# ChanghyeonKim93/bundle_adjustment_solver

Measured on AMD Instinct MI355X. Metric: lm_iterations_per_sec, higher is better.
Workload: dtype f64; 1 GPU; C4 stereo 6-DoF: 1000 poses / 500k landmarks / 5M obs; n_opt_poses=995, n_opt_landmarks=500000, n_observations=5000000, parallelism=single GPU, exchange=none

## Files before the change

### bundle_adjustment_solver_amd/_lib.py

```python
import ctypes as C
import os

_HERE = os.path.dirname(os.path.abspath(__file__))
LIB_PATH = os.environ.get("BA_HIP_LIB") or os.path.join(_HERE, "libba_hip.so")


class BaOptions(C.Structure):
    _fields_ = [
        ("threshold_step_size", C.c_float),
        ("threshold_cost_change", C.c_float),
        ("threshold_huber_loss", C.c_float),
        ("threshold_outlier_rejection", C.c_float),
        ("max_num_iterations", C.c_int),
        ("initial_lambda", C.c_float),
        ("decrease_ratio_lambda", C.c_float),
        ("increase_ratio_lambda", C.c_float),
        ("gauss_newton", C.c_int),
    ]


def make_options(max_iter=50, thr_step=1e-5, thr_cost=1e-5, huber=1.0,
                 outlier=2.0, lambda0=100.0, dec=0.33, inc=3.0,
                 gauss_newton=False):
    o = BaOptions()
# ... 47 lines not shown

SIGNATURES = {
    "ba_create": (C.c_int, [C.POINTER(_P), C.c_int]),
    "ba_destroy": (None, [_P]),
    "ba_last_error": (C.c_char_p, []),
    "ba_set_stream": (C.c_int, [_P, _P]),
    "ba_set_cameras": (C.c_int, [_P, C.c_int, _D, _D]),
    "ba_set_poses": (C.c_int, [_P, C.c_int, _D, _U8]),
    "ba_set_points": (C.c_int, [_P, C.c_int, _D, _U8]),
    "ba_set_observations": (C.c_int, [_P, C.c_int64, _I32, _I32, _I32, _D]),
    "ba_set_shard": (C.c_int, [_P, C.c_int, C.c_int]),
    "ba_finalize": (C.c_int, [_P]),
    "ba_update_values": (C.c_int, [_P, _D, _D]),
    "ba_partition_points": (C.c_int, [C.c_int, _U8, C.c_int, _U8, C.c_int64,
                                      _I32, _I32, C.c_int, _I32]),
    "ba_set_allreduce": (C.c_int, [_P, ALLREDUCE_FN, _P]),
    "ba_reduce_buffer_size": (C.c_int64, [_P, C.c_int]),
    "ba_bind_reduce_buffer": (C.c_int, [_P, C.c_int, _P, C.c_int64]),
    "ba_gather_points": (C.c_int, [_P]),
    "ba_rccl_available": (C.c_int, []),
    "ba_rccl_get_unique_id": (C.c_int, [_U8]),
    "ba_rccl_comm_create": (C.c_int, [C.POINTER(_P), C.c_int, C.c_int, _U8, C.c_int]),
    "ba_rccl_comm_size": (C.c_int, [_P]),
    "ba_rccl_comm_calls": (C.c_int64, [_P]),
    "ba_rccl_comm_destroy": (None, [_P]),
    "ba_rccl_allreduce_hook": (C.c_int, [_P, C.c_int, _P, C.c_int64, _P]),
    "ba_stream_create": (C.c_int, [C.POINTER(_P), C.c_int, C.c_int, C.c_int64]),
    "ba_stream_destroy": (None, [_P]),
    "ba_stream_set_cameras": (C.c_int, [_P, C.c_int, _D, _D]),
    "ba_stream_set_poses": (C.c_int, [_P, C.c_int, _D, _U8]),
    "ba_stream_set_points": (C.c_int, [_P, C.c_int, _D, _U8]),
    "ba_stream_set_observations": (C.c_int, [_P, C.c_int64, _I32, _I32, _I32, _D]),
    "ba_stream_finalize": (C.c_int, [_P]),
    "ba_stream_solve": (C.c_int, [_P, C.POINTER(BaOptions), C.POINTER(BaIterInfo),
                                  C.c_int, C.POINTER(C.c_int), C.POINTER(C.c_int)]),
    "ba_stream_lm_begin": (C.c_int, [_P, C.POINTER(BaOptions)]),
    "ba_stream_lm_iterate": (C.c_int, [_P, C.c_int]),
    "ba_stream_lm_sync": (C.c_int, [_P, C.POINTER(BaIterInfo), C.c_int,
                                    C.POINTER(C.c_int), C.POINTER(C.c_int)]),
    "ba_stream_get_poses": (C.c_int, [_P, _D]),
    "ba_stream_get_points": (C.c_int, [_P, _D]),
    "ba_stream_info": (C.c_int, [_P, C.POINTER(C.c_int64)]),
    "ba_solve": (C.c_int, [_P, C.POINTER(BaOptions), C.POINTER(BaIterInfo),
                           C.c_int, C.POINTER(C.c_int), C.POINTER(C.c_int)]),
    "ba_lm_begin": (C.c_int, [_P, C.POINTER(BaOptions)]),
    "ba_lm_iterate": (C.c_int, [_P, C.c_int]),
    "ba_lm_sync": (C.c_int, [_P, C.POINTER(BaIterInfo), C.c_int,
                             C.POINTER(C.c_int), C.POINTER(C.c_int)]),
    "ba_gd_begin": (C.c_int, [_P, C.POINTER(BaOptions)]),
    "ba_gd_iterate": (C.c_int, [_P, C.c_int]),
    "ba_gd_sync": (C.c_int, [_P, C.POINTER(BaIterInfo), C.c_int,
                             C.POINTER(C.c_int), C.POINTER(C.c_int)]),
    "ba_solve_gd": (C.c_int, [_P, C.POINTER(BaOptions), C.POINTER(BaIterInfo),
                              C.c_int, C.POINTER(C.c_int), C.POINTER(C.c_int)]),
    "ba_gd_get_gradient": (C.c_int, [_P, _D, _D]),
    "ba_stage_cost": (C.c_int, [_P, _D]),
    "ba_stage_linearize": (C.c_int, [_P, C.c_double, C.c_double]),
    "ba_stage_schur": (C.c_int, [_P]),
    "ba_stage_solve_reduced": (C.c_int, [_P]),
    "ba_stage_backsub_update": (C.c_int, [_P]),
    "ba_stage_scalars": (C.c_int, [_P, _D, _D, _D, _D]),
    "ba_stage_commit": (C.c_int, [_P, C.c_int]),
    "ba_enable_stage_timing": (C.c_int, [_P, C.c_int]),
    "ba_get_stage_ms": (C.c_int, [_P, _D, C.c_int]),
    "ba_num_opt_poses": (C.c_int, [_P]),
    "ba_num_opt_points": (C.c_int, [_P]),
    "ba_num_pairs": (C.c_int64, [_P]),
    "ba_num_schur_blocks": (C.c_int64, [_P]),
    "ba_num_schur_triples": (C.c_int64, [_P]),
    "ba_get_poses": (C.c_int, [_P, _D]),
    "ba_get_points": (C.c_int, [_P, _D, _U8]),
    "ba_get_A": (C.c_int, [_P, _D, _D]),
    "ba_get_C": (C.c_int, [_P, _D, _D]),
    "ba_get_Cinv": (C.c_int, [_P, _D, _D]),
    "ba_get_pairs": (C.c_int, [_P, _I32, _I32, _D]),
    "ba_get_S": (C.c_int, [_P, _D, _D]),
    "ba_get_xy": (C.c_int, [_P, _D, _D]),
    "ba_kernel_count": (C.c_int, []),
    "ba_kernel_name": (C.c_char_p, [C.c_int]),
    "ba_get_kernel_ms": (C.c_int, [_P, _D, C.POINTER(C.c_int64), C.c_int]),
    "ba_get_dense_info": (C.c_int, [_P, _D]),
    "ba_get_schur_info": (C.c_int, [_P, C.POINTER(C.c_int64)]),
    "ba_get_lin_info": (C.c_int, [_P, C.POINTER(C.c_int64)]),
    "ba_get_mask_info": (C.c_int, [_P, C.POINTER(C.c_int64)]),
    "ba_get_dropped_pivots": (C.c_int, [_P, C.POINTER(C.c_int64), C.c_int]),
    "ba_dense_spd_solve": (C.c_int, [_P, C.c_int, _D, _D, _D, _D]),
    "ba_pose_only_mono6": (C.c_int, [_P, _F, _F, C.c_int, C.c_float, C.c_float,
                                     C.c_float, C.c_float, _F, _U8,
                                     C.POINTER(BaOptions), C.POINTER(BaPoIter),
                                     C.c_int, C.POINTER(C.c_int),
                                     C.POINTER(C.c_int), _F]),
    "ba_pose_only_stereo6": (C.c_int, [_P, _F, _F, _F, C.c_int, _F, _F, _F, _F,
                                       _U8, _U8, C.POINTER(BaOptions),
                                       C.POINTER(BaPoIter), C.c_int,
                                       C.POINTER(C.c_int), C.POINTER(C.c_int),
                                       _F]),
    "ba_pose_only_mono3": (C.c_int, [_P, _F, _F, C.c_int, C.c_float, C.c_float,
                                     C.c_float, C.c_float, _F, _F, _F, _U8,
                                     C.POINTER(BaOptions), C.POINTER(BaPoIter),
                                     C.c_int, C.POINTER(C.c_int),
                                     C.POINTER(C.c_int), _F]),
    "ba_pose_only_stereo3": (C.c_int, [_P, _F, _F, _F, C.c_int, _F, _F, _F, _F,
                                       _F, _F, _U8, _U8, C.POINTER(BaOptions),
                                       C.POINTER(BaPoIter), C.c_int,
                                       C.POINTER(C.c_int), C.POINTER(C.c_int),
                                       _F]),
    "ba_pose_only_mono6_batch": (C.c_int, [_P, C.c_int, _I32, _F, _F, _F, _F, _U8,
                                           C.POINTER(BaOptions), C.POINTER(BaPoIter),
                                           C.c_int, C.POINTER(BaPoResult), _F]),
    "ba_pose_only_stereo6_batch": (C.c_int, [_P, C.c_int, _I32, _F, _F, _F, _F, _F,
                                             _F, _F, _U8, _U8, C.POINTER(BaOptions),
                                             C.POINTER(BaPoIter), C.c_int,
                                             C.POINTER(BaPoResult), _F]),
    "ba_pose_only_mono6_batch_device": (C.c_int, [_P, C.c_int, _P, _P, _P, _P, _P, _P,
                                                  C.POINTER(BaOptions), _P, C.c_int,
                                                  _P, _P, _P]),
    "ba_pose_only_stereo6_batch_device": (C.c_int, [_P, C.c_int, _P, _P, _P, _P, _P, _P,
                                                    _P, _P, _P, C.POINTER(BaOptions),
                                                    _P, C.c_int, _P, _P, _P]),
    "ba_right_camera_record": (C.c_int, [_F, _F, _F]),
    "ba_pose_only_mono3_batch": (C.c_int, [_P, C.c_int, _I32, _F, _F, _F, _F, _F, _F, _U8,
                                           C.POINTER(BaOptions), C.POINTER(BaPoIter),
                                           C.c_int, C.POINTER(BaPoResult), _F]),
    "ba_pose_only_stereo3_batch": (C.c_int, [_P, C.c_int, _I32, _F, _F, _F, _F, _F, _F,
                                             _F, _F, _F, _U8, _U8, C.POINTER(BaOptions),
                                             C.POINTER(BaPoIter), C.c_int,
                                             C.POINTER(BaPoResult), _F]),
    "ba_pose_only_mono3_batch_device": (C.c_int, [_P, C.c_int, _P, _P, _P, _P, _P, _P, _P,
                                                  C.POINTER(BaOptions), _P, C.c_int,
                                                  _P, _P, _P]),
    "ba_pose_only_stereo3_batch_device": (C.c_int, [_P, C.c_int, _P, _P, _P, _P, _P, _P,
                                                    _P, _P, _P, C.POINTER(BaOptions),
                                                    _P, C.c_int, _P, _P, _P]),
    "ba_planar_record": (C.c_int, [_F, _F, _F, _F, _F, _F]),
}

_lib = None


def _preload_shared_hip_runtime():
    import importlib.util
    try:
        spec = importlib.util.find_spec("torch")
    except (ImportError, ValueError):
        spec = None
    if spec is None or not spec.submodule_search_locations:
        return
    libdir = os.path.join(list(spec.submodule_search_locations)[0], "lib")
    for name in ("libhsa-runtime64.so", "libamdhip64.so"):
        path = os.path.join(libdir, name)
        if os.path.exists(path):
            try:
                C.CDLL(path, mode=C.RTLD_GLOBAL)
            except OSError:
                return


def load():
    global _lib
    if _lib is not None:
        return _lib
    if not os.path.exists(LIB_PATH):
        raise RuntimeError(
            "libba_hip.so is not built (%s). Run `python -c 'import "
            "__graft_entry__ as g; g.build()'` or `make -C "
            "bundle_adjustment_solver_amd/csrc`. The HIP path has no CPU "
# ... 21 lines not shown
```

### bundle_adjustment_solver_amd/csrc/ba_api.hip

```cpp
#include <hip/hip_runtime.h>

#include <algorithm>
#include <chrono>
#include <cmath>
#include <cstdio>
#include <cstdlib>
#include <cstring>
#include <string>
#include <vector>

#include "ba_handle.h"

namespace {
thread_local std::string g_err;
}
void ba::set_last_error(const std::string &m) { g_err = m; }
int ba::fail(const std::string &m) {
  g_err = m;
  return -1;
}
using ba::fail;

namespace {

// ... 421 lines not shown
    for (int64_t bk = 0; bk < pl.B; ++bk) {
      int32_t *r = bd.data() + 16 * bk;
      const int64_t c0 = pl.blk_contrib_ptr[bk], c1 = pl.blk_contrib_ptr[bk + 1];
      r[0] = pl.sblk_j[bk];
      r[1] = pl.sblk_k[bk];
      r[2] = (int32_t)c0;
      r[3] = (int32_t)(c1 - c0);
      r[4] = pl.sblk_tchunk_ptr[bk];
      r[5] = pl.sblk_tchunk_ptr[bk + 1] - pl.sblk_tchunk_ptr[bk];
      for (int t = 0; t < 8; ++t) r[8 + t] = c0 + t < c1 ? pl.contrib_slot[c0 + t] : 0;
    }
    if (pl.contrib_slot.size() >= (size_t)INT32_MAX) return fail("too many slot contributions for int32 indices");
    if (h->upload(&d.blk_desc, bd)) return -1;
  }
  d.n_sup = (int)pl.sup_desc.size();
  d.n_bchunk = (int)pl.bchunk_lm.size() - 1;
  if (h->upload(&d.bchunk_lm, pl.bchunk_lm)) return -1;
  {
    std::vector<ba::DevProblem::LmChunk> lc((size_t)d.n_bchunk);
    for (int c = 0; c < d.n_bchunk; ++c) {
      const int l0 = pl.bchunk_lm[c], l1 = pl.bchunk_lm[c + 1];
      lc[c].pb = pl.lm_pair_ptr[l0];
      lc[c].ob = pl.lm_obs_ptr[l0];
      lc[c].l0 = l0;
      lc[c].nl = l1 - l0;
      lc[c].np = (int32_t)(pl.lm_pair_ptr[l1] - pl.lm_pair_ptr[l0]);
      lc[c].no = (int32_t)(pl.lm_obs_ptr[l1] - pl.lm_obs_ptr[l0]);
    }
    if (h->upload(&d.lm_chunk, lc)) return -1;
  }
  d.n_slot = (int)pl.slot_blk.size();
  {
    static_assert(sizeof(ba::Plan::SupDesc) == sizeof(ba::DevProblem::SupDesc), "desc layout");
    static_assert(sizeof(ba::Plan::ChunkDesc) == sizeof(ba::DevProblem::ChunkDesc), "desc layout");
    if (h->dalloc(&d.sup_desc, pl.sup_desc.size()) || h->dalloc(&d.chunk_desc, pl.chunk_desc.size()))
      return -1;
    if (!pl.sup_desc.empty())
      HIP_TRY(hipMemcpy(d.sup_desc, pl.sup_desc.data(), pl.sup_desc.size() * sizeof(ba::Plan::SupDesc),
                        hipMemcpyHostToDevice));
    if (!pl.chunk_desc.empty())
      HIP_TRY(hipMemcpy(d.chunk_desc, pl.chunk_desc.data(),
                        pl.chunk_desc.size() * sizeof(ba::Plan::ChunkDesc), hipMemcpyHostToDevice));
  }
  h->kind(2);
  if (h->dalloc(&d.spart2, (size_t)d.n_slot * ba::kSlotStride)) return -1;
  h->kind(1);
  {
    static_assert(sizeof(ba::Plan::GrpDesc) == sizeof(ba::DevProblem::GrpDesc) && sizeof(ba::Plan::GrpDesc) == 128,
                  "group descriptor layout");
    static_assert(sizeof(ba::Plan::LinDesc) == sizeof(ba::DevProblem::LinDesc) && sizeof(ba::Plan::LinDesc) == 48,
                  "group linearisation descriptor layout");
    d.n_grp32 = (int)pl.grp32.size();
    d.n_grp64 = (int)pl.grp64.size();
    d.n_grp128 = (int)pl.grp128.size();
    if (h->dalloc(&d.grp32, pl.grp32.size()) || h->dalloc(&d.grp64, pl.grp64.size()) ||
        h->dalloc(&d.grp128, pl.grp128.size()))
      return -1;
    if (d.n_grp128)
      HIP_TRY(hipMemcpy(d.grp128, pl.grp128.data(), pl.grp128.size() * sizeof(ba::Plan::GrpDesc), hipMemcpyHostToDevice));
    if (d.n_grp32)
      HIP_TRY(hipMemcpy(d.grp32, pl.grp32.data(), pl.grp32.size() * sizeof(ba::Plan::GrpDesc), hipMemcpyHostToDevice));
    if (d.n_grp64)
      HIP_TRY(hipMemcpy(d.grp64, pl.grp64.data(), pl.grp64.size() * sizeof(ba::Plan::GrpDesc), hipMemcpyHostToDevice));
    d.lin_chunk0 = pl.lin_groups ? pl.n_bchunk_grp : 0;
    d.n_lin_desc = (int)pl.lin_desc.size();
    d.n_lin_plain = pl.n_lin_plain;
    d.n_bs_grp = d.n_lin_desc;
    d.n_lm_part = d.n_bs_grp + (d.n_bchunk - d.lin_chunk0 + ba::kBsChunks - 1) / ba::kBsChunks;
    d.n_lin_cost = d.n_bchunk + d.n_lin_desc;
    if (h->dalloc(&d.lin_desc, pl.lin_desc.size())) return -1;
    if (d.n_lin_desc)
      HIP_TRY(hipMemcpy(d.lin_desc, pl.lin_desc.data(), pl.lin_desc.size() * sizeof(ba::Plan::LinDesc), hipMemcpyHostToDevice));
    if (h->dalloc(&d.grp_pat, pl.grp_pat.size() / 2) || h->upload(&d.pose_gpart_ptr, pl.pose_gpart_ptr) ||
        h->upload(&d.pose_gpart, pl.pose_gpart))
      return -1;
    h->kind(2);
    if (h->dalloc(&d.Apart2, (size_t)pl.n_apart2 * 27) || h->dalloc(&d.lin_dump, (size_t)ba::kLinDump)) return -1;
    if (!pl.grp_pat.empty())
      HIP_TRY(hipMemcpy(d.grp_pat, pl.grp_pat.data(), pl.grp_pat.size() * sizeof(int32_t), hipMemcpyHostToDevice));
    if (pl.n_apart2 > 0) HIP_TRY(hipMemset(d.Apart2, 0, (size_t)pl.n_apart2 * 27 * sizeof(double)));
  }

  lap("structure uploads");
  for (int k = 0; k < 2; ++k) {
    h->kind(2);
    if (h->dalloc(&d.Cu[k], (size_t)pl.M * 6) || h->dalloc(&d.b[k], (size_t)pl.M * 3) ||
        h->dalloc(&d.W[k], std::max<size_t>(2, (size_t)pl.P * ba::kWStride)))
      return -1;
    h->kind(0);
    if (h->dalloc(&d.A[k], (size_t)pl.N * 36) || h->dalloc(&d.a[k], (size_t)pl.N * 6)) return -1;
    HIP_TRY(hipMemset(d.W[k], 0, std::max<size_t>(1, (size_t)pl.P * ba::kWStride) * sizeof(double)));
    HIP_TRY(hipMemset(d.A[k], 0, std::max<size_t>(1, (size_t)pl.N * 36) * sizeof(double)));
    HIP_TRY(hipMemset(d.a[k], 0, std::max<size_t>(1, (size_t)pl.N * 6) * sizeof(double)));
  }
  d.n_obs_lm = pl.M > 0 ? pl.lm_obs_ptr[pl.M] : 0;
  h->kind(2);
  if (h->dalloc(&d.Cd, (size_t)pl.M * 6) || h->dalloc(&d.Cinv, (size_t)pl.M * 6) ||
      h->dalloc(&d.lin_cost_part, (size_t)std::max(1, d.n_lin_cost)) ||
      h->dalloc(&d.Apart, (size_t)d.n_achunk * 27) ||
      h->dalloc(&d.spart, (size_t)d.n_tchunk * ba::kSlotStride) ||
      h->dalloc(&d.y, (size_t)pl.M * 3) || h->dalloc(&d.lm_part, (size_t)std::max(1, d.n_lm_part) * 2))
    return -1;
  h->kind(0);
  if (h->dalloc(&d.x, (size_t)pl.N * 6 + 64) || h->dalloc(&d.cost_part, (size_t)ba::kCostGrid) ||
      h->dalloc(&d.pose_part, (size_t)2 + 2 * ba::kPoseGrid) ||
      h->dalloc(&d.scal, (size_t)4) || h->dalloc(&d.ctrl, (size_t)1))
    return -1;
  HIP_TRY(hipMemset(d.lin_cost_part, 0, (size_t)std::max(1, d.n_lin_cost) * sizeof(double)));
  HIP_TRY(hipMemset(d.x, 0, ((size_t)pl.N * 6 + 64) * sizeof(double)));
  HIP_TRY(hipMemset(d.y, 0, std::max<size_t>(1, (size_t)pl.M * 3) * sizeof(double)));
  HIP_TRY(hipMemset(d.cost_part, 0, ba::kCostGrid * sizeof(double)));
  HIP_TRY(hipMemset(d.lm_part, 0, (size_t)std::max(1, d.n_lm_part) * 2 * sizeof(double)));
  HIP_TRY(hipMemset(d.pose_part, 0, (2 + 2 * ba::kPoseGrid) * sizeof(double)));
  HIP_TRY(hipMemset(d.scal, 0, 4 * sizeof(double)));
  d.log_cap = 4096;
  if (h->dalloc(&d.log, (size_t)d.log_cap)) return -1;

  lap("block storage");
  if (h->dense_owner) {
    const ba_handle *o = h->dense_owner;
    if (!o->finalized || o->plan.N != pl.N || o->plan.B != pl.B)
      return fail("ba_finalize: the dense owner belongs to a different problem");
    h->sched = o->sched;
    h->ddev = o->ddev;
    h->pose_col_h = o->pose_col_h;
    d.nb = o->d.nb; d.npad = o->d.npad; d.ld = o->d.ld;
    d.L = o->d.L; d.Ldiag = o->d.Ldiag; d.pose_col = o->d.pose_col; d.col_x = o->d.col_x;
    d.zt_I = o->d.zt_I; d.zt_J = o->d.zt_J; d.n_zt = o->d.n_zt;
    d.x = o->d.x;
    h->xbuf_n[0] = pl.B * 36 + 6 * (int64_t)pl.N;
    h->xbuf_n[1] = 4;
    h->xbuf_n[2] = 3 * (int64_t)pl.n_pt_global;
    if (h->dalloc(&d.Spk, (size_t)h->xbuf_n[0])) return -1;
    HIP_TRY(hipMemset(d.Spk, 0, (size_t)h->xbuf_n[0] * sizeof(double)));
  } else {
    const char *nat = getenv("BA_DENSE_NATURAL");
    const char *full = getenv("BA_DENSE_FULL");
    const char *force = getenv("BA_DENSE_NB");
    ba::DenseSchedule cand[2];
    double cost[2];
    const int orders[2] = {32, 64};
    const double level_us[2] = {16.0, 30.0};
    for (int k = 0; k < 2; ++k) {
      int ncb_k = 0;
      std::vector<uint8_t> adj;
      ba::tile_pattern(pl, ba::dense_poses_per_tile(orders[k]), ncb_k, adj);
      if (full && atoi(full) != 0) std::fill(adj.begin(), adj.end(), 1);
      ba::build_dense_schedule(ncb_k, adj, nat && atoi(nat) != 0, orders[k], cand[k]);
      cost[k] = cand[k].nlev * level_us[k];
    }
    if (getenv("BA_PLAN_STATS"))
      fprintf(stderr, "dense schedules: nb32 %d tiles %d levels max_rows %d fill %.3f | nb64 %d tiles %d levels max_rows %d fill %.3f\n",
              cand[0].ncb, cand[0].nlev, cand[0].max_rows, cand[0].fill, cand[1].ncb, cand[1].nlev, cand[1].max_rows,
              cand[1].fill);
    const bool narrow = cand[0].max_rows <= 6;
    int pick = (narrow && cost[0] <= cost[1]) ? 0 : 1;
    if (force && atoi(force) == 32) pick = 0;
    if (force && atoi(force) == 64) pick = 1;
    h->sched = cand[pick];
    const int nb = h->sched.nb;
    const int ppt = ba::dense_poses_per_tile(nb);
    const int ncb = h->sched.ncb;
    d.nb = nb;
    d.npad = ncb * nb;
    d.ld = d.npad + nb;
    h->xbuf_n[0] = pl.B * 36 + 6 * (int64_t)pl.N;
    h->xbuf_n[1] = 4;
    h->xbuf_n[2] = 3 * (int64_t)pl.n_pt_global;
    if (h->dalloc(&d.Spk, (size_t)h->xbuf_n[0])) return -1;
    if (h->dalloc(&d.L, (size_t)d.npad * d.ld)) return -1;
    if (h->dalloc(&d.Ldiag, (size_t)ncb * ba::dense_ws_per_block(nb))) return -1;
    h->pose_col_h.assign(pl.N, 0);
    std::vector<int> col_x((size_t)d.npad, -1);
    for (int j = 0; j < pl.N; ++j) {
      const int c0 = h->sched.pos_of_tile[j / ppt] * nb + 6 * (j % ppt);
      h->pose_col_h[j] = c0;
      for (int r = 0; r < 6; ++r) col_x[c0 + r] = 6 * j + r;
    }
    const ba::DenseSchedule &sc = h->sched;
    ba::DenseDev &dd = h->ddev;
    if (h->upload(&d.pose_col, h->pose_col_h) || upload_dense_schedule(h, sc, col_x, dd)) return -1;
    d.col_x = dd.col_x;
    if (times && dd.dag_items) fprintf(stderr, "[finalize] k_chol_dag: %d items\n", dd.n_dag_items);
    std::vector<int> ztI, ztJ;
    for (int p = 0; p < ncb; ++p) {
      ztI.push_back(p);
      ztJ.push_back(p);
      for (int q = sc.row_ptr[p]; q < sc.row_ptr[p + 1]; ++q) {
        ztI.push_back(sc.rows[q]);
        ztJ.push_back(p);
      }
    }
    d.n_zt = (int)ztI.size();
    if (h->upload(&d.zt_I, ztI) || h->upload(&d.zt_J, ztJ)) return -1;
    HIP_TRY(hipMemset(d.L, 0, (size_t)d.npad * d.ld * sizeof(double)));
    HIP_TRY(hipMemset(d.Spk, 0, (size_t)h->xbuf_n[0] * sizeof(double)));
  }

  lap("dense schedule + image");
  std::memset(&h->hc, 0, sizeof(h->hc));
  h->hc.lambda = 100.0;
  h->hc.huber = 1.0;
  h->hc.max_iter = 1;
  HIP_TRY(hipMemcpy(d.ctrl, &h->hc, sizeof(ba::DevCtrl), hipMemcpyHostToDevice));
  HIP_TRY(hipDeviceSynchronize());
  h->finalized = true;
  return 0;
}

int ba_update_values(ba_handle *h, const double *T_jw12, const double *X3) {
  if (!h || !h->finalized) return fail("ba_update_values: not finalized");
  if (h->arena) return fail("ba_update_values: not available on a streamed chunk");
  if (use_device(h)) return -1;
  const ba::Plan &pl = h->plan;
  join_side(h);
  HIP_TRY(hipStreamSynchronize(h->stream));
  if (T_jw12) {
    h->pose_T.assign(T_jw12, T_jw12 + 12 * (size_t)pl.n_pose);
    std::vector<double> poses((size_t)pl.n_pose * 12);
    for (int p = 0; p < pl.n_pose; ++p)
      std::memcpy(&poses[(size_t)p * 12], T_jw12 + (size_t)pl.pose_user_of_int[p] * 12, 12 * sizeof(double));
    for (int k = 0; k < 2; ++k)
      HIP_TRY(hipMemcpy(h->d.poses[k], poses.data(), poses.size() * sizeof(double), hipMemcpyHostToDevice));
  }
  if (X3) {
    h->pt_X.assign(X3, X3 + 3 * (size_t)pl.n_pt_global);
    std::vector<double> pts((size_t)pl.n_pt * 3);
    for (int q = 0; q < pl.n_pt; ++q)
      std::memcpy(&pts[(size_t)q * 3], X3 + (size_t)pl.pt_user_of_int[q] * 3, 3 * sizeof(double));
    if (pl.n_pt > 0)
      for (int k = 0; k < 2; ++k)
        HIP_TRY(hipMemcpy(h->d.pts[k], pts.data(), pts.size() * sizeof(double), hipMemcpyHostToDevice));
  }
  h->gathered_valid = false;
  h->lm_begun = false;
  h->gd_begun = false;
  h->tiles_ready = false;
  return 0;
}

int ba_set_allreduce(ba_handle *h, ba_allreduce_fn fn, void *user) {
  if (!h) return fail("null handle");
  h->ar_fn = fn;
  h->ar_user = user;
  return 0;
}

int64_t ba_reduce_buffer_size(ba_handle *h, int which) {
  if (!h || !h->finalized || which < 0 || which > 2) return -1;
  return h->xbuf_n[which];
}

int ba_bind_reduce_buffer(ba_handle *h, int which, void *dev_ptr, int64_t n) {
  if (!h || !h->finalized) return fail("ba_bind_reduce_buffer: not finalized");
  h->drop_graph();
  if (which < 0 || which > 2 || !dev_ptr || n < h->xbuf_n[which])
    return fail("ba_bind_reduce_buffer: bad argument");
  if (which == 0)
    h->d.Spk = (double *)dev_ptr;
  else if (which == 1)
    h->d.scal = (double *)dev_ptr;
  else {
    h->gbuf = (double *)dev_ptr;
    h->gbuf_bound = true;
  }
  return 0;
}

}

int ba::lm_prepare_ctrl(ba_handle *h, const ba_options *opt, int *done_after) {
  if (opt->max_num_iterations > h->d.log_cap) {
    ba::DevIterRec *nl = nullptr;
    const int keep = h->alloc_kind;
    h->alloc_kind = 0;
    const int rc = h->dalloc(&nl, (size_t)opt->max_num_iterations);
    h->alloc_kind = keep;
    if (rc) return -1;
    h->drop_graph();
    h->d.log = nl;
    h->d.log_cap = opt->max_num_iterations;
  }
  h->tiles_ready = false;
  h->gathered_valid = false;
  if (pull_ctrl(h)) return -1;
  ba::DevCtrl &c = h->hc;
  c.lambda = (double)opt->initial_lambda;
  c.huber = (double)opt->threshold_huber_loss;
  c.thr_step = (double)opt->threshold_step_size;
  c.thr_cost = (double)opt->threshold_cost_change;
  c.dec_ratio = (double)opt->decrease_ratio_lambda;
  c.inc_ratio = (double)opt->increase_ratio_lambda;
  c.max_iter = opt->max_num_iterations;
  c.gn = opt->gauss_newton ? 1 : 0;
  c.iter = 0;
  c.converged = 0;
  c.prev_cost = 0.0;
  *done_after = (opt->max_num_iterations <= 0) ? 1 : 0;
  c.done = 0;
  if (push_ctrl(h)) return -1;
  HIP_TRY(hipMemsetAsync(h->ddev.bad_pivots, 0, sizeof(int), h->stream));
  return 0;
}
int ba::ctrl_pull(ba_handle *h) { return pull_ctrl(h); }
int ba::ctrl_push(ba_handle *h) { return push_ctrl(h); }

extern "C" {

int ba_lm_begin(ba_handle *h, const ba_options *opt) {
  if (!h || !opt) return fail("ba_lm_begin: bad argument");
  if (!h->finalized && ba_finalize(h)) return -1;
  if (use_device(h)) return -1;
  join_side(h);
  int done_after = 0;
  if (ba::lm_prepare_ctrl(h, opt, &done_after)) return -1;
  h->gd_begun = false;
  enqueue_linearize(h, 0);
  ba::launch_scalars_cost_only(h->d, 1, h->stream);
  if (xchg(h, 1)) return -1;
  ba::launch_init_ctrl_cost(h->d, h->stream);
  if (done_after) {
    if (pull_ctrl(h)) return -1;
    h->hc.done = 1;
    if (push_ctrl(h)) return -1;
  }
  HIP_TRY(hipGetLastError());
  h->lm_begun = true;
  return 0;
}

int ba_lm_iterate(ba_handle *h, int n) {
  if (h && !h->lm_begun && h->gd_begun)
    return fail("ba_lm_iterate: the handle is in a gradient-descent loop (ba_gd_begin); call ba_lm_begin first");
  if (!h || !h->lm_begun) return fail("ba_lm_iterate: call ba_lm_begin first");
  if (use_device(h)) return -1;
  h->gathered_valid = false;
  const bool graphable = h->use_graph && !h->timing && !h->ar_fn && h->stream != nullptr;
  if (graphable && !h->graph_exec && n > 0) {
    HIP_TRY(hipStreamBeginCapture(h->stream, hipStreamCaptureModeThreadLocal));
    const int rc = enqueue_iteration(h);
    hipGraph_t g = nullptr;
    const hipError_t ec = hipStreamEndCapture(h->stream, &g);
    if (rc != 0 || ec != hipSuccess || !g) {
      if (g) (void)hipGraphDestroy(g);
      (void)hipGetLastError();
      h->use_graph = false;
    } else {
      h->graph = g;
      if (hipGraphInstantiate(&h->graph_exec, g, nullptr, nullptr, 0) != hipSuccess) {
        (void)hipGetLastError();
        h->drop_graph();
        h->use_graph = false;
      }
    }
  }
  for (int k = 0; k < n; ++k) {
    if (graphable && h->graph_exec) {
      HIP_TRY(hipGraphLaunch(h->graph_exec, h->stream));
    } else if (enqueue_iteration(h)) {
      return -1;
    }
  }
  return 0;
}

int ba_lm_sync(ba_handle *h, ba_iter_info *out, int cap, int *n_iter,
               int *converged) {
  if (!h || !h->lm_begun) return fail("ba_lm_sync: call ba_lm_begin first");
  if (use_device(h)) return -1;
  if (h->side_pending) (void)hipStreamWaitEvent(h->stream, h->ev_join, 0);
  if (pull_ctrl(h)) return -1;
  {
    int bp = 0;
    HIP_TRY(hipMemcpy(&bp, h->ddev.bad_pivots, sizeof(int), hipMemcpyDeviceToHost));
    if (bp >= ba::kFlowTimeout)
      return fail("ba_lm_sync: a dataflow hand-off of the reduced solve timed out (" +
                  std::to_string(bp / ba::kFlowTimeout) + " polls gave up); the iterations since ba_lm_begin "
                  "are invalid. BA_DENSE_FLOW=0 selects the per-level launches");
  }
  const int n = h->hc.iter;
  if (n_iter) *n_iter = n;
  if (converged) *converged = h->hc.converged;
  if (out && cap > 0 && n > 0) {
    static_assert(sizeof(ba::DevIterRec) == sizeof(ba_iter_info), "iter layout");
    const int m = std::min(std::min(n, cap), h->d.log_cap);
    HIP_TRY(hipMemcpy(out, h->d.log, (size_t)m * sizeof(ba_iter_info), hipMemcpyDeviceToHost));
  }
  return h->hc.done ? 1 : 0;
}

int ba_solve(ba_handle *h, const ba_options *opt, ba_iter_info *out, int cap,
             int *n_iter, int *converged) {
  if (ba_lm_begin(h, opt)) return -1;
  int done = opt->max_num_iterations <= 0;
  int issued = 0;
  while (!done) {
    const int batch = std::min(4, opt->max_num_iterations - issued);
    if (batch <= 0) break;
    if (ba_lm_iterate(h, batch)) return -1;
    issued += batch;
    int rc = ba_lm_sync(h, nullptr, 0, nullptr, nullptr);
    if (rc < 0) return -1;
    done = rc;
  }
  int rc = ba_lm_sync(h, out, cap, n_iter, converged);
  return rc < 0 ? -1 : 0;
}


static int gd_prepare(ba_handle *h, const char *who) {
// ... 93 lines not shown
  h->gathered_valid = false;
  for (int k = 0; k < n; ++k) {
    ba::launch_gd_update(h->d, h->gd, h->stream);
    ba::launch_gd_pass(h->d, h->gd, h->stream);
    ba::launch_gd_control(h->d, h->gd, 1, h->stream);
  }
  HIP_TRY(hipGetLastError());
  return 0;
}

int ba_gd_sync(ba_handle *h, ba_iter_info *out, int cap, int *n_iter, int *converged) {
  if (!h) return fail("ba_gd_sync: null handle");
  if (!h->gd_begun) return fail("ba_gd_sync: call ba_gd_begin first");
  if (use_device(h)) return -1;
  if (pull_ctrl(h)) return -1;
  const int n = h->hc.iter;
  if (n_iter) *n_iter = n;
  if (converged) *converged = h->hc.converged;
  if (out && cap > 0 && n > 0) {
    const int m = std::min(std::min(n, cap), h->d.log_cap);
    HIP_TRY(hipMemcpy(out, h->d.log, (size_t)m * sizeof(ba_iter_info), hipMemcpyDeviceToHost));
  }
  return h->hc.done ? 1 : 0;
}

int ba_solve_gd(ba_handle *h, const ba_options *opt, ba_iter_info *out, int cap, int *n_iter, int *converged) {
  if (ba_gd_begin(h, opt)) return -1;
  int done = opt->max_num_iterations <= 0;
  int issued = 0;
  while (!done) {
    const int batch = std::min(8, opt->max_num_iterations - issued);
    if (batch <= 0) break;
    if (ba_gd_iterate(h, batch)) return -1;
    issued += batch;
    const int rc = ba_gd_sync(h, nullptr, 0, nullptr, nullptr);
    if (rc < 0) return -1;
    done = rc;
  }
  const int rc = ba_gd_sync(h, out, cap, n_iter, converged);
  return rc < 0 ? -1 : 0;
}

int ba_gd_get_gradient(ba_handle *h, double *a6, double *b3) {
  if (!h || !h->finalized) return fail("ba_gd_get_gradient: not finalized");
  if (!h->gd_ready) return fail("ba_gd_get_gradient: call ba_gd_begin first");
  if (use_device(h)) return -1;
  const ba::Plan &pl = h->plan;
  HIP_TRY(hipStreamSynchronize(h->stream));
  if (a6 && pl.N > 0) HIP_TRY(hipMemcpy(a6, h->gd.a, (size_t)pl.N * 6 * sizeof(double), hipMemcpyDeviceToHost));
  if (b3) {
    std::vector<double> b;
    if (download(b, h->gd.b, (size_t)pl.M * 3, h->stream)) return -1;
    for (int i = 0; i < pl.M; ++i)
      std::memcpy(b3 + (size_t)pl.iopt_of_user[pl.pt_user_of_int[i]] * 3, &b[(size_t)i * 3], 3 * sizeof(double));
  }
  return 0;
}

int ba_stage_cost(ba_handle *h, double *cost) {
  if (!h || !h->finalized || !cost) return fail("ba_stage_cost: bad argument");
  if (use_device(h)) return -1;
  if (pull_ctrl(h)) return -1;
  h->hc.done = 0;
  if (push_ctrl(h)) return -1;
  join_side(h);
  ba::launch_cost(h->d, 0, 0, h->stream);
  ba::launch_scalars_cost_only(h->d, 0, h->stream);
  if (xchg(h, 1)) return -1;
  HIP_TRY(hipMemcpyAsync(cost, h->d.scal, sizeof(double), hipMemcpyDeviceToHost, h->stream));
  HIP_TRY(hipStreamSynchronize(h->stream));
  return 0;
}

int ba_stage_linearize(ba_handle *h, double lambda, double huber) {
  if (!h || !h->finalized) return fail("ba_stage_linearize: not finalized");
  if (use_device(h)) return -1;
  if (pull_ctrl(h)) return -1;
  h->hc.done = 0;
  h->hc.lambda = lambda;
  h->hc.huber = huber;
  if (push_ctrl(h)) return -1;
  join_side(h);
  enqueue_linearize(h, 0);
  ba::launch_damp_invert(h->d, h->stream);
  HIP_TRY(hipStreamSynchronize(h->stream));
  HIP_TRY(hipGetLastError());
  return 0;
}

int ba_stage_schur(ba_handle *h) {
  if (!h || !h->finalized) return fail("ba_stage_schur: not finalized");
  if (use_device(h)) return -1;
  join_side(h);
  ba::launch_schur(h->d, false, true, h->stream);
  if (xchg(h, 0)) return -1;
  HIP_TRY(hipStreamSynchronize(h->stream));
  HIP_TRY(hipGetLastError());
  return 0;
}

int ba_stage_solve_reduced(ba_handle *h) {
  if (!h || !h->finalized) return fail("ba_stage_solve_reduced: not finalized");
  if (use_device(h)) return -1;
  ba::launch_scatter(h->d, h->stream);
  ba::launch_dense_solve(h->d, h->sched, h->ddev, h->stream);
  HIP_TRY(hipStreamSynchronize(h->stream));
  HIP_TRY(hipGetLastError());
  return 0;
}

int ba_stage_backsub_update(ba_handle *h) {
  if (!h || !h->finalized) return fail("ba_stage_backsub_update: not finalized");
  if (use_device(h)) return -1;
  ba::launch_backsub_update(h->d, h->stream);
  HIP_TRY(hipStreamSynchronize(h->stream));
  HIP_TRY(hipGetLastError());
  return 0;
}

int ba_stage_scalars(ba_handle *h, double *trial_cost, double *model_change,
                     double *pose_step_sum, double *point_step_sum) {
  if (!h || !h->finalized) return fail("ba_stage_scalars: not finalized");
  if (use_device(h)) return -1;
  ba::launch_cost(h->d, 1, 0, h->stream);
  ba::launch_scalars(h->d, 0, h->stream);
  if (xchg(h, 1)) return -1;
  double sc[4], pp[2];
  HIP_TRY(hipMemcpyAsync(sc, h->d.scal, sizeof(sc), hipMemcpyDeviceToHost, h->stream));
  HIP_TRY(hipMemcpyAsync(pp, h->d.pose_part, sizeof(pp), hipMemcpyDeviceToHost, h->stream));
  HIP_TRY(hipStreamSynchronize(h->stream));
  if (trial_cost) *trial_cost = sc[0];
  if (model_change) *model_change = -sc[1];
  if (point_step_sum) *point_step_sum = sc[2];
  if (pose_step_sum) *pose_step_sum = pp[1];
  return 0;
}

int ba_stage_commit(ba_handle *h, int accept) {
  if (!h || !h->finalized) return fail("ba_stage_commit: not finalized");
  if (use_device(h)) return -1;
  h->gathered_valid = false;
  if (pull_ctrl(h)) return -1;
  if (accept) h->hc.cur ^= 1;
  if (push_ctrl(h)) return -1;
  HIP_TRY(hipStreamSynchronize(h->stream));
  return 0;
}

int ba_enable_stage_timing(ba_handle *h, int on) {
  if (!h) return fail("null handle");
  if (use_device(h)) return -1;
  if (on && !h->ev_ok) {
    for (int k = 0; k <= ST_N; ++k) HIP_TRY(hipEventCreate(&h->ev[k]));
    h->ev_ok = true;
  }
  h->timing = on != 0;
  h->kt.on = h->timing;
  return 0;
}

int ba_get_stage_ms(ba_handle *h, double out8[8], int reset) {
  if (!h || !out8) return fail("ba_get_stage_ms: bad argument");
  for (int k = 0; k < 8; ++k) out8[k] = h->stage_ms[k];
  if (reset)
    for (int k = 0; k < 8; ++k) h->stage_ms[k] = 0.0;
  return 0;
}

int ba_num_opt_poses(ba_handle *h) { return (h && h->finalized) ? h->plan.N : -1; }
int ba_num_opt_points(ba_handle *h) { return (h && h->finalized) ? h->plan.M : -1; }
int64_t ba_num_pairs(ba_handle *h) { return (h && h->finalized) ? h->plan.P - h->plan.n_pair_pad : -1; }
int64_t ba_num_schur_blocks(ba_handle *h) { return (h && h->finalized) ? h->plan.B : -1; }
int64_t ba_num_schur_triples(ba_handle *h) { return (h && h->finalized) ? h->plan.T : -1; }

int ba_get_poses(ba_handle *h, double *T_jw12) {
  if (!h || !h->finalized || !T_jw12) return fail("ba_get_poses: bad argument");
  if (use_device(h) || pull_ctrl(h)) return -1;
  std::vector<double> buf;
  if (download(buf, h->d.poses[h->hc.cur], (size_t)h->plan.n_pose * 12, h->stream)) return -1;
  for (int p = 0; p < h->plan.n_pose; ++p)
    std::memcpy(T_jw12 + (size_t)h->plan.pose_user_of_int[p] * 12, &buf[(size_t)p * 12],
                12 * sizeof(double));
  return 0;
}

__global__ void k_points_to_user(const double *__restrict__ src, const int32_t *__restrict__ user_of_int, int n,
                                 double *__restrict__ dst) {
  const int q = blockIdx.x * blockDim.x + threadIdx.x;
  if (q >= n) return;
  const size_t u = (size_t)user_of_int[q] * 3;
  dst[u + 0] = src[(size_t)q * 3 + 0];
  dst[u + 1] = src[(size_t)q * 3 + 1];
  dst[u + 2] = src[(size_t)q * 3 + 2];
}

int ba_gather_points(ba_handle *h) {
  if (!h || !h->finalized) return fail("ba_gather_points: not finalized");
  if (use_device(h)) return -1;
  h->gathered_valid = false;
  if (!h->ar_fn || h->world <= 1) return 0;
  const ba::Plan &pl = h->plan;
  const size_t n3 = (size_t)pl.n_pt_global * 3;
  if (!h->gbuf && h->dalloc(&h->gbuf, n3)) return -1;
  if (!h->pt_user_dev && h->upload(&h->pt_user_dev, pl.pt_user_of_int)) return -1;
  if (pull_ctrl(h)) return -1;
  join_side(h);
  HIP_TRY(hipMemsetAsync(h->gbuf, 0, n3 * sizeof(double), h->stream));
  if (pl.n_pt > 0)
    hipLaunchKernelGGL(k_points_to_user, dim3((pl.n_pt + 255) / 256), dim3(256), 0, h->stream,
                       (const double *)h->d.pts[h->hc.cur], (const int32_t *)h->pt_user_dev, pl.n_pt, h->gbuf);
  if (h->ar_fn(h->ar_user, 2, (void *)h->gbuf, (int64_t)n3, (void *)h->stream) != 0)
    return fail("ba_gather_points: all-reduce hook returned an error");
  if (download(h->gathered, h->gbuf, n3, h->stream)) return -1;
  HIP_TRY(hipGetLastError());
  h->gathered_valid = true;
  return 0;
}

int ba_get_points(ba_handle *h, double *X3, uint8_t *owned_mask) {
  if (!h || !h->finalized || !X3) return fail("ba_get_points: bad argument");
  if (h->gathered_valid) {
    std::memcpy(X3, h->gathered.data(), h->gathered.size() * sizeof(double));
    if (owned_mask) std::memset(owned_mask, 1, (size_t)h->plan.n_pt_global);
    return 0;
  }
  if (use_device(h) || pull_ctrl(h)) return -1;
// ... 12 lines not shown
  if (!h || !h->finalized) return fail("ba_get_A: not finalized");
  if (use_device(h)) return -1;
  join_side(h);
  if (pull_ctrl(h)) return -1;
  const int lb = h->hc.lcur;
  if (A36) {
    HIP_TRY(hipMemcpy(A36, h->d.A[lb], (size_t)h->plan.N * 36 * sizeof(double), hipMemcpyDeviceToHost));
    const double lp1 = 1.0 + h->hc.lambda;
    for (int j = 0; j < h->plan.N; ++j)
      for (int r = 0; r < 6; ++r) A36[(size_t)j * 36 + r * 7] *= lp1;
  }
  if (a6) HIP_TRY(hipMemcpy(a6, h->d.a[lb], (size_t)h->plan.N * 6 * sizeof(double), hipMemcpyDeviceToHost));
  return 0;
}

static void expand_sym3(const double *s6, double *f9) {
  f9[0] = s6[0]; f9[1] = s6[1]; f9[2] = s6[2];
  f9[3] = s6[1]; f9[4] = s6[3]; f9[5] = s6[4];
  f9[6] = s6[2]; f9[7] = s6[4]; f9[8] = s6[5];
}

static int get_sym_vec(ba_handle *h, const double *dS6, const double *dV3,
                       double *out9, double *out3) {
  const ba::Plan &pl = h->plan;
  std::vector<double> s6, v3;
  if (download(s6, dS6, (size_t)pl.M * 6, h->stream)) return -1;
  if (download(v3, dV3, (size_t)pl.M * 3, h->stream)) return -1;
  for (int i = 0; i < pl.M; ++i) {
    const int g = pl.iopt_of_user[pl.pt_user_of_int[i]];
    if (out9) expand_sym3(&s6[(size_t)i * 6], out9 + (size_t)g * 9);
    if (out3) std::memcpy(out3 + (size_t)g * 3, &v3[(size_t)i * 3], 3 * sizeof(double));
  }
  return 0;
}

int ba_get_C(ba_handle *h, double *C9, double *b3) {
  if (!h || !h->finalized) return fail("ba_get_C: not finalized");
  if (use_device(h)) return -1;
  join_side(h);
  if (pull_ctrl(h)) return -1;
  ba::launch_damp_invert_export(h->d, h->stream);
  return get_sym_vec(h, h->d.Cd, h->d.b[h->hc.lcur], C9, b3);
}

int ba_get_Cinv(ba_handle *h, double *Cinv9, double *Cinvb3) {
  if (!h || !h->finalized) return fail("ba_get_Cinv: not finalized");
  if (use_device(h)) return -1;
  const ba::Plan &pl = h->plan;
  std::vector<double> s6, b3;
  join_side(h);
  if (pull_ctrl(h)) return -1;
  ba::launch_damp_invert_export(h->d, h->stream);
  if (download(s6, h->d.Cinv, (size_t)pl.M * 6, h->stream)) return -1;
  if (download(b3, h->d.b[h->hc.lcur], (size_t)pl.M * 3, h->stream)) return -1;
  for (int i = 0; i < pl.M; ++i) {
    const int g = pl.iopt_of_user[pl.pt_user_of_int[i]];
    const double *ci = &s6[(size_t)i * 6], *b = &b3[(size_t)i * 3];
    if (Cinv9) expand_sym3(ci, Cinv9 + (size_t)g * 9);
    if (Cinvb3) {
      double *o = Cinvb3 + (size_t)g * 3;
      o[0] = ci[0] * b[0] + ci[1] * b[1] + ci[2] * b[2];
      o[1] = ci[1] * b[0] + ci[3] * b[1] + ci[4] * b[2];
      o[2] = ci[2] * b[0] + ci[4] * b[1] + ci[5] * b[2];
    }
  }
  return 0;
}

int ba_get_pairs(ba_handle *h, int32_t *pair_i, int32_t *pair_j, double *W18) {
  if (!h || !h->finalized) return fail("ba_get_pairs: not finalized");
  if (use_device(h)) return -1;
  const ba::Plan &pl = h->plan;
  auto padded = [&](int64_t p) { return !pl.pair_pad.empty() && pl.pair_pad[p]; };
  {
    int64_t o = 0;
    for (int64_t p = 0; p < pl.P; ++p) {
      if (padded(p)) continue;
      if (pair_i) pair_i[o] = pl.iopt_of_user[pl.pt_user_of_int[pl.pair_lm[p]]];
      if (pair_j) pair_j[o] = pl.pair_pose[p];
      ++o;
    }
  }
  if (W18) {
    if (pull_ctrl(h)) return -1;
    std::vector<double> w12((size_t)pl.P * ba::kWStride);
    if (pl.P > 0)
      HIP_TRY(hipMemcpy(w12.data(), h->d.W[h->hc.lcur], w12.size() * sizeof(double), hipMemcpyDeviceToHost));
    int64_t o = 0;
    for (int64_t p = 0; p < pl.P; ++p) {
      if (padded(p)) continue;
      const double *k = &w12[(size_t)p * ba::kWStride];
      double *W = W18 + (size_t)o * 18;
      for (int e = 0; e < 9; ++e) W[e] = k[e];
      for (int c = 0; c < 3; ++c) {
        W[9 + c] = k[10] * k[6 + c] - k[11] * k[3 + c];
        W[12 + c] = k[11] * k[c] - k[9] * k[6 + c];
        W[15 + c] = k[9] * k[3 + c] - k[10] * k[c];
      }
      ++o;
    }
  }
  return 0;
}

int ba_get_S(ba_handle *h, double *S, double *rhs) {
  if (!h || !h->finalized) return fail("ba_get_S: not finalized");
  if (use_device(h)) return -1;
  const ba::DevProblem &d = h->d;
  const int n6 = 6 * h->plan.N;
  std::vector<double> L;
  ba::launch_scatter(d, h->stream);
  if (download(L, d.L, (size_t)d.npad * d.ld, h->stream)) return -1;
  auto colof = [&](int e) { return h->pose_col_h[e / 6] + e % 6; };
  for (int c = 0; c < n6; ++c) {
    for (int r = c; r < n6; ++r) {
      int rr = colof(r), cc = colof(c);
      if (rr < cc) std::swap(rr, cc);
      const double v = L[(size_t)cc * d.ld + rr];
      if (S) {
        S[(size_t)r * n6 + c] = v;
        S[(size_t)c * n6 + r] = v;
      }
    }
    if (rhs) rhs[c] = L[(size_t)colof(c) * d.ld + d.npad];
  }
  return 0;
}

int ba_get_xy(ba_handle *h, double *x6, double *y3) {
  if (!h || !h->finalized) return fail("ba_get_xy: not finalized");
  if (use_device(h)) return -1;
  const ba::Plan &pl = h->plan;
  HIP_TRY(hipStreamSynchronize(h->stream));
  if (x6 && pl.N > 0)
    HIP_TRY(hipMemcpy(x6, h->d.x, (size_t)pl.N * 6 * sizeof(double), hipMemcpyDeviceToHost));
  if (y3) {
    std::vector<double> y;
    if (download(y, h->d.y, (size_t)pl.M * 3, h->stream)) return -1;
    for (int i = 0; i < pl.M; ++i) {
      const int g = pl.iopt_of_user[pl.pt_user_of_int[i]];
      std::memcpy(y3 + (size_t)g * 3, &y[(size_t)i * 3], 3 * sizeof(double));
    }
  }
  return 0;
}

int ba_kernel_count(void) { return ba::K_COUNT; }

const char *ba_kernel_name(int id) {
  static const char *names[ba::K_COUNT] = {
      "k_cost", "k_lin_landmarks", "k_lin_poses", "k_pose_finalize", "k_dense_init",
      "k_schur_lds", "k_schur_partial", "k_schur_final", "k_scatter",
      "k_chol_diag", "k_chol_trsm", "k_chol_update", "k_chol_back", "k_chol_diag_trsm", "k_chol_tail", "k_backsub_update",
      "k_pose_update", "k_scalars", "k_control", "k_damp_invert", "k_schur_grp", "k_lin_grp"};
  return (id >= 0 && id < ba::K_COUNT) ? names[id] : "";
}

int ba_get_kernel_ms(ba_handle *h, double *ms_out, int64_t *calls_out, int reset) {
  if (!h || !ms_out || !calls_out) return fail("ba_get_kernel_ms: bad argument");
  for (int k = 0; k < ba::K_COUNT; ++k) {
    ms_out[k] = h->kt.ms[k];
    calls_out[k] = h->kt.calls[k];
  }
  if (reset) h->kt.reset();
  return 0;
}

int ba_get_dense_info(ba_handle *h, double out4[4]) {
  if (!h || !h->finalized || !out4) return fail("ba_get_dense_info: bad argument");
  out4[0] = h->sched.fill;
  out4[1] = h->sched.flops;
  out4[2] = (double)h->sched.nlev;
  out4[3] = (double)h->d.npad;
  return 0;
}

int ba_get_schur_info(ba_handle *h, int64_t out8[8]) {
  if (!h || !h->finalized || !out8) return fail("ba_get_schur_info: bad argument");
  const ba::Plan &pl = h->plan;
  int64_t pairs = 0, triples = 0, mfma = 0;
  for (const auto *list : {&pl.grp32, &pl.grp64, &pl.grp128})
    for (const auto &g : *list) {
      pairs += (int64_t)g.nl * g.d;
      triples += (int64_t)g.nl * g.d * (g.d + 1) / 2;
      const int nt = list == &pl.grp32 ? 2 : (list == &pl.grp64 ? 4 : 8), krw = nt == 2 ? 36 : (nt == 4 ? 20 : 8);
      const int nlw = std::min(64 / g.d, krw / 3);
      for (int c0 = 0; c0 < g.nl; c0 += nlw)
        mfma += (int64_t)((3 * std::min(nlw, g.nl - c0) + 3) / 4) * (nt * (nt + 1) / 2);
    }
  out8[0] = (int64_t)pl.grp32.size();
  out8[1] = (int64_t)(pl.grp64.size() + pl.grp128.size());
  out8[2] = pl.M_grp;
  out8[3] = (int64_t)pl.sup_desc.size();
  out8[4] = pairs;
  out8[5] = triples;
  out8[6] = mfma;
  out8[7] = (int64_t)pl.tri_p.size();
  return 0;
}

int ba_get_lin_info(ba_handle *h, int64_t out4[4]) {
  if (!h || !h->finalized || !out4) return fail("ba_get_lin_info: bad argument");
  const ba::Plan &pl = h->plan;
  int64_t obs = 0;
  for (const auto &g : pl.lin_desc) obs += (int64_t)g.nl * g.no;
  out4[0] = (int64_t)pl.lin_desc.size();
  out4[1] = obs;
  out4[2] = (int64_t)pl.bchunk_lm.size() - 1 - (pl.lin_groups ? pl.n_bchunk_grp : 0);
  out4[3] = pl.n_pobs;
  return 0;
}

int ba_get_mask_info(ba_handle *h, int64_t out4[4]) {
  if (!h || !h->finalized || !out4) return fail("ba_get_mask_info: bad argument");
  const ba::Plan &pl = h->plan;
  int64_t lm = 0;
  for (const auto &g : pl.grp_range) lm += g.masked ? g.nl : 0;
  out4[0] = (int64_t)pl.lin_desc.size() - pl.n_lin_plain;
  out4[1] = lm;
  out4[2] = pl.n_obs - (pl.n_obs_global > 0 && h->world == 1 ? pl.n_obs_global : pl.n_obs);
  {
    int64_t pad = 0;
    for (int64_t s2 = 0; s2 < pl.n_obs; ++s2) pad += !(pl.obs_uv[2 * s2] == pl.obs_uv[2 * s2]);
    out4[2] = pad;
  }
  out4[3] = pl.n_pair_pad;
  return 0;
}

int ba_get_dropped_pivots(ba_handle *h, int64_t *count, int reset) {
  if (!h || !h->finalized || !count) return fail("ba_get_dropped_pivots: bad argument");
  if (use_device(h)) return -1;
  int v = 0;
  HIP_TRY(hipMemcpyAsync(&v, h->ddev.bad_pivots, sizeof(int), hipMemcpyDeviceToHost, h->stream));
  if (reset) HIP_TRY(hipMemsetAsync(h->ddev.bad_pivots, 0, sizeof(int), h->stream));
  HIP_TRY(hipStreamSynchronize(h->stream));
  *count = v % ba::kFlowTimeout;
  return 0;
}

int ba_dense_spd_solve(ba_handle *h, int n, const double *A, const double *b,
                       double *x, double *ms) {
  if (!h || n <= 0 || !A || !b || !x) return fail("ba_dense_spd_solve: bad argument");
  if (use_device(h)) return -1;
  const int nb = 64;
  const int ncb = (n + nb - 1) / nb;
  const int npad = ncb * nb;
  const int ld = npad + nb;
  std::vector<uint8_t> adj((size_t)ncb * ncb, 0);
  for (int I = 0; I < ncb; ++I)
    for (int J = 0; J < I; ++J) {
      bool any = false;
      for (int r = I * nb; r < std::min(n, (I + 1) * nb) && !any; ++r)
        for (int c = J * nb; c < (J + 1) * nb && !any; ++c) any = A[(size_t)r * n + c] != 0.0;
      adj[(size_t)I * ncb + J] = adj[(size_t)J * ncb + I] = any;
    }
  ba::DenseSchedule sc;
  const char *nat = getenv("BA_DENSE_NATURAL");
  ba::build_dense_schedule(ncb, adj, nat && atoi(nat) != 0, nb, sc);
  std::vector<int> colmap(npad), col_x(npad, -1);
  for (int c = 0; c < npad; ++c) colmap[c] = sc.pos_of_tile[c / nb] * nb + c % nb;
  std::vector<double> L((size_t)npad * ld, 0.0);
  for (int c = 0; c < npad; ++c) {
    if (c < n) {
      col_x[colmap[c]] = c;
      for (int r = c; r < n; ++r) {
        int rr = colmap[r], cc = colmap[c];
        if (rr < cc) std::swap(rr, cc);
        L[(size_t)cc * ld + rr] = A[(size_t)r * n + c];
      }
      L[(size_t)colmap[c] * ld + npad] = b[c];
    } else {
      L[(size_t)colmap[c] * ld + colmap[c]] = 1.0;
    }
  }
  struct Scratch {
    ba_handle *h;
    size_t mark;
    int kind;
    ~Scratch() {
// ... 522 lines not shown
```

### bundle_adjustment_solver_amd/csrc/ba_device.h

```cpp
#ifndef BA_DEVICE_H_
#define BA_DEVICE_H_

#include <hip/hip_runtime.h>
#include <stdint.h>
#include <stdlib.h>

#include <vector>

namespace ba {

struct DevCtrl {
  double lambda;
  double prev_cost;
  double huber;
  double thr_step;
  double thr_cost;
  double dec_ratio;
  double inc_ratio;
  unsigned long long t_last;
  int cur;
  int done;
  int iter;
  int converged;
  int max_iter;
  int gn;
  int lcur;
  int tcur, tlcur;
  int pad_;
};

struct DevIterRec {
  double cost, cost_change, average_reprojection_error, abs_gradient, abs_step,
      damping_term, iter_time_ms;
  int iteration_status, pad_;
  double rho, model_change, trial_cost;
};

constexpr int kWStride = 12;

struct DevProblem {
  int n_cam, n_pose, N, n_pt, M, M_global;
  int64_t n_obs, n_obs_opt, n_obs_global, P, n_pobs, T, B;
  int n_achunk, n_tchunk;
  double *cams;
  double *poses[2];
  double *pts[2];
  int4 *obs_idx;
  double2 *obs_uv;
  int64_t *lm_obs_ptr;
  int64_t *lm_pair_ptr;
  int32_t *pair_pose;
  int32_t *pair_lm;
  int2 *pobs_idx;
  int2 *obs_cp;
  double2 *pobs_uv;
  int32_t *achunk_pose;
  int64_t *achunk_begin, *achunk_end;
  int32_t *pose_achunk_ptr;
  int32_t *sblk_j, *sblk_k;
  int32_t *diag_blk;
  int64_t *tri_p, *tri_q;
  int32_t *tchunk_blk;
  int64_t *tchunk_begin, *tchunk_end;
  int32_t *sblk_tchunk_ptr;
  int n_sup, n_slot;
  struct SupDesc {
    int32_t s0, ns, chunk_begin, chunk_end;
  };
  struct ChunkDesc {
    int64_t p0, tb, sp;
    int32_t l0, nl, np, nt;
  };
  struct GrpDesc {
    int64_t p0;
    int32_t l0, nl, d, s0;
    int32_t pose[20];
    int32_t pad_[6];
  };
  struct LinDesc {
    int64_t p0, o0;
    int32_t l0, nl, d, no;
    int32_t pat0;
    int32_t apart0, cost_idx;
    int32_t pad_;
  };
  LinDesc *lin_desc;
  int n_lin_desc;
  int n_lin_plain;
  GrpDesc *grp32, *grp64, *grp128;
  int n_grp32, n_grp64, n_grp128;
  int2 *grp_pat;
  double *Apart2;
  double *lin_dump;
  int32_t *pose_gpart_ptr, *pose_gpart;
  int lin_chunk0;
  int n_lin_cost;
  int n_bs_grp;
  int n_lm_part;
  SupDesc *sup_desc;
  uint32_t *sup_lane;
  ChunkDesc *chunk_desc;
  uint16_t *chunk_sp;
  uint32_t *ltri;
  int64_t *blk_contrib_ptr;
  int32_t *contrib_slot;
  int32_t *blk_desc;
  double *spart2;
  double *Cu[2];
  double *b[2];
  double *W[2];
  double *A[2];
  double *a[2];
  double *Cinv;
  double *Cd;
  double *Apart;
  double *spart;
  double *x;
  double *y;
  double *cost_part;
  double *lin_cost_part;
  int64_t n_obs_lm;
  double *lm_part;
  double *pose_part;
  double *scal;
  DevCtrl *ctrl;
  DevIterRec *log;
  int log_cap;
  double *Spk;
  double *L;
  int npad, ld;
  double *Ldiag;
  int nb;
  int *pose_col;
  int *col_x;
  int32_t *bchunk_lm;
  struct LmChunk {
    int64_t pb, ob;
    int32_t l0, nl, np, no;
  };
  LmChunk *lm_chunk;
  int n_bchunk;
  int *zt_I, *zt_J;
  int n_zt;
};

constexpr int kLinDump = 64 * 4 * 4;
constexpr int kFlowTimeout = 1 << 20;
constexpr int kBsChunks = 4;
constexpr int kCostGrid = 1792;
constexpr int kLmGrid = 1024;
constexpr int kPoseGrid = 16;
constexpr int kGdFixGrid = 1024;
constexpr int kGdChunk = 512;
constexpr int kSlotStride = 42;

enum KernelId {
  K_COST = 0, K_LIN_LANDMARKS, K_LIN_POSES, K_POSE_FINALIZE, K_DENSE_INIT,
  K_SCHUR_LDS, K_SCHUR_PARTIAL, K_SCHUR_FINAL, K_SCATTER,
  K_CHOL_DIAG, K_CHOL_TRSM, K_CHOL_UPDATE, K_CHOL_BACK, K_CHOL_DIAG_TRSM, K_CHOL_TAIL, K_BACKSUB_UPDATE,
  K_POSE_UPDATE, K_SCALARS, K_CONTROL, K_DAMP_INVERT, K_SCHUR_GRP, K_LIN_GRP, K_COUNT
};
struct KernelTimer {
  bool on = false;
  std::vector<hipEvent_t> pool;
  std::vector<int> ids;
  double ms[K_COUNT] = {0};
  long calls[K_COUNT] = {0};
  void begin(int id, hipStream_t s);
  void end(hipStream_t s);
  void collect();
  void reset();
};
extern thread_local KernelTimer *g_ktimer;
#define BA_LAUNCH(id, kernel, grid, block, stream, ...)                     \
  do {                                                                      \
    if (::ba::g_ktimer && ::ba::g_ktimer->on) ::ba::g_ktimer->begin(id, stream); \
    hipLaunchKernelGGL(kernel, grid, block, 0, stream, __VA_ARGS__);        \
    if (::ba::g_ktimer && ::ba::g_ktimer->on) ::ba::g_ktimer->end(stream);  \
  } while (0)

#define BA_KEEP_S(x) asm volatile("" ::"s"(x))

void launch_cost(const DevProblem &d, int sel, int64_t begin, hipStream_t s);
void launch_lin_poses(const DevProblem &d, int sel, hipStream_t s);
void launch_lin_landmarks(const DevProblem &d, int sel, hipStream_t s);
void launch_damp_invert(const DevProblem &d, hipStream_t s);
void launch_schur(const DevProblem &d, bool direct, bool with_init, hipStream_t s);
void launch_schur_accumulate(const DevProblem &d, hipStream_t s);
void launch_schur_final(const DevProblem &d, bool direct, hipStream_t s);
void launch_backsub_update(const DevProblem &d, hipStream_t s, bool zero_tiles = false);
void launch_scatter(const DevProblem &d, hipStream_t s);
void launch_scalars_cost_only(const DevProblem &d, int cost_src, hipStream_t s);
void launch_scalars(const DevProblem &d, int cost_src, hipStream_t s);
// ... 129 lines not shown
```

### bundle_adjustment_solver_amd/csrc/ba_handle.h

```cpp
#ifndef BA_HANDLE_H_
#define BA_HANDLE_H_

#include <hip/hip_runtime.h>

#include <cstdint>
#include <chrono>
#include <string>
#include <vector>

#include "../../include/ba_hip.h"
#include "ba_dense_sched.h"
#include "ba_device.h"
#include "ba_plan.h"

namespace ba {
void launch_damp_invert_export(const DevProblem &d, hipStream_t s);
void set_last_error(const std::string &m);
int fail(const std::string &m);

struct DeviceArena {
  char *base = nullptr;
  size_t cap = 0;
};
}

#define HIP_TRY(expr)                                                        \
  do {                                                                       \
    hipError_t e_ = (expr);                                                  \
    if (e_ != hipSuccess)                                                    \
      return ::ba::fail(std::string(#expr) + ": " + hipGetErrorString(e_));  \
  } while (0)

enum Stage { ST_BUILD = 0, ST_SCHUR, ST_SOLVE, ST_BACKSUB, ST_COST, ST_CTRL, ST_XCHG, ST_N = 8 };

struct ba_handle {
  int device = 0;
  hipStream_t own_stream = nullptr;
  hipStream_t stream = nullptr;
  hipStream_t side_stream = nullptr;
  hipEvent_t ev_fork = nullptr, ev_join = nullptr;
  bool overlap = true;
  bool side_pending = false;
  bool tiles_ready = false;
  bool use_graph = false;
  hipGraph_t graph = nullptr;
  hipGraphExec_t graph_exec = nullptr;
  void drop_graph() {
    if (graph_exec) (void)hipGraphExecDestroy(graph_exec);
    if (graph) (void)hipGraphDestroy(graph);
    graph_exec = nullptr;
    graph = nullptr;
  }
  int n_cam = 0, n_pose = 0, n_pt = 0;
  int64_t n_obs = 0;
  std::vector<double> cam_intr, cam_T, pose_T, pt_X, obs_uv;
  std::vector<uint8_t> pose_fixed, pt_fixed;
  std::vector<int32_t> obs_cam, obs_pose, obs_pt;
  int rank = 0, world = 1;
  bool finalized = false;
  ba::Plan plan;
  ba::DevProblem d;
  std::vector<void *> allocs;
  ba_allreduce_fn ar_fn = nullptr;
  void *ar_user = nullptr;
  int64_t xbuf_n[3] = {0, 0, 0};
  double *gbuf = nullptr;
  bool gbuf_bound = false;
  int32_t *pt_user_dev = nullptr;
  std::vector<double> gathered;
  bool gathered_valid = false;
  ba::DevCtrl hc;
  bool timing = false;
  hipEvent_t ev[ST_N + 1];
  bool ev_ok = false;
  double stage_ms[ST_N] = {0, 0, 0, 0, 0, 0, 0, 0};
  bool lm_begun = false;
  ba::KernelTimer kt;
  ba::DenseSchedule sched;
  ba::DenseDev ddev;
  std::vector<int> pose_col_h;
  bool gd_ready = false;
  bool gd_begun = false;
  ba::GdDev gd{};
  uint8_t *po_dev = nullptr, *po_host = nullptr;
  size_t po_cap = 0;
  float *po_part = nullptr;

  ba::DeviceArena *arena = nullptr;
  size_t arena_imm = 0, arena_mut = 0;
  int alloc_kind = 0;
  ba_handle *dense_owner = nullptr;
  void kind(int k) { alloc_kind = arena ? k : 0; }

  template <class T>
  int dalloc(T **p, size_t n) {
    *p = nullptr;
    if (n == 0) n = 1;
    if (arena && alloc_kind != 0) {
      const size_t sz = (n * sizeof(T) + 255) & ~(size_t)255;
      if (arena_imm + arena_mut + sz > arena->cap)
        return ::ba::fail("the landmark chunk does not fit the device arena (" + std::to_string(arena->cap >> 20) +
                          " MiB): use more chunks or a larger arena");
      if (alloc_kind == 1) {
        *p = (T *)(arena->base + arena_imm);
        arena_imm += sz;
      } else {
        arena_mut += sz;
        *p = (T *)(arena->base + arena->cap - arena_mut);
      }
      return 0;
    }
    hipError_t e = hipMalloc((void **)p, n * sizeof(T));
    if (e != hipSuccess)
      return ::ba::fail(std::string("hipMalloc: ") + hipGetErrorString(e));
    allocs.push_back((void *)*p);
    return 0;
  }
  bool up_times = false;
  double up_alloc_s = 0, up_copy_s = 0;
  size_t up_bytes = 0, up_calls = 0;
  template <class T, class A>
  int upload(T **p, const std::vector<T, A> &v) {
    const auto t0 = up_times ? std::chrono::steady_clock::now() : std::chrono::steady_clock::time_point();
    if (dalloc(p, v.size())) return -1;
    const auto t1 = up_times ? std::chrono::steady_clock::now() : std::chrono::steady_clock::time_point();
    if (!v.empty()) {
      hipError_t e = hipMemcpy(*p, v.data(), v.size() * sizeof(T),
                               hipMemcpyHostToDevice);
      if (e != hipSuccess)
        return ::ba::fail(std::string("hipMemcpy H2D: ") + hipGetErrorString(e));
    }
    if (up_times) {
      const auto t2 = std::chrono::steady_clock::now();
      up_alloc_s += std::chrono::duration<double>(t1 - t0).count();
      up_copy_s += std::chrono::duration<double>(t2 - t1).count();
      up_bytes += v.size() * sizeof(T);
      ++up_calls;
    }
    return 0;
  }
  void free_device() {
    for (void *p : allocs) (void)hipFree(p);
    allocs.clear();
    if (po_dev) (void)hipFree(po_dev);
    if (po_host) (void)hipHostFree(po_host);
    po_dev = po_host = nullptr;
    po_cap = 0;
    po_part = nullptr;
    gbuf = nullptr;
    gbuf_bound = false;
    pt_user_dev = nullptr;
    gathered_valid = false;
    gd_ready = false;
    gd_begun = false;
    gd = ba::GdDev{};
    finalized = false;
  }
};

// ... 8 lines not shown
```

### bundle_adjustment_solver_amd/csrc/ba_kernels.hip

```cpp
#include "ba_device.h"
#include "ba_plan.h"

namespace ba {

thread_local KernelTimer *g_ktimer = nullptr;

void KernelTimer::begin(int id, hipStream_t s) {
  const size_t k = ids.size();
  while (pool.size() < 2 * (k + 1)) {
    hipEvent_t e;
    if (hipEventCreate(&e) != hipSuccess) return;
    pool.push_back(e);
  }
  ids.push_back(id);
  (void)hipEventRecord(pool[2 * k], s);
}
void KernelTimer::end(hipStream_t s) {
  if (ids.empty()) return;
  (void)hipEventRecord(pool[2 * (ids.size() - 1) + 1], s);
}
void KernelTimer::collect() {
  for (size_t k = 0; k < ids.size(); ++k) {
    float t = 0.f;
    if (hipEventElapsedTime(&t, pool[2 * k], pool[2 * k + 1]) == hipSuccess) {
// ... 18 lines not shown

template <int CTRL>
__device__ __forceinline__ double dpp_f64(double v) {
  union { double d; int i[2]; } u, r;
  u.d = v;
  r.i[0] = __builtin_amdgcn_update_dpp(0, u.i[0], CTRL, 0xf, 0xf, false);
  r.i[1] = __builtin_amdgcn_update_dpp(0, u.i[1], CTRL, 0xf, 0xf, false);
  return r.d;
}
__device__ __forceinline__ double lane_f64(double v, int src) {
  union { double d; int i[2]; } u;
  u.d = v;
  u.i[0] = __builtin_amdgcn_readlane(u.i[0], src);
  u.i[1] = __builtin_amdgcn_readlane(u.i[1], src);
  return u.d;
}
__device__ __forceinline__ double wave_sum(double v) {
  v += dpp_f64<0xB1>(v);
  v += dpp_f64<0x4E>(v);
  v += dpp_f64<0x141>(v);
  v += dpp_f64<0x140>(v);
  return ((lane_f64(v, 0) + lane_f64(v, 16)) + lane_f64(v, 32)) + lane_f64(v, 48);
}

__device__ __forceinline__ double block_sum(double v, double *sm) {
  v = wave_sum(v);
  const int lane = threadIdx.x & 63, wv = threadIdx.x >> 6;
  __syncthreads();
  if (lane == 0) sm[wv] = v;
  __syncthreads();
  double r = 0.0;
  if (threadIdx.x == 0) {
    const int nw = (blockDim.x + 63) >> 6;
    for (int w = 0; w < nw; ++w) r += sm[w];
  }
  return r;
}

__device__ __forceinline__ void block_sum2(double &a, double &b, double *sm) {
  a = wave_sum(a);
  b = wave_sum(b);
  const int lane = threadIdx.x & 63, wv = threadIdx.x >> 6;
  __syncthreads();
  if (lane == 0) {
    sm[wv] = a;
    sm[4 + wv] = b;
  }
  __syncthreads();
  if (threadIdx.x == 0) {
    a = ((sm[0] + sm[1]) + sm[2]) + sm[3];
    b = ((sm[4] + sm[5]) + sm[6]) + sm[7];
  }
}

constexpr int kCamLds = 8;
__device__ __forceinline__ void stage_cams(const DevProblem &d, double *cams_s) {
  const int n = (d.n_cam < kCamLds ? d.n_cam : kCamLds) * 16;
  for (int k = threadIdx.x; k < n; k += blockDim.x) cams_s[k] = d.cams[k];
}
template <bool LDSCAM>
__device__ __forceinline__ void load_cam(const DevProblem &d, const double *cams_s,
                                         int idx, double cam[16]) {
  if (LDSCAM) {
#pragma unroll
    for (int k = 0; k < 16; ++k) cam[k] = cams_s[idx * 16 + k];
  } else {
#pragma unroll
    for (int k = 0; k < 16; ++k) cam[k] = d.cams[(size_t)idx * 16 + k];
  }
}

struct ObsGeom {
  double Xij[3];
  double Xc[3];
  double r0, r1;
};

__device__ __forceinline__ void project(const double *__restrict__ cam,
                                        const double *__restrict__ T,
                                        const double X0, const double X1,
                                        const double X2, const double u,
                                        const double v, ObsGeom &g) {
#pragma clang fp contract(fast)
#pragma unroll
  for (int r = 0; r < 3; ++r)
    g.Xij[r] = (T[r * 3 + 0] * X0 + T[r * 3 + 1] * X1 + T[r * 3 + 2] * X2) +
               T[9 + r];
  const double *Rc = cam + 4;
  const double *tc = cam + 13;
#pragma unroll
  for (int r = 0; r < 3; ++r)
    g.Xc[r] = (Rc[r * 3 + 0] * g.Xij[0] + Rc[r * 3 + 1] * g.Xij[1] +
               Rc[r * 3 + 2] * g.Xij[2]) +
              tc[r];
  const double invz = 1.0 / g.Xc[2];
  g.r0 = cam[0] * (g.Xc[0] * invz) + cam[2] - u;
  g.r1 = cam[1] * (g.Xc[1] * invz) + cam[3] - v;
}

__device__ __forceinline__ void weight_and_G(const double *__restrict__ cam,
                                             const ObsGeom &g, double huber,
                                             double &w, double G[6]) {
#pragma clang fp contract(fast)
  const double invz = 1.0 / g.Xc[2];
  const double fxinvz = cam[0] * invz, fyinvz = cam[1] * invz;
  const double xinvz = g.Xc[0] * invz, yinvz = g.Xc[1] * invz;
  const double fx_xinvz2 = fxinvz * xinvz, fy_yinvz2 = fyinvz * yinvz;
  const double absr = fabs(g.r0) + fabs(g.r1);
  w = (absr > huber) ? (huber / absr) : 1.0;
  const double *Rc = cam + 4;
  G[0] = fxinvz * Rc[0] + (-fx_xinvz2) * Rc[6];
  G[1] = fxinvz * Rc[1] + (-fx_xinvz2) * Rc[7];
  G[2] = fxinvz * Rc[2] + (-fx_xinvz2) * Rc[8];
  G[3] = fyinvz * Rc[3] + (-fy_yinvz2) * Rc[6];
  G[4] = fyinvz * Rc[4] + (-fy_yinvz2) * Rc[7];
  G[5] = fyinvz * Rc[5] + (-fy_yinvz2) * Rc[8];
}

__device__ __forceinline__ void make_Q(const double G[6], const double Xij[3],
                                       double Q[12]) {
#pragma clang fp contract(fast)
#pragma unroll
  for (int r = 0; r < 2; ++r) {
    const double g0 = G[r * 3 + 0], g1 = G[r * 3 + 1], g2 = G[r * 3 + 2];
    Q[r * 6 + 0] = g0;
    Q[r * 6 + 1] = g1;
    Q[r * 6 + 2] = g2;
    Q[r * 6 + 3] = g2 * Xij[1] - g1 * Xij[2];
    Q[r * 6 + 4] = g0 * Xij[2] - g2 * Xij[0];
    Q[r * 6 + 5] = g1 * Xij[0] - g0 * Xij[1];
  }
}

__device__ __forceinline__ void make_R(const double G[6],
                                       const double *__restrict__ T,
                                       double Rm[6]) {
#pragma clang fp contract(fast)
#pragma unroll
  for (int r = 0; r < 2; ++r)
#pragma unroll
    for (int c = 0; c < 3; ++c)
      Rm[r * 3 + c] = G[r * 3 + 0] * T[0 * 3 + c] + G[r * 3 + 1] * T[1 * 3 + c] +
                      G[r * 3 + 2] * T[2 * 3 + c];
}

__device__ __forceinline__ void expand_W(const double *__restrict__ k12, double W[18]) {
#pragma unroll
  for (int e = 0; e < 9; ++e) W[e] = k12[e];
  const double X0 = k12[9], X1 = k12[10], X2 = k12[11];
#pragma unroll
  for (int c = 0; c < 3; ++c) {
    W[9 + c] = X1 * k12[6 + c] - X2 * k12[3 + c];
    W[12 + c] = X2 * k12[c] - X0 * k12[6 + c];
    W[15 + c] = X0 * k12[3 + c] - X1 * k12[c];
  }
}

__device__ __forceinline__ void ldlt3_inverse(const double c[6], double o[6]) {
  double a00 = c[0], a01 = c[1], a02 = c[2], a11 = c[3], a12 = c[4], a22 = c[5];
  int s0 = 0;
  {
    double m = fabs(a00);
    if (fabs(a11) > m) {
      m = fabs(a11);
      s0 = 1;
    }
    if (fabs(a22) > m) s0 = 2;
  }
  double t;
  if (s0 == 1) {
// ... 151 lines not shown
    id0.load(d, s);
    cuv = d.obs_uv[s];
  }
  if (d.ctrl->done) return;
  const int buf = sel == 2 ? d.ctrl->tcur : (d.ctrl->cur ^ sel);
  const double *__restrict__ poses = d.poses[buf];
  const double *__restrict__ pts = d.pts[buf];
  const int64_t s1 = s + stride < d.n_obs ? s + stride : d.n_obs - 1;
  ObsRec<SLIM> idn;
  idn.load(d, s1);
  double2 uvn = d.obs_uv[s1];
  double TA[12], XA[3], TB[12], XB[3];
  {
    const double *Tp = poses + (size_t)id0.pose() * 12;
    const double *Xp = pts + (size_t)id0.pt() * 3;
#pragma unroll
    for (int k = 0; k < 12; ++k) TA[k] = Tp[k];
#pragma unroll
    for (int k = 0; k < 3; ++k) XA[k] = Xp[k];
  }
  int ccam = id0.cam();
  double acc = 0.0;
  __syncthreads();
  while (s < d.n_obs) {
    COST_STEP(TA, XA, TB, XB)
    s += stride;
    if (s >= d.n_obs) break;
    COST_STEP(TB, XB, TA, XA)
    s += stride;
  }
  const double tot = block_sum(acc, sm);
  if (threadIdx.x == 0) d.cost_part[blockIdx.x] = tot;
}

#ifdef BA_LL_DBG
__device__ long long g_ll_dbg[32];
#define LL_STAMP() { if (ll_on && ll_n < 32) ll_s[ll_n++] = clock64(); }
#else
#define LL_STAMP()
#endif
template <bool LDSCAM>
__global__ __launch_bounds__(kBlock, 5) void k_lin_landmarks(DevProblem d, int sel) {
#ifdef BA_LL_DBG
  __shared__ long long ll_s[32];
  const bool ll_on = blockIdx.x == 9000 && threadIdx.x == 0;
  int ll_n = 0;
#endif
  LL_STAMP()
  __shared__ __attribute__((aligned(16))) double Wst[kSchurPairs * kWStride];
  __shared__ double Cb[kBlock * 9];
  __shared__ double cams_s[kCamLds * 16];
  __shared__ int lq[kSchurLandmarks + 1];
  __shared__ double smc[4];
  const int chunk = blockIdx.x + d.lin_chunk0;
  const DevProblem::LmChunk lc = d.lm_chunk[chunk];
  const int done = d.ctrl->done;
  const int buf = sel ? d.ctrl->tcur : d.ctrl->cur;
  const int lb = sel ? d.ctrl->tlcur : d.ctrl->lcur;
  const double huber = d.ctrl->huber;
  BA_KEEP_S((int)lc.pb);
  BA_KEEP_S((int)lc.ob);
  BA_KEEP_S(lc.l0);
  BA_KEEP_S(lc.no);
  BA_KEEP_S(done);
  if (LDSCAM) stage_cams(d, cams_s);
  const int tid = threadIdx.x;
  const int64_t pb = lc.pb;
  const int npair = lc.np;
  const int64_t ob = lc.ob, oe = lc.ob + lc.no;
  int4 id = make_int4(0, 0, 0, -1);
  double2 uv = make_double2(0.0, 0.0);
  if (tid < lc.no) {
    id = d.obs_idx[ob + tid];
    uv = d.obs_uv[ob + tid];
  }
  const int i = lc.l0 + tid;
  const bool own = tid < lc.nl;
  int64_t q0 = 0;
  if (own) q0 = d.lm_obs_ptr[i];
  if (done) return;
  LL_STAMP()
  const double *__restrict__ poses = d.poses[buf];
  const double *__restrict__ pts = d.pts[buf];
  double *__restrict__ Wg = d.W[lb];
  double cost_acc = 0.0;
  if (tid <= lc.nl) lq[tid] = (tid < lc.nl) ? (int)(q0 - ob) : lc.no;
  constexpr int kSumIt = (kSchurLandmarks * 9 + kBlock - 1) / kBlock;
  double csum[kSumIt];
#pragma unroll
  for (int k = 0; k < kSumIt; ++k) csum[k] = 0.0;
  __syncthreads();
  for (int64_t t0 = ob; t0 < oe; t0 += kBlock) {
    const int64_t s = t0 + tid;
    if (t0 > ob && s < oe) {
      id = d.obs_idx[s];
      uv = d.obs_uv[s];
    }
    if (s < oe) {
#pragma clang fp contract(fast)
      double cam[16];
      load_cam<LDSCAM>(d, cams_s, id.x, cam);
      const double *T = poses + (size_t)id.y * 12;
      const double *X = pts + (size_t)id.z * 3;
      ObsGeom g;
      project(cam, T, X[0], X[1], X[2], uv.x, uv.y, g);
      cost_acc += sqrt(g.r0 * g.r0 + g.r1 * g.r1);
      double w, G[6], Rm[6];
      weight_and_G(cam, g, huber, w, G);
      make_R(G, T, Rm);
      double *cb = Cb + tid * 9;
      cb[0] = w * (Rm[0] * Rm[0] + Rm[3] * Rm[3]);
      cb[1] = w * (Rm[0] * Rm[1] + Rm[3] * Rm[4]);
      cb[2] = w * (Rm[0] * Rm[2] + Rm[3] * Rm[5]);
      cb[3] = w * (Rm[1] * Rm[1] + Rm[4] * Rm[4]);
      cb[4] = w * (Rm[1] * Rm[2] + Rm[4] * Rm[5]);
      cb[5] = w * (Rm[2] * Rm[2] + Rm[5] * Rm[5]);
      const double wr0 = w * g.r0, wr1 = w * g.r1;
      cb[6] = Rm[0] * wr0 + Rm[3] * wr1;
      cb[7] = Rm[1] * wr0 + Rm[4] * wr1;
      cb[8] = Rm[2] * wr0 + Rm[5] * wr1;
      if (id.w >= 0) {
        const int lp = (int)(id.w - pb);
        double *Wp = (lp < kSchurPairs) ? (Wst + lp * kWStride)
                                        : (Wg + (size_t)id.w * kWStride);
#pragma unroll
        for (int r = 0; r < 3; ++r)
#pragma unroll
          for (int c = 0; c < 3; ++c)
            Wp[r * 3 + c] = w * (G[r] * Rm[c] + G[3 + r] * Rm[3 + c]);
#pragma unroll
        for (int r = 0; r < 3; ++r) Wp[9 + r] = g.Xij[r];
      }
    }
    LL_STAMP()
    __syncthreads();
    LL_STAMP()
    {
      const int o0 = (int)(t0 - ob);
#pragma unroll
      for (int k = 0; k < kSumIt; ++k) {
        const int t = tid + k * kBlock;
        if (t < lc.nl * 9) {
          const int li = t / 9, v = t - li * 9;
          const int a = max(lq[li], o0), b = min(lq[li + 1], o0 + kBlock);
          double sacc = 0.0;
          const double *cp = Cb + (a - o0) * 9 + v;
          int n = b - a;
          for (; n >= 4; n -= 4, cp += 36) {
            const double v0 = cp[0], v1 = cp[9], v2 = cp[18], v3 = cp[27];
            sacc = (((sacc + v0) + v1) + v2) + v3;
          }
          for (; n > 0; --n, cp += 9) sacc += cp[0];
          csum[k] += sacc;
        }
      }
    }
    LL_STAMP()
    __syncthreads();
    LL_STAMP()
  }
#pragma unroll
  for (int k = 0; k < kSumIt; ++k) {
    const int t = tid + k * kBlock;
    if (t < lc.nl * 9) Cb[t] = csum[k];
  }
  __syncthreads();
  double c00 = 0, c01 = 0, c02 = 0, c11 = 0, c12 = 0, c22 = 0;
// ... 48 lines not shown
template <bool LDSCAM, bool MASKED>
__device__ __forceinline__ void lin_grp_body(const DevProblem &d, const int sel, const int bid, double *red,
                                             double *cams_s, double *smc, int *slot_b, int *slot_e) {
#ifdef BA_LG_DBG
  __shared__ long long lg_s[64];
  const bool lg_on = blockIdx.x == 300 && threadIdx.x == 0;
  int lg_n = 0;
#endif
  LG_STAMP()
  const DevProblem::LinDesc *gp = d.lin_desc + bid;
  const int64_t p0 = gp->p0, o0 = gp->o0;
  const int l0 = gp->l0, nl = gp->nl, dd = gp->d, no = gp->no, pat0 = gp->pat0;
  const int apart0 = gp->apart0, cost_idx = gp->cost_idx;
  const int done = d.ctrl->done;
  const int buf = sel ? d.ctrl->tcur : d.ctrl->cur;
  const int lb = sel ? d.ctrl->tlcur : d.ctrl->lcur;
  const double huber = d.ctrl->huber;
  if (LDSCAM) stage_cams(d, cams_s);
  const int tid = threadIdx.x, lane = tid & 63;
  const int wv = __builtin_amdgcn_readfirstlane(tid >> 6);
  const int nlw = 64 / no < 7 ? 64 / no : 7;
  const int ilw = lane / no, oo = lane - ilw * no;
  const bool lane_on = ilw < nlw;
  const int2 pat = d.grp_pat[pat0 + oo];
  if (done) return;
  const int cam_id = pat.y & 0xffff, jj = (pat.y >> 16) & 0xff;
  const bool opt = (pat.y >> 29) & 1, lastw = (pat.y >> 30) & 1;
  {
    const int pose_prev = __shfl_up(pat.x, 1), pose_next = __shfl_down(pat.x, 1);
    if (tid < no && opt) {
      if (oo == 0 || pose_prev != pat.x) slot_b[jj] = oo;
      if (oo == no - 1 || pose_next != pat.x) slot_e[jj] = oo + 1;
    }
  }
  const double *__restrict__ pts = d.pts[buf];
#define LING_LDX(p_) (*(p_))
  double T[12], cam[16];
  {
    const double *Tp = d.poses[buf] + (size_t)pat.x * 12;
#pragma unroll
    for (int k = 0; k < 12; ++k)
      T[k] = Tp[k];
  }
  __syncthreads();
  load_cam<LDSCAM>(d, cams_s, cam_id, cam);
  unsigned later_bits = 0u, pose_bits = 0u;
  if (MASKED && opt) {
    const int sb_l = slot_b[jj], se_l = slot_e[jj];
    const unsigned upto_e = se_l >= 32 ? 0xffffffffu : ((1u << se_l) - 1u);
    pose_bits = upto_e & ~((1u << sb_l) - 1u);
    later_bits = oo + 1 >= 32 ? 0u : (upto_e & ~((1u << (oo + 1)) - 1u));
  }
  double *__restrict__ Wg = d.W[lb];
  double *__restrict__ Cg = d.Cu[lb];
  double *__restrict__ bg = d.b[lb];
  double *cbw = red + wv * kLgArea;
  double acc[27];
#pragma unroll
  for (int k = 0; k < 27; ++k) acc[k] = 0.0;
  double cost_acc = 0.0;
  const int per_step = 4 * nlw;
  const int nstep = (nl + per_step - 1) / per_step;
  auto il_of = [&](int st) { return (st * 4 + wv) * nlw + ilw; };
  auto clampi = [&](int il) { return min(il, nl - 1); };
  double2 uvq[3];
  double Xq[3][3];
#pragma unroll
  for (int u = 0; u < 2; ++u) {
    const int ilc = clampi(il_of(u));
    uvq[u] = d.obs_uv[o0 + (int64_t)ilc * no + oo];
    const double *Xp = pts + (size_t)(l0 + ilc) * 3;
    Xq[u][0] = LING_LDX(&Xp[0]);
    Xq[u][1] = LING_LDX(&Xp[1]);
    Xq[u][2] = LING_LDX(&Xp[2]);
  }
  const int sum_li = lane / 9, sum_v = lane - sum_li * 9;
  const bool sum_on = lane < nlw * 9, sum_neg = sum_v >= 6;
  const double *sum_p = cbw + (sum_on ? sum_li * no * 9 + sum_v : 0);
  double *sum_g = sum_v < 6 ? Cg + (size_t)l0 * 6 + sum_v : bg + (size_t)l0 * 3 + (sum_v - 6);
  const int sum_stride = sum_v < 6 ? 6 : 3;
  double2 *dumpW = (double2 *)(d.lin_dump + (size_t)((bid & 63) * 4 + wv) * 4);
  double *dumpC = (double *)dumpW + 2;
  double2 *stgW = (double2 *)(cbw + 64 * 9);
  double2 *stgW_mine = stgW + (ilw * dd + jj) * 6;
  constexpr int kLgPass = (7 * 10 * 6 + 63) / 64;
  int il0p = nl;
  double vv[8];
  double2 wvv[kLgPass];
  int lastp = 0;
  double2 *dstWp = dumpW;
#define LING_FLUSH_ISSUE()                                                          \
  {                                                                                 \
    _Pragma("unroll") for (int u_ = 0; u_ < 8; ++u_) vv[u_] = sum_p[(u_ < no ? u_ : 0) * 9]; \
    const int nls_ = nl - il0p < nlw ? nl - il0p : nlw;                             \
    const int n2_ = nls_ * dd * 6;                                                  \
    dstWp = n2_ > 0 ? (double2 *)(Wg + (size_t)(p0 + (int64_t)il0p * dd) * kWStride) : dumpW; \
    lastp = n2_ > 0 ? n2_ - 1 : 0;                                                  \
    _Pragma("unroll") for (int k_ = 0; k_ < kLgPass; ++k_) wvv[k_] = stgW[min(lane + 64 * k_, lastp)]; \
  }
#define LING_FLUSH_FINISH()                                                         \
  {                                                                                 \
    double sacc_ = 0.0;                                                             \
    _Pragma("unroll") for (int u_ = 0; u_ < 8; ++u_) sacc_ += (u_ < no) ? vv[u_] : 0.0; \
    for (int q_ = 8; q_ < no; ++q_) sacc_ += sum_p[q_ * 9];                         \
    const int ils_ = il0p + sum_li;                                                 \
    double *dst_ = (sum_on && ils_ < nl) ? sum_g + (size_t)ils_ * sum_stride : dumpC; \
    *dst_ = sum_neg ? -sacc_ : sacc_;                                               \
    _Pragma("unroll") for (int k_ = 0; k_ < kLgPass; ++k_) dstWp[min(lane + 64 * k_, lastp)] = wvv[k_]; \
  }
#define LING_STEP(CUR, NXT2)                                                        \
  {                                                                                 \
    _Pragma("clang fp contract(fast)")                                              \
    LG_STAMP()                                                                      \
    LING_FLUSH_ISSUE()                                                              \
    {                                                                               \
      const int ilc_ = clampi(il_of(st + 2));                                       \
      uvq[NXT2] = d.obs_uv[o0 + (int64_t)ilc_ * no + oo];                           \
      const double *Xp_ = pts + (size_t)(l0 + ilc_) * 3;                            \
      Xq[NXT2][0] = LING_LDX(&Xp_[0]);                                              \
      Xq[NXT2][1] = LING_LDX(&Xp_[1]);                                              \
      Xq[NXT2][2] = LING_LDX(&Xp_[2]);                                              \
    }                                                                               \
    const int il0_ = (st * 4 + wv) * nlw;                                           \
    const int il_ = il0_ + ilw;                                                     \
    const bool valid_ = lane_on && il_ < nl && (!MASKED || uvq[CUR].x == uvq[CUR].x); \
    bool wr_ = lastw;                                                               \
    if (MASKED) {                                                                   \
      const unsigned long long vb_ = __ballot(valid_);                              \
      const unsigned mine_ = (unsigned)(vb_ >> (lane - oo));                        \
      wr_ = opt && (valid_ ? (mine_ & later_bits) == 0u : (lastw && (mine_ & pose_bits) == 0u)); \
    }                                                                               \
    ObsGeom g;                                                                      \
    project(cam, T, Xq[CUR][0], Xq[CUR][1], Xq[CUR][2], uvq[CUR].x, uvq[CUR].y, g); \
    if (MASKED) {                                                                   \
      g.r0 = valid_ ? g.r0 : 0.0;                                                   \
      g.r1 = valid_ ? g.r1 : 0.0;                                                   \
    }                                                                               \
    cost_acc += valid_ ? sqrt(g.r0 * g.r0 + g.r1 * g.r1) : 0.0;                     \
    double w, G[6], Rm[6], Q[12], cbv[9], kk[12];                                   \
    weight_and_G(cam, g, huber, w, G);                                              \
    w = valid_ ? w : 0.0;                                                           \
    make_R(G, T, Rm);                                                               \
    {                                                                               \
                      \
      double wR[6];                                                                 \
      _Pragma("unroll") for (int e_ = 0; e_ < 6; ++e_) wR[e_] = w * Rm[e_];         \
      cbv[0] = Rm[0] * wR[0] + Rm[3] * wR[3];                                       \
      cbv[1] = Rm[0] * wR[1] + Rm[3] * wR[4];                                       \
      cbv[2] = Rm[0] * wR[2] + Rm[3] * wR[5];                                       \
      cbv[3] = Rm[1] * wR[1] + Rm[4] * wR[4];                                       \
      cbv[4] = Rm[1] * wR[2] + Rm[4] * wR[5];                                       \
      cbv[5] = Rm[2] * wR[2] + Rm[5] * wR[5];                                       \
      cbv[6] = wR[0] * g.r0 + wR[3] * g.r1;                                         \
      cbv[7] = wR[1] * g.r0 + wR[4] * g.r1;                                         \
      cbv[8] = wR[2] * g.r0 + wR[5] * g.r1;                                         \
       \
       \
      _Pragma("unroll") for (int r = 0; r < 3; ++r)                                 \
      _Pragma("unroll") for (int c = 0; c < 3; ++c)                                 \
        kk[r * 3 + c] = G[r] * wR[c] + G[3 + r] * wR[3 + c];                        \
      _Pragma("unroll") for (int r = 0; r < 3; ++r) kk[9 + r] = g.Xij[r];           \
    }                                                                               \
    {                                                                               \
             \
      const double wq = opt ? w : 0.0;                                              \
      make_Q(G, g.Xij, Q);                                                          \
      int k = 0;                                                                    \
      _Pragma("unroll") for (int r = 0; r < 6; ++r) {                               \
        const double q0 = wq * Q[r], q1 = wq * Q[6 + r];                            \
        _Pragma("unroll") for (int c = r; c < 6; ++c)                               \
          { acc[k] = fma(q0, Q[c], fma(q1, Q[6 + c], acc[k])); ++k; }               \
      }                                                                             \
      const double ar0 = wq * g.r0, ar1 = wq * g.r1;                                \
      _Pragma("unroll") for (int c = 0; c < 6; ++c)                                 \
        acc[21 + c] = fma(Q[c], ar0, fma(Q[6 + c], ar1, acc[21 + c]));              \
    }                                                                               \
    LG_STAMP()                                                                      \
    LING_FLUSH_FINISH()                                                             \
    LG_STAMP()                                                                      \
                           \
    __builtin_amdgcn_fence(__ATOMIC_RELEASE, "wavefront");                          \
    __builtin_amdgcn_wave_barrier();                                                \
    __builtin_amdgcn_fence(__ATOMIC_ACQUIRE, "wavefront");                          \
    {                                                                               \
      double *cb = cbw + lane * 9;                                                  \
      _Pragma("unroll") for (int e_ = 0; e_ < 9; ++e_) cb[e_] = cbv[e_];            \
      if (wr_ && lane_on) {                                                         \
        _Pragma("unroll") for (int r = 0; r < 6; ++r)                               \
          stgW_mine[r] = make_double2(kk[2 * r], kk[2 * r + 1]);                    \
      }                                                                             \
    }                                                                               \
    il0p = il0_;                                                                    \
    __builtin_amdgcn_fence(__ATOMIC_RELEASE, "wavefront");                          \
    __builtin_amdgcn_wave_barrier();                                                \
    __builtin_amdgcn_fence(__ATOMIC_ACQUIRE, "wavefront");                          \
  }
  int st = 0;
  while (st < nstep) {
    LING_STEP(0, 2)
    if (++st >= nstep) break;
    LING_STEP(1, 0)
    if (++st >= nstep) break;
    LING_STEP(2, 1)
    ++st;
  }
  LING_FLUSH_ISSUE()
  LING_FLUSH_FINISH()
#undef LING_STEP
#undef LING_LDX
#undef LING_FLUSH_ISSUE
#undef LING_FLUSH_FINISH
  LG_STAMP()
  {
    const double tot = block_sum(cost_acc, smc);
    if (tid == 0) d.lin_cost_part[cost_idx] = tot;
  }
#pragma unroll
  for (int half = 0; half < 2; ++half) {
    __syncthreads();
#pragma unroll
    for (int k = 0; k < 14; ++k)
      if (half * 14 + k < 27) cbw[k * 64 + lane] = acc[half * 14 + k];
    __syncthreads();
    for (int t = tid; t < dd * 14; t += kBlock) {
      const int pj = t / 14, k = t - pj * 14, e = half * 14 + k;
      if (e >= 27) continue;
      const int sb = slot_b[pj], se = slot_e[pj];
      double sacc = 0.0;
      for (int w4 = 0; w4 < 4; ++w4)
        for (int li = 0; li < nlw; ++li)
          for (int q = sb; q < se; ++q) sacc += red[w4 * kLgArea + k * 64 + li * no + q];
      d.Apart2[(size_t)(apart0 + pj) * 27 + e] = sacc;
    }
  }
  LG_STAMP()
#ifdef BA_LG_DBG
  if (lg_on) { for (int q = 0; q < 64; ++q) g_lg_dbg[q] = q < lg_n ? lg_s[q] : 0; }
#endif
}

template <bool LDSCAM, bool MASKED>
__global__ __launch_bounds__(kBlock, 2) void k_lin_grp(DevProblem d, int sel, int piece0) {
  __shared__ __attribute__((aligned(16))) double red[4 * kLgArea];
  __shared__ double cams_s[kCamLds * 16];
  __shared__ double smc[4];
  __shared__ int slot_b[kGrpMaxPoses], slot_e[kGrpMaxPoses];
  lin_grp_body<LDSCAM, MASKED>(d, sel, piece0 + blockIdx.x, red, cams_s, smc, slot_b, slot_e);
}

__global__ __launch_bounds__(kBlock) void k_damp_invert(DevProblem d, int store_cd) {
  const int i = blockIdx.x * kBlock + threadIdx.x;
  const int ic = i < d.M ? i : 0;
  const double lp1 = 1.0 + d.ctrl->lambda;
  const int lb = d.ctrl->lcur;
  const int done = d.ctrl->done;
  const double *c = d.Cu[lb] + (size_t)ic * 6;
  double cd[6];
#pragma unroll
  for (int k = 0; k < 6; ++k) cd[k] = c[k];
  if (done || i >= d.M) return;
  cd[0] *= lp1;
  cd[3] *= lp1;
  cd[5] *= lp1;
  double ci[6];
  spd3_inverse(cd, ci);
  double *Io = d.Cinv + (size_t)i * 6;
#pragma unroll
  for (int k = 0; k < 6; ++k) Io[k] = ci[k];
  if (store_cd) {
    double *Do = d.Cd + (size_t)i * 6;
#pragma unroll
    for (int k = 0; k < 6; ++k) Do[k] = cd[k];
// ... 121 lines not shown
    while (k >= 6 - r) {
      k -= 6 - r;
      ++r;
    }
    const int c = r + k;
    d.A[lb][(size_t)j * 36 + r * 6 + c] = s;
    d.A[lb][(size_t)j * 36 + c * 6 + r] = s;
  } else {
    const int r = e - 21;
    d.a[lb][(size_t)j * 6 + r] = -s;
  }
}
__global__ __launch_bounds__(kBlock) void k_pose_finalize(DevProblem d, int sel) {
  if (d.ctrl->done) return;
  pose_finalize_body(d, sel, blockIdx.x * kBlock + threadIdx.x);
}

constexpr int kWLds = 14;
constexpr int kSchurRW = (kSchurPairs * (kWStride / 2) + kBlock - 1) / kBlock;
constexpr int kSchurRC = (kSchurLandmarks * 3 + kBlock - 1) / kBlock;
static_assert(kSchurTri <= 4 * kBlock, "one uint4 of triple words per lane");
constexpr int kSchurRB = (kSchurLandmarks * 3 + kBlock - 1) / kBlock;

#define SCHUR_PREFETCH(cd_)                                                   \
  {                                                                           \
    const double2 *src_ = (const double2 *)(Wg + (size_t)(cd_).p0 * kWStride);  \
    _Pragma("unroll") for (int k_ = 0; k_ < kSchurRW; ++k_) {                 \
      const int t_ = tid + k_ * kBlock;                                       \
      rw[k_] = (t_ < (cd_).np * 6) ? src_[t_] : make_double2(0.0, 0.0);       \
    }                                                                         \
    const double2 *cs_ = (const double2 *)(d.Cinv + (size_t)(cd_).l0 * 6);    \
    _Pragma("unroll") for (int k_ = 0; k_ < kSchurRC; ++k_) {                 \
      const int t_ = tid + k_ * kBlock;                                       \
      rc[k_] = (t_ < (cd_).nl * 3) ? cs_[t_] : make_double2(0.0, 0.0);        \
    }                                                                         \
     \
    rt = (tid * 4 < (cd_).nt) ? ((const uint4 *)(d.ltri + (cd_).tb))[tid]     \
                              : make_uint4(0u, 0u, 0u, 0u);                   \
    _Pragma("unroll") for (int k_ = 0; k_ < kSchurRB; ++k_) {                 \
      const int t_ = tid + k_ * kBlock;                                       \
      rb[k_] = (t_ < (cd_).nl * 3) ? bg[(size_t)(cd_).l0 * 3 + t_] : 0.0;     \
    }                                                                         \
          \
    rpl = (tid < (cd_).np) ? d.pair_lm[(cd_).p0 + tid] : 0;                   \
    rsp = (tid <= ns) ? (int)d.chunk_sp[(cd_).sp + tid] : 0;                  \
  }

__device__ __forceinline__ int64_t uni64(int64_t v) {
  const uint32_t lo = __builtin_amdgcn_readfirstlane((uint32_t)v);
  const uint32_t hi = __builtin_amdgcn_readfirstlane((uint32_t)((uint64_t)v >> 32));
  return (int64_t)(((uint64_t)hi << 32) | lo);
}
#ifdef BA_SCHUR_DBG
__device__ long long g_schur_dbg[4][160];
#define DBG_STAMP() { if (dbg_on && dbg_n < 160) dbg_s[dbg_n++] = clock64(); }
#else
#define DBG_STAMP()
#endif
__global__ __launch_bounds__(kBlock, 3) void k_schur_lds(DevProblem d) {
#ifdef BA_SCHUR_DBG
  __shared__ long long dbg_s[160];
  const int dbg_slot = blockIdx.x == 10 ? 0 : blockIdx.x == 700 ? 1 : blockIdx.x == 1200 ? 2 : blockIdx.x == 1900 ? 3 : -1;
  const bool dbg_on = dbg_slot >= 0 && threadIdx.x == 0;
  int dbg_n = 0;
  DBG_STAMP()
#endif
  __shared__ __attribute__((aligned(16))) double Ws[kSchurPairs * kWLds];
  __shared__ __attribute__((aligned(16))) double Vs[kSchurPairs * 18];
  __shared__ __attribute__((aligned(16))) double Cs[kSchurLandmarks * 6];
  __shared__ double Bs[kSchurLandmarks * 3];
  __shared__ __attribute__((aligned(16))) uint32_t Ts[kSchurTri];
  __shared__ uint16_t Sp[kSchurSlots + 1];
  __shared__ uint16_t Pl[kSchurPairs];
  __shared__ DevProblem::ChunkDesc Cdsc[kSchurSuperChunks];
  const int tid = threadIdx.x;
  const DevProblem::SupDesc sd = d.sup_desc[blockIdx.x];
  const uint32_t lane_word = d.sup_lane[(size_t)blockIdx.x * kBlock + tid];
  const int ns = sd.ns;
  const int done = d.ctrl->done;
  const int lbs = d.ctrl->lcur;
  BA_KEEP_S(sd.chunk_begin);
  BA_KEEP_S(done);
  if (done) return;
  const double *__restrict__ Wg = d.W[lbs];
  const double *__restrict__ bg = d.b[lbs];
  const int slot = (int)(lane_word & 0xffu);
  const int h = (int)((lane_word >> 8) & 1u), sub2 = (int)((lane_word >> 9) & 0x1fu);
  const int tps2 = (int)((lane_word >> 14) & 0x3fu);
  const bool owner = slot < ns;
  double acc[18], racc[3];
#pragma unroll
  for (int k = 0; k < 18; ++k) acc[k] = 0.0;
#pragma unroll
  for (int k = 0; k < 3; ++k) racc[k] = 0.0;
  DevProblem::ChunkDesc cd = d.chunk_desc[sd.chunk_begin];
  if (tid < sd.chunk_end - sd.chunk_begin) Cdsc[tid] = d.chunk_desc[sd.chunk_begin + tid];
  double2 rw[kSchurRW], rc[kSchurRC];
  uint4 rt;
  double rb[kSchurRB];
  int rpl, rsp;
  SCHUR_PREFETCH(cd)
  __syncthreads();
  for (int ch = sd.chunk_begin; ch < sd.chunk_end; ++ch) {
    {
      double2 *dst = (double2 *)Ws;
#pragma unroll
      for (int k = 0; k < kSchurRW; ++k) {
        const int t = tid + k * kBlock;
        const int pr = t / 6;
        if (t < cd.np * 6) dst[pr * (kWLds / 2) + (t - pr * 6)] = rw[k];
      }
      double2 *cdst = (double2 *)Cs;
#pragma unroll
      for (int k = 0; k < kSchurRC; ++k) {
        const int t = tid + k * kBlock;
        if (t < cd.nl * 3) cdst[t] = rc[k];
      }
      if (tid * 4 < cd.nt) ((uint4 *)Ts)[tid] = rt;
#pragma unroll
      for (int k = 0; k < kSchurRB; ++k) {
        const int t = tid + k * kBlock;
        if (t < cd.nl * 3) Bs[t] = rb[k];
      }
      if (tid < cd.np) Pl[tid] = (uint16_t)(rpl - cd.l0);
      if (tid <= ns) Sp[tid] = (uint16_t)rsp;
    }
    const int np = cd.np;
    DBG_STAMP()
    if (ch + 1 < sd.chunk_end) {
      const DevProblem::ChunkDesc *q = &Cdsc[ch + 1 - sd.chunk_begin];
      cd.p0 = uni64(q->p0);
      cd.tb = uni64(q->tb);
      cd.sp = uni64(q->sp);
      cd.l0 = __builtin_amdgcn_readfirstlane(q->l0);
      cd.nl = __builtin_amdgcn_readfirstlane(q->nl);
      cd.np = __builtin_amdgcn_readfirstlane(q->np);
      cd.nt = __builtin_amdgcn_readfirstlane(q->nt);
      SCHUR_PREFETCH(cd)
    }
    DBG_STAMP()
    __syncthreads();
    DBG_STAMP()
    {
      static_assert(kBlock == 2 * kSchurPairs && (kSchurPairs & (kSchurPairs - 1)) == 0, "V phase mapping");
      const int pr = tid & (kSchurPairs - 1);
      const bool hi = tid >= kSchurPairs;
      if (pr < np) {
        const double *kk = Ws + pr * kWLds;
        const double *ci = Cs + (int)Pl[pr] * 6;
        double k9[9], c6[6], x3[3], wr[9];
#pragma unroll
        for (int e = 0; e < 9; ++e) k9[e] = kk[e];
#pragma unroll
        for (int e = 0; e < 6; ++e) c6[e] = ci[e];
        if (hi) {
#pragma unroll
          for (int e = 0; e < 3; ++e) x3[e] = kk[9 + e];
#pragma unroll
          for (int c = 0; c < 3; ++c) {
            wr[c] = x3[1] * k9[6 + c] - x3[2] * k9[3 + c];
            wr[3 + c] = x3[2] * k9[c] - x3[0] * k9[6 + c];
            wr[6 + c] = x3[0] * k9[3 + c] - x3[1] * k9[c];
          }
        } else {
#pragma unroll
          for (int e = 0; e < 9; ++e) wr[e] = k9[e];
        }
// ... 9 lines not shown
    }
    DBG_STAMP()
    __syncthreads();
    DBG_STAMP()
    if (owner) {
      const int t1 = (int)Sp[slot + 1];
      int t = (int)Sp[slot] + sub2;
      uint32_t pq = Ts[t < kSchurTri ? t : kSchurTri - 1];
      while (t < t1) {
        const int tn = t + tps2;
        const uint32_t pqn = Ts[tn < kSchurTri ? tn : kSchurTri - 1];
        __builtin_amdgcn_sched_barrier(0);
        const uint32_t pp = pq >> 16, qq = pq & 0xffu;
        const double *vp = Vs + pp * 18 + h * 9;
        const double2 *wp = (const double2 *)(Ws + qq * kWLds);
        const double *bp = Bs + ((pq >> 8) & 0xffu) * 3;
        const double bm = (pp == qq) ? 1.0 : 0.0;
        const double b0 = bp[0] * bm, b1 = bp[1] * bm, b2 = bp[2] * bm;
        double w[12];
#pragma unroll
        for (int k = 0; k < 6; ++k) {
          const double2 b2 = wp[k];
          w[2 * k] = b2.x;
          w[2 * k + 1] = b2.y;
        }
        const double X0 = w[9], X1 = w[10], X2 = w[11];
#pragma unroll
        for (int r = 0; r < 3; ++r) {
          const double v0 = vp[r * 3 + 0], v1 = vp[r * 3 + 1], v2 = vp[r * 3 + 2];
          const double t0 = fma(v2, w[2], fma(v1, w[1], v0 * w[0]));
          const double t1 = fma(v2, w[5], fma(v1, w[4], v0 * w[3]));
          const double t2 = fma(v2, w[8], fma(v1, w[7], v0 * w[6]));
          acc[r * 6 + 0] += t0;
          acc[r * 6 + 1] += t1;
          acc[r * 6 + 2] += t2;
          acc[r * 6 + 3] = fma(-X2, t1, fma(X1, t2, acc[r * 6 + 3]));
          acc[r * 6 + 4] = fma(-X0, t2, fma(X2, t0, acc[r * 6 + 4]));
          acc[r * 6 + 5] = fma(-X1, t0, fma(X0, t1, acc[r * 6 + 5]));
          racc[r] = fma(v2, b2, fma(v1, b1, fma(v0, b0, racc[r])));
        }
        pq = pqn;
        t = tn;
      }
    }
    DBG_STAMP()
    __syncthreads();
    DBG_STAMP()
  }
  DBG_STAMP()
#pragma unroll
  for (int k = 0; k < 21; ++k) {
    double a2 = k < 18 ? acc[k] : racc[k - 18];
    int w = tps2;
#pragma unroll
    for (int off = 8; off >= 1; off >>= 1) {
      const double o2 = __shfl_down(a2, 2 * off, 64);
      if (sub2 + off < w) a2 += o2;
      w = w < off ? w : off;
    }
    if (k < 18) acc[k] = a2; else racc[k - 18] = a2;
  }
#ifdef BA_SCHUR_DBG
  if (dbg_on)
    for (int k = 0; k < 160; ++k) g_schur_dbg[dbg_slot][k] = k < dbg_n ? dbg_s[k] : 0;
#endif
  if (owner && sub2 == 0) {
    double *o = d.spart2 + (size_t)(sd.s0 + slot) * kSlotStride;
#pragma unroll
    for (int k = 0; k < 18; ++k) o[h * 18 + k] = acc[k];
#pragma unroll
    for (int k = 0; k < 3; ++k) o[36 + h * 3 + k] = racc[k];
  }
}

#ifndef BA_GRP_KRW
#define BA_GRP_KRW 36
#endif
#ifdef BA_GRP_DBG
__device__ long long g_grp_dbg[256];
#define GRP_STAMP() { if (gdbg_on && gdbg_n < 256) gdbg_s[gdbg_n++] = clock64(); }
#else
#define GRP_STAMP()
#endif
template <int NT>
__global__ __launch_bounds__(kBlock, (NT == 2 && BA_GRP_KRW <= 24) ? 3 : 2) void k_schur_grp(DevProblem d, const DevProblem::GrpDesc *grps) {
  constexpr int TW = 16 * NT;
#ifndef BA_GRP_KRW
#define BA_GRP_KRW 36
#endif
  constexpr int KRW = NT == 2 ? BA_GRP_KRW : 20;
  constexpr int NTILE = NT * (NT + 1) / 2;
  constexpr int RS = 2 * TW + (NT == 2 ? 6 : 0);
  constexpr int IMG = (KRW / 2) * RS;
  __shared__ __attribute__((aligned(16))) double VA[4][IMG];
  __shared__ __attribute__((aligned(16))) double WB[4][IMG];
  static_assert(IMG >= 256, "the final reduction uses VA as 4 x 256 doubles");
#ifdef BA_GRP_DBG
  __shared__ long long gdbg_s[256];
  const bool gdbg_on = blockIdx.x == 600 && threadIdx.x == 0;
  int gdbg_n = 0;
#endif
  const int tid = threadIdx.x, lane = tid & 63, wv = tid >> 6;
  const int lr = lane & 15, lk = lane >> 4;
  const DevProblem::GrpDesc gd = grps[blockIdx.x];
  const int done = d.ctrl->done;
  const int lb = d.ctrl->lcur;
  BA_KEEP_S(gd.l0);
  BA_KEEP_S(done);
  if (done) return;
  const double *__restrict__ Wg = d.W[lb];
  const double *__restrict__ bg = d.b[lb];
  const double *__restrict__ Cug = d.Cu[lb];
  const double lp1 = 1.0 + d.ctrl->lambda;
  const int dd = gd.d;
  const int nlw = min(64 / dd, KRW / 3);
  const int il = lane / dd, jj = lane - il * dd;
  const int nch = (gd.nl + nlw - 1) / nlw;
  double *va = VA[wv], *wb = WB[wv];
  for (int e = lane; e < IMG; e += 64) {
    va[e] = 0.0;
    wb[e] = 0.0;
  }
  double2 rw[2][6], rc[2][3];
  double rb[2][3];
#define GRP_PREFETCH(B, ch_)                                                        \
  {                                                                                 \
    const int c0_ = (ch_) * nlw;                                                    \
    const bool on_ = il < min(nlw, gd.nl - c0_);                                    \
    const double2 *wp_ = (const double2 *)(Wg + (size_t)(gd.p0 + (int64_t)c0_ * dd + (on_ ? lane : 0)) * kWStride); \
    const int lm_ = gd.l0 + c0_ + (on_ ? il : 0);                                   \
    const double2 *cp_ = (const double2 *)(Cug + (size_t)lm_ * 6);                  \
    _Pragma("unroll") for (int k_ = 0; k_ < 6; ++k_) rw[B][k_] = wp_[k_];           \
    _Pragma("unroll") for (int k_ = 0; k_ < 3; ++k_) rc[B][k_] = cp_[k_];           \
    _Pragma("unroll") for (int k_ = 0; k_ < 3; ++k_) rb[B][k_] = bg[(size_t)lm_ * 3 + k_]; \
  }
  v4f64 acc[NTILE];
#pragma unroll
  for (int t = 0; t < NTILE; ++t) acc[t] = (v4f64){0.0, 0.0, 0.0, 0.0};
  if (wv < nch) GRP_PREFETCH(0, wv)
  if (wv + 4 < nch) GRP_PREFETCH(1, wv + 4)
#define GRP_IDX(k_, col_) (((k_) >> 1) * RS + (col_) * 2 + ((k_) & 1))
#define GRP_STAGE(B)                                                                \
  if (ch < nch) {                                                                   \
    GRP_STAMP()                                                                     \
    const int nlc = min(nlw, gd.nl - ch * nlw);                                     \
    if (il < nlc) {                                                                 \
       \
      _Pragma("clang fp contract(fast)")                                            \
      const double k9[9] = {rw[B][0].x, rw[B][0].y, rw[B][1].x, rw[B][1].y, rw[B][2].x, \
                            rw[B][2].y, rw[B][3].x, rw[B][3].y, rw[B][4].x};        \
      const double x0 = rw[B][4].y, x1 = rw[B][5].x, x2 = rw[B][5].y;               \
          \
      const double cd_[6] = {rc[B][0].x * lp1, rc[B][0].y, rc[B][1].x, rc[B][1].y * lp1, rc[B][2].x, rc[B][2].y * lp1}; \
      double c6[6];                                                                 \
      spd3_inverse(cd_, c6);                                                        \
      double w[18];                                                                 \
      _Pragma("unroll") for (int e = 0; e < 9; ++e) w[e] = k9[e];                   \
      _Pragma("unroll") for (int c = 0; c < 3; ++c) {                               \
        w[9 + c] = x1 * k9[6 + c] - x2 * k9[3 + c];                                 \
        w[12 + c] = x2 * k9[c] - x0 * k9[6 + c];                                    \
        w[15 + c] = x0 * k9[3 + c] - x1 * k9[c];                                    \
      }                                                                             \
      const int kb = 3 * il, cb = 6 * jj;                                           \
      const int i0 = GRP_IDX(kb, cb), i1 = GRP_IDX(kb + 1, cb), i2 = GRP_IDX(kb + 2, cb); \
      _Pragma("unroll") for (int r = 0; r < 6; ++r) {                               \
        const double w0 = w[r * 3], w1 = w[r * 3 + 1], w2 = w[r * 3 + 2];           \
        va[i0 + 2 * r] = w0 * c6[0] + w1 * c6[1] + w2 * c6[2];                      \
        va[i1 + 2 * r] = w0 * c6[1] + w1 * c6[3] + w2 * c6[4];                      \
        va[i2 + 2 * r] = w0 * c6[2] + w1 * c6[4] + w2 * c6[5];                      \
        wb[i0 + 2 * r] = w0;                                                        \
        wb[i1 + 2 * r] = w1;                                                        \
        wb[i2 + 2 * r] = w2;                                                        \
      }                                                                             \
      if (jj == 0) {                           \
        wb[GRP_IDX(kb, 6 * dd)] = rb[B][0];                                         \
        wb[GRP_IDX(kb + 1, 6 * dd)] = rb[B][1];                                     \
        wb[GRP_IDX(kb + 2, 6 * dd)] = rb[B][2];                                     \
      }                                                                             \
    }                                                                               \
    const int nks = (3 * nlc + 3) >> 2;                                             \
    if (nlc < nlw) {  \
      for (int e = lane; e < (4 * nks - 3 * nlc) * TW; e += 64) {                   \
        const int k_ = 3 * nlc + e / TW, c_ = e - (e / TW) * TW;                    \
        va[GRP_IDX(k_, c_)] = 0.0;                                                  \
        wb[GRP_IDX(k_, c_)] = 0.0;                                                  \
      }                                                                             \
    }                                                                               \
    GRP_STAMP()                                                                     \
    if (ch + 8 < nch) GRP_PREFETCH(B, ch + 8)                                       \
    GRP_STAMP()                                                                     \
    __builtin_amdgcn_fence(__ATOMIC_RELEASE, "wavefront");                          \
    __builtin_amdgcn_wave_barrier();                                                \
    __builtin_amdgcn_fence(__ATOMIC_ACQUIRE, "wavefront");                          \
    {                                                                               \
       \
      const double *ap = va + (lk >> 1) * RS + lr * 2 + (lk & 1);                   \
      const double *bp = wb + (lk >> 1) * RS + lr * 2 + (lk & 1);                   \
      double a[NT], b[NT], an[NT], bn[NT];                                          \
      _Pragma("unroll") for (int t = 0; t < NT; ++t) {                              \
        a[t] = ap[32 * t];                                                          \
        b[t] = bp[32 * t];                                                          \
      }                                                                             \
      for (int ks = 0; ks < nks; ++ks) {                                            \
        const int kn = ks + 1 < nks ? ks + 1 : ks;  \
        _Pragma("unroll") for (int t = 0; t < NT; ++t) {                            \
          an[t] = ap[kn * 2 * RS + 32 * t];                                         \
          bn[t] = bp[kn * 2 * RS + 32 * t];                                         \
        }                                                                           \
        int tile = 0;                                                               \
        _Pragma("unroll") for (int ti = 0; ti < NT; ++ti)                           \
        _Pragma("unroll") for (int tj = ti; tj < NT; ++tj) {                        \
          acc[tile] = __builtin_amdgcn_mfma_f64_16x16x4f64(a[ti], b[tj], acc[tile], 0, 0, 0); \
          ++tile;                                                                   \
        }                                                                           \
        _Pragma("unroll") for (int t = 0; t < NT; ++t) {                            \
          a[t] = an[t];                                                             \
          b[t] = bn[t];                                                             \
        }                                                                           \
      }                                                                             \
    }                                                                               \
    __builtin_amdgcn_fence(__ATOMIC_RELEASE, "wavefront");                          \
    __builtin_amdgcn_wave_barrier();                                                \
    __builtin_amdgcn_fence(__ATOMIC_ACQUIRE, "wavefront");                          \
    GRP_STAMP()                                                                     \
    ch += 4;                                                                        \
  }
  for (int ch = wv; ch < nch;) {
    GRP_STAGE(0)
    GRP_STAGE(1)
  }
#undef GRP_STAGE
#undef GRP_IDX
#undef GRP_PREFETCH
  GRP_STAMP()
#ifdef BA_GRP_DBG
  if (gdbg_on) for (int q = 0; q < 256; ++q) g_grp_dbg[q] = q < gdbg_n ? gdbg_s[q] : 0;
#endif
  __syncthreads();
  double *R = &VA[0][0];
  int tile = 0;
#pragma unroll
  for (int ti = 0; ti < NT; ++ti)
#pragma unroll
    for (int tj = ti; tj < NT; ++tj) {
#pragma unroll
      for (int g = 0; g < 4; ++g) R[wv * 256 + g * 64 + lane] = acc[tile][g];
      __syncthreads();
      {
        const double v = ((R[tid] + R[256 + tid]) + R[512 + tid]) + R[768 + tid];
        const int g = tid >> 6, ln = tid & 63;
        const int row = 16 * ti + (ln >> 4) + 4 * g;
        const int col = 16 * tj + (ln & 15);
        const int pj = row / 6, r = row - 6 * pj;
        if (pj < dd) {
          const int sj = gd.s0 + pj * dd - (pj * (pj - 1)) / 2;
          if (col == 6 * dd) {
            d.spart2[(size_t)sj * kSlotStride + 36 + r] = v;
          } else if (col < 6 * dd) {
            const int pk = col / 6, c = col - 6 * pk;
            if (pk >= pj) d.spart2[(size_t)(sj + (pk - pj)) * kSlotStride + r * 6 + c] = v;
          }
        }
      }
      __syncthreads();
      ++tile;
    }
}

#define GW_LDS_BARRIER() asm volatile("s_waitcnt lgkmcnt(0)\n\ts_barrier" ::: "memory")
__global__ __launch_bounds__(kBlock, 2) void k_schur_grp_wide(DevProblem d, const DevProblem::GrpDesc *grps) {
  constexpr int TW = 128;
  constexpr int LPW = 2;
  constexpr int KRW = 4 * LPW * 3;
  constexpr int RS = 2 * TW + 6;
  constexpr int IMG = (KRW / 2) * RS;
  __shared__ __attribute__((aligned(16))) double VA[IMG];
  __shared__ __attribute__((aligned(16))) double WB[IMG];
#ifdef BA_GRP_DBG
  __shared__ long long gdbg_s[256];
  #ifndef BA_GRP_DBG_TID
#define BA_GRP_DBG_TID 0
#endif
  const bool gdbg_on = blockIdx.x == 100 && threadIdx.x == BA_GRP_DBG_TID;
  int gdbg_n = 0;
#endif
  GRP_STAMP()
  const int tid = threadIdx.x, lane = tid & 63, wv = tid >> 6;
  const int lr = lane & 15, lk = lane >> 4;
  const DevProblem::GrpDesc *gp = grps + blockIdx.x;
  const int64_t gp0 = gp->p0;
  const int gl0 = gp->l0, gnl = gp->nl, dd = gp->d, gs0 = gp->s0;
  const int done = d.ctrl->done;
  const int lb = d.ctrl->lcur;
  if (done) return;
  const double *__restrict__ Wg = d.W[lb];
  const double *__restrict__ bg = d.b[lb];
  const double *__restrict__ Cug = d.Cu[lb];
  const double lp1 = 1.0 + d.ctrl->lambda;
  const int nlw = min(64 / dd, LPW);
  const int il = lane / dd, jj = lane - il * dd;
  const int li = wv * nlw + il;
  const int per_stage = 4 * nlw;
  const int nst = (gnl + per_stage - 1) / per_stage;
  for (int e = tid; e < IMG; e += kBlock) {
    VA[e] = 0.0;
    WB[e] = 0.0;
  }
  double2 rw[1][6], rc[1][3];
  double rb[1][3];
#define GW_PREFETCH(B, st_)                                                         \
  {                                                                                 \
    const int c0_ = (st_) * per_stage;                                              \
    const bool on_ = il < nlw && c0_ + li < gnl;                                     \
    const double2 *wp_ = (const double2 *)(Wg + (size_t)(gp0 + (int64_t)(c0_ + wv * nlw) * dd + (on_ ? lane : 0)) * kWStride); \
    const int lm_ = gl0 + (on_ ? c0_ + li : 0);                                     \
    const double2 *cp_ = (const double2 *)(Cug + (size_t)lm_ * 6);                  \
    if (!on_) wp_ = (const double2 *)(Wg + (size_t)gp0 * kWStride);                 \
    _Pragma("unroll") for (int k_ = 0; k_ < 6; ++k_) rw[B][k_] = wp_[k_];           \
    _Pragma("unroll") for (int k_ = 0; k_ < 3; ++k_) rc[B][k_] = cp_[k_];           \
    _Pragma("unroll") for (int k_ = 0; k_ < 3; ++k_) rb[B][k_] = bg[(size_t)lm_ * 3 + k_]; \
  }
  v4f64 acc[9];
#pragma unroll
  for (int t = 0; t < 9; ++t) acc[t] = (v4f64){0.0, 0.0, 0.0, 0.0};
  const int n_first = 8 - wv;
  GW_PREFETCH(0, 0)
#define GW_IDX(k_, col_) (((k_) >> 1) * RS + (col_) * 2 + ((k_) & 1))
#define GW_STAGE(B)                                                                 \
  {                                                                                 \
    const int c0 = st * per_stage;                                                  \
    const int nlc = min(per_stage, gnl - c0);                                       \
               \
    _Pragma("unroll") for (int k_ = 0; k_ < 6; ++k_) asm volatile("" : "+v"(rw[B][k_].x), "+v"(rw[B][k_].y)); \
    _Pragma("unroll") for (int k_ = 0; k_ < 3; ++k_) asm volatile("" : "+v"(rc[B][k_].x), "+v"(rc[B][k_].y), "+v"(rb[B][k_])); \
    if (il < nlw && li < nlc) {                                                     \
      _Pragma("clang fp contract(fast)")                                            \
      const double k9[9] = {rw[B][0].x, rw[B][0].y, rw[B][1].x, rw[B][1].y, rw[B][2].x, \
                            rw[B][2].y, rw[B][3].x, rw[B][3].y, rw[B][4].x};        \
      const double x0 = rw[B][4].y, x1 = rw[B][5].x, x2 = rw[B][5].y;               \
      const double cd_[6] = {rc[B][0].x * lp1, rc[B][0].y, rc[B][1].x, rc[B][1].y * lp1, rc[B][2].x, rc[B][2].y * lp1}; \
      double c6[6];                                                                 \
      spd3_inverse(cd_, c6);                                                        \
      double w[18];                                                                 \
      _Pragma("unroll") for (int e = 0; e < 9; ++e) w[e] = k9[e];                   \
      _Pragma("unroll") for (int c = 0; c < 3; ++c) {                               \
        w[9 + c] = x1 * k9[6 + c] - x2 * k9[3 + c];                                 \
        w[12 + c] = x2 * k9[c] - x0 * k9[6 + c];                                    \
        w[15 + c] = x0 * k9[3 + c] - x1 * k9[c];                                    \
      }                                                                             \
      const int kb = 3 * li, cb = 6 * jj;                                           \
      const int i0 = GW_IDX(kb, cb), i1 = GW_IDX(kb + 1, cb), i2 = GW_IDX(kb + 2, cb); \
      _Pragma("unroll") for (int r = 0; r < 6; ++r) {                               \
        const double w0 = w[r * 3], w1 = w[r * 3 + 1], w2 = w[r * 3 + 2];           \
        VA[i0 + 2 * r] = w0 * c6[0] + w1 * c6[1] + w2 * c6[2];                      \
        VA[i1 + 2 * r] = w0 * c6[1] + w1 * c6[3] + w2 * c6[4];                      \
        VA[i2 + 2 * r] = w0 * c6[2] + w1 * c6[4] + w2 * c6[5];                      \
        WB[i0 + 2 * r] = w0;                                                        \
        WB[i1 + 2 * r] = w1;                                                        \
        WB[i2 + 2 * r] = w2;                                                        \
      }                                                                             \
      if (jj == 0) {                                                                \
        WB[GW_IDX(kb, 6 * dd)] = rb[B][0];                                          \
        WB[GW_IDX(kb + 1, 6 * dd)] = rb[B][1];                                      \
        WB[GW_IDX(kb + 2, 6 * dd)] = rb[B][2];                                      \
      }                                                                             \
    }                                                                               \
    GRP_STAMP()                                                                     \
    const int nks = (3 * nlc + 3) >> 2;                                             \
    if (nlc < per_stage) {  \
      for (int e = tid; e < (4 * nks - 3 * nlc) * TW; e += kBlock) {                \
        const int k_ = 3 * nlc + e / TW, c_ = e - (e / TW) * TW;                    \
        VA[GW_IDX(k_, c_)] = 0.0;                                                   \
        WB[GW_IDX(k_, c_)] = 0.0;                                                   \
      }                                                                             \
    }                                                                               \
        \
    GW_PREFETCH(B, min(st + 1, nst - 1))                                            \
    GRP_STAMP()                                                                     \
    asm volatile("s_waitcnt lgkmcnt(0)" ::: "memory");                              \
    GRP_STAMP()                                                                     \
    GW_LDS_BARRIER();                                                                \
    GRP_STAMP()                                                                     \
    {                                                                               \
      const double *ap = VA + (lk >> 1) * RS + lr * 2 + (lk & 1);                   \
      const double *bp = WB + (lk >> 1) * RS + lr * 2 + (lk & 1);                   \
      for (int ks = 0; ks < nks; ++ks) {                                            \
        const double a0 = ap[ks * 2 * RS + 32 * wv], a1 = ap[ks * 2 * RS + 32 * (7 - wv)]; \
        _Pragma("unroll") for (int t = 0; t < 9; ++t) {                             \
          const bool first = t < n_first;                                           \
          const int tj = first ? wv + t : 7 - wv + (t - n_first);                   \
          const double bv = bp[ks * 2 * RS + 32 * tj];                              \
          acc[t] = __builtin_amdgcn_mfma_f64_16x16x4f64(first ? a0 : a1, bv, acc[t], 0, 0, 0); \
        }                                                                           \
      }                                                                             \
    }                                                                               \
    GRP_STAMP()                                                                     \
    GW_LDS_BARRIER();                                                                \
    GRP_STAMP()                                                                     \
    ++st;                                                                           \
  }
  GW_LDS_BARRIER();
  for (int st = 0; st < nst;) {
    GW_STAGE(0)
  }
#undef GW_STAGE
#undef GW_IDX
#undef GW_PREFETCH
  GRP_STAMP()
#pragma unroll
  for (int t = 0; t < 9; ++t) {
    const bool first = t < n_first;
    const int ti = first ? wv : 7 - wv;
    const int tj = first ? wv + t : 7 - wv + (t - n_first);
#pragma unroll
    for (int g = 0; g < 4; ++g) {
      const double v = acc[t][g];
      const int row = 16 * ti + lk + 4 * g;
      const int col = 16 * tj + lr;
      const int pj = row / 6, r = row - 6 * pj;
      if (pj < dd) {
        const int sj = gs0 + pj * dd - (pj * (pj - 1)) / 2;
        if (col == 6 * dd) {
          d.spart2[(size_t)sj * kSlotStride + 36 + r] = v;
        } else if (col < 6 * dd) {
          const int pk = col / 6, c = col - 6 * pk;
          if (pk >= pj) d.spart2[(size_t)(sj + (pk - pj)) * kSlotStride + r * 6 + c] = v;
        }
      }
    }
  }
  GRP_STAMP()
#ifdef BA_GRP_DBG
  if (gdbg_on) for (int q = 0; q < 256; ++q) g_grp_dbg[q] = q < gdbg_n ? gdbg_s[q] : 0;
#endif
}

__global__ __launch_bounds__(64) void k_schur_partial(DevProblem d) {
  if (d.ctrl->done) return;
  const double *__restrict__ Wg = d.W[d.ctrl->lcur];
  const double *__restrict__ bg = d.b[d.ctrl->lcur];
  const int ch = blockIdx.x;
  double acc[36], racc[6];
#pragma unroll
  for (int k = 0; k < 36; ++k) acc[k] = 0.0;
#pragma unroll
  for (int k = 0; k < 6; ++k) racc[k] = 0.0;
  const int64_t e = d.tchunk_end[ch];
  for (int64_t t = d.tchunk_begin[ch] + threadIdx.x; t < e; t += 64) {
    const int64_t p = d.tri_p[t];
    const bool dg = p == d.tri_q[t];
    double Wp[18];
    expand_W(Wg + (size_t)p * kWStride, Wp);
    const double *ci = d.Cinv + (size_t)d.pair_lm[p] * 6;
    const double *bi = bg + (size_t)d.pair_lm[p] * 3;
    const double b0 = dg ? bi[0] : 0.0, b1 = dg ? bi[1] : 0.0, b2 = dg ? bi[2] : 0.0;
    double v[18], w[18];
#pragma unroll
    for (int r = 0; r < 6; ++r) {
      const double w0 = Wp[r * 3 + 0], w1 = Wp[r * 3 + 1], w2 = Wp[r * 3 + 2];
      v[r * 3 + 0] = w0 * ci[0] + w1 * ci[1] + w2 * ci[2];
      v[r * 3 + 1] = w0 * ci[1] + w1 * ci[3] + w2 * ci[4];
      v[r * 3 + 2] = w0 * ci[2] + w1 * ci[4] + w2 * ci[5];
      racc[r] += v[r * 3 + 0] * b0 + v[r * 3 + 1] * b1 + v[r * 3 + 2] * b2;
    }
    expand_W(Wg + (size_t)d.tri_q[t] * kWStride, w);
#pragma unroll
    for (int r = 0; r < 6; ++r)
#pragma unroll
      for (int c = 0; c < 6; ++c)
        acc[r * 6 + c] += v[r * 3 + 0] * w[c * 3 + 0] +
                          v[r * 3 + 1] * w[c * 3 + 1] +
                          v[r * 3 + 2] * w[c * 3 + 2];
  }
#pragma unroll
  for (int k = 0; k < 36; ++k) {
    const double tot = wave_sum(acc[k]);
    if (threadIdx.x == 0) d.spart[(size_t)ch * kSlotStride + k] = tot;
  }
#pragma unroll
  for (int k = 0; k < 6; ++k) {
    const double tot = wave_sum(racc[k]);
    if (threadIdx.x == 0) d.spart[(size_t)ch * kSlotStride + 36 + k] = tot;
  }
}

template <bool DIRECT>
__device__ __forceinline__ void schur_final_body(const DevProblem &d, int64_t blk,
                                                 double (*part)[42]) {
  const int q = threadIdx.x / 42, e = threadIdx.x - q * 42;
  const int4 *bq = (const int4 *)(d.blk_desc + 16 * (size_t)blk);
  const int4 b0 = bq[0], b1 = bq[1], b2 = bq[2], b3 = bq[3];
  const int done = d.ctrl->done;
  if (done) return;
  const int j = b0.x, k = b0.y;
  double pre = 0.0;
  int pcj = 0, pck = 0;
  if (threadIdx.x < 42 && (e < 36 || j == k)) {
    const int lb = d.ctrl->lcur;
    if (e >= 36) pre = d.a[lb][(size_t)j * 6 + (e - 36)];
    else if (j == k) {
      pre = d.A[lb][(size_t)j * 36 + e];
      if (e % 7 == 0) pre *= (1.0 + d.ctrl->lambda);
    }
    pcj = d.pose_col[j];
    pck = d.pose_col[k];
  }
  if (q < 6 && (e < 36 || j == k)) {
    double s = 0.0;
    const int nc = b0.w;
    if (q < nc) {
      const int sl = q == 0 ? b2.x : q == 1 ? b2.y : q == 2 ? b2.z : q == 3 ? b2.w : q == 4 ? b3.x : b3.y;
      s += d.spart2[(size_t)sl * kSlotStride + e];
    }
    if (q + 6 < nc) {
      const int sl = q == 0 ? b3.z : q == 1 ? b3.w : d.contrib_slot[(size_t)b0.z + q + 6];
      s += d.spart2[(size_t)sl * kSlotStride + e];
    }
    for (int ci = q + 12; ci < nc; ci += 6)
      s += d.spart2[(size_t)d.contrib_slot[(size_t)b0.z + ci] * kSlotStride + e];
    const int ch1 = b1.x + b1.y;
    for (int ch = b1.x + q; ch < ch1; ch += 6)
      s += d.spart[(size_t)ch * kSlotStride + e];
// ... 103 lines not shown
__device__ __forceinline__ void pose_update_body(const DevProblem &d, const int bid, double *sm) {
  const int cur = d.ctrl->cur;
  const int lbp = d.ctrl->lcur;
  const double lp1p = 1.0 + d.ctrl->lambda;
  if (bid == 0 && threadIdx.x == 0) {
    d.ctrl->tcur = cur ^ 1;
    d.ctrl->tlcur = lbp ^ 1;
  }
  const double *__restrict__ Tc = d.poses[cur];
  double *__restrict__ Tt = d.poses[cur ^ 1];
  double est = 0.0, nrm = 0.0;
  for (int j = bid * kBlock + threadIdx.x; j < d.N; j += kPoseGrid * kBlock) {
    const double *xj = d.x + (size_t)j * 6;
    const double v0 = xj[0], v1 = xj[1], v2 = xj[2];
    const double w0 = xj[3], w1 = xj[4], w2 = xj[5];
    double dR[9], dt[3];
    se3_exp(v0, v1, v2, w0, w1, w2, dR, dt);
    const double *T = Tc + (size_t)j * 12;
    double *To = Tt + (size_t)j * 12;
#pragma unroll
    for (int r = 0; r < 3; ++r) {
#pragma unroll
      for (int c = 0; c < 3; ++c)
        To[r * 3 + c] = dR[r * 3 + 0] * T[0 * 3 + c] + dR[r * 3 + 1] * T[1 * 3 + c] + dR[r * 3 + 2] * T[2 * 3 + c];
      To[9 + r] = dR[r * 3 + 0] * T[9] + dR[r * 3 + 1] * T[10] + dR[r * 3 + 2] * T[11] + dt[r];
    }
    const double *aj = d.a[lbp] + (size_t)j * 6;
    const double *Aj = d.A[lbp] + (size_t)j * 36;
    double e = 0.0;
#pragma unroll
    for (int r = 0; r < 6; ++r) e += aj[r] * xj[r];
    double q = 0.0;
#pragma unroll
    for (int c = 0; c < 6; ++c) {
      double rowc = 0.0;
#pragma unroll
      for (int r = 0; r < 6; ++r)
        rowc += xj[r] * (r == c ? Aj[r * 6 + c] * lp1p : Aj[r * 6 + c]);
      q += rowc * xj[c];
    }
    est += e + q;
    nrm += sqrt(v0 * v0 + v1 * v1 + v2 * v2 + w0 * w0 + w1 * w1 + w2 * w2);
  }
  const double t0 = block_sum(est, sm);
  const double t1 = block_sum(nrm, sm);
  if (threadIdx.x == 0) {
    d.pose_part[2 + 2 * bid + 0] = t0;
    d.pose_part[2 + 2 * bid + 1] = t1;
  }
}

#define BACKSUB_ISSUE(t0_, np_)                                                 \
  {                                                                             \
    const double2 *src_ = (const double2 *)(Wg + (size_t)(t0_) * kWStride);     \
    _Pragma("unroll") for (int k_ = 0; k_ < kBsRW; ++k_) {                      \
      const int t_ = tid + k_ * kBlock;                                         \
      rw[k_] = (t_ < (np_) * 6) ? src_[t_] : make_double2(0.0, 0.0);            \
    }                                                                           \
    _Pragma("unroll") for (int k_ = 0; k_ < kBsRX; ++k_) {                      \
      const int t_ = tid + k_ * kBlock;                                         \
      rpj[k_] = (t_ < (np_) * 3) ? d.pair_pose[(t0_) + t_ / 3] : 0;             \
    }                                                                           \
  }
#define BACKSUB_GATHER(np_)                                                     \
  {                                                                             \
    _Pragma("unroll") for (int q_ = 0; q_ < kBsRX; ++q_) {                      \
      const int t_ = tid + q_ * kBlock;                                         \
      const int c_ = t_ - (t_ / 3) * 3;                                         \
      rx[q_] = (t_ < (np_) * 3)                                                 \
                   ? *(const double2 *)(d.x + (size_t)rpj[q_] * 6 + 2 * c_)     \
                   : make_double2(0.0, 0.0);                                    \
    }                                                                           \
  }
constexpr int kBsRW = (kSchurPairs * (kWStride / 2) + kBlock - 1) / kBlock;
constexpr int kBsRX = (kSchurPairs * 3 + kBlock - 1) / kBlock;

#ifdef BA_BS_DBG
__device__ long long g_bs_dbg[96];
#define BS_STAMP() { if (bs_on && bs_n < 96) bs_s[bs_n++] = clock64(); }
#else
#define BS_STAMP()
#endif
constexpr int kBgLm = 16;
constexpr int kBgArea = 64 * kWStride + 64 * 3 + 64 * 12 + 64 * 3;
constexpr int kBsLds = (kSchurPairs * (kWStride + 6 + 3) > 4 * kBgArea) ? kSchurPairs * (kWStride + 6 + 3) : 4 * kBgArea;

__device__ __forceinline__ void backsub_chunk_body(const DevProblem &d, const int bx, const int part, double *lds,
                                                   double *sm, int *recs) {
  double *Ws = lds;
  double *Xs = Ws + kSchurPairs * kWStride;
  double *Us = Xs + kSchurPairs * 6;
  const int tid = threadIdx.x;
#ifdef BA_BS_DBG
  __shared__ long long bs_s[96];
  const bool bs_on = bx == 2000 && threadIdx.x == 0;
  int bs_n = 0;
#endif
  BS_STAMP()
  const int c0 = d.lin_chunk0 + bx * kBsChunks;
  const int nk = min(kBsChunks, d.n_bchunk - c0);
  const DevProblem::LmChunk lc0 = d.lm_chunk[c0];
  if (tid < nk * 8) recs[tid] = ((const int *)d.lm_chunk)[(size_t)c0 * 8 + tid];
  const int done = d.ctrl->done;
  const int cur = d.ctrl->cur;
  const int lbs = d.ctrl->lcur;
  const double lp1 = 1.0 + d.ctrl->lambda;
  BA_KEEP_S((int)lc0.pb);
  BA_KEEP_S(lc0.np);
  BA_KEEP_S(done);
  if (done) return;
  const double *__restrict__ Xc = d.pts[cur];
  double *__restrict__ Xt = d.pts[cur ^ 1];
  const double *__restrict__ Wg = d.W[lbs];
  const double *__restrict__ bg = d.b[lbs];
  const double *__restrict__ Cg = d.Cu[lbs];
  double2 rw[kBsRW];
  int rpj[kBsRX];
  int64_t r_pb = lc0.pb;
  int r_l0 = lc0.l0, r_nl = lc0.nl, r_np = lc0.np;
  double2 rx[kBsRX];
  {
    const int np0 = r_np < kSchurPairs ? r_np : kSchurPairs;
    BACKSUB_ISSUE(r_pb, np0)
    BACKSUB_GATHER(np0)
  }
  __syncthreads();
  BS_STAMP()
  double est_acc = 0.0, nrm_acc = 0.0;
  for (int k = 0; k < nk; ++k) {
    const int64_t pb = r_pb, pe = r_pb + r_np;
    const int l0 = r_l0, nl = r_nl;
    const int i = l0 + tid;
    const bool own = tid < nl;
    int64_t q0 = 0, q1 = 0;
    double ci[6], Xi[3], bi[3], C[6];
#pragma unroll
    for (int e = 0; e < 6; ++e) ci[e] = C[e] = 0.0;
#pragma unroll
    for (int e = 0; e < 3; ++e) Xi[e] = bi[e] = 0.0;
    if (own) {
      q0 = d.lm_pair_ptr[i];
      q1 = d.lm_pair_ptr[i + 1];
#pragma unroll
      for (int e = 0; e < 3; ++e) Xi[e] = Xc[(size_t)i * 3 + e];
#pragma unroll
      for (int e = 0; e < 3; ++e) bi[e] = bg[(size_t)i * 3 + e];
#pragma unroll
      for (int e = 0; e < 6; ++e) C[e] = Cg[(size_t)i * 6 + e];
    }
    BS_STAMP()
    double bx0 = 0, bx1 = 0, bx2 = 0;
    int64_t t0 = pb;
    int np = (int)min((int64_t)kSchurPairs, pe - t0);
    for (;;) {
      {
        double2 *dst = (double2 *)Ws;
#pragma unroll
        for (int q = 0; q < kBsRW; ++q) {
          const int t = tid + q * kBlock;
          if (t < np * 6) dst[t] = rw[q];
        }
        double2 *xd = (double2 *)Xs;
#pragma unroll
        for (int q = 0; q < kBsRX; ++q) {
          const int t = tid + q * kBlock;
          if (t < np * 3) xd[t] = rx[q];
        }
      }
      BS_STAMP()
      const bool last_tile = t0 + kSchurPairs >= pe;
      if (last_tile && k + 1 < nk) {
        const int *rr = recs + (k + 1) * 8;
        r_pb = uni64(*(const int64_t *)rr);
        r_l0 = __builtin_amdgcn_readfirstlane(rr[4]);
        r_nl = __builtin_amdgcn_readfirstlane(rr[5]);
        r_np = __builtin_amdgcn_readfirstlane(rr[6]);
        const int npn = r_np < kSchurPairs ? r_np : kSchurPairs;
        BACKSUB_ISSUE(r_pb, npn)
      }
      BS_STAMP()
      __syncthreads();
      BS_STAMP()
      for (int t = tid; t < np * 3; t += kBlock) {
        const int lp = t / 3, c = t - lp * 3;
        const double *xj = Xs + lp * 6;
        const double *w = Ws + lp * kWStride;
        const double X0 = w[9], X1 = w[10], X2 = w[11];
        const double e0 = xj[0] + (xj[4] * X2 - xj[5] * X1);
        const double e1 = xj[1] + (xj[5] * X0 - xj[3] * X2);
        const double e2 = xj[2] + (xj[3] * X1 - xj[4] * X0);
        Us[t] = fma(w[6 + c], e2, fma(w[3 + c], e1, w[c] * e0));
      }
      BS_STAMP()
      __syncthreads();
      BS_STAMP()
      if (own) {
// ... 2 lines not shown
          const double *u = Us + (p - t0) * 3;
          bx0 += u[0];
          bx1 += u[1];
          bx2 += u[2];
        }
      }
      BS_STAMP()
      if (last_tile) break;
      t0 += kSchurPairs;
      np = (int)min((int64_t)kSchurPairs, pe - t0);
      __syncthreads();
      BACKSUB_ISSUE(t0, np)
      BACKSUB_GATHER(np)
    }
    if (k + 1 < nk) {
      const int npn = r_np < kSchurPairs ? r_np : kSchurPairs;
      BACKSUB_GATHER(npn)
    }
    double est = 0.0, nrm = 0.0;
    if (own) {
      {
        const double cdm[6] = {C[0] * lp1, C[1], C[2], C[3] * lp1, C[4], C[5] * lp1};
        ldlt3_inverse(cdm, ci);
      }
      const double cb0 = ci[0] * bi[0] + ci[1] * bi[1] + ci[2] * bi[2];
      const double cb1 = ci[1] * bi[0] + ci[3] * bi[1] + ci[4] * bi[2];
      const double cb2 = ci[2] * bi[0] + ci[4] * bi[1] + ci[5] * bi[2];
      const double y0 = cb0 - (ci[0] * bx0 + ci[1] * bx1 + ci[2] * bx2);
      const double y1 = cb1 - (ci[1] * bx0 + ci[3] * bx1 + ci[4] * bx2);
      const double y2 = cb2 - (ci[2] * bx0 + ci[4] * bx1 + ci[5] * bx2);
      double *yo = d.y + (size_t)i * 3;
      yo[0] = y0; yo[1] = y1; yo[2] = y2;
      double *Xo = Xt + (size_t)i * 3;
      Xo[0] = Xi[0] + y0;
      Xo[1] = Xi[1] + y1;
      Xo[2] = Xi[2] + y2;
      const double C0 = C[0] * lp1, C3 = C[3] * lp1, C5 = C[5] * lp1;
      double e = bi[0] * y0 + bi[1] * y1 + bi[2] * y2;
      const double r0 = y0 * C0 + y1 * C[1] + y2 * C[2];
      const double r1 = y0 * C[1] + y1 * C3 + y2 * C[4];
      const double r2 = y0 * C[2] + y1 * C[4] + y2 * C5;
      e += r0 * y0 + r1 * y1 + r2 * y2;
      e += 2.0 * (y0 * bx0 + y1 * bx1 + y2 * bx2);
      est = e;
      nrm = sqrt(y0 * y0 + y1 * y1 + y2 * y2);
    }
    BS_STAMP()
    est_acc += est;
    nrm_acc += nrm;
  }
  block_sum2(est_acc, nrm_acc, sm);
  if (tid == 0) {
    d.lm_part[2 * part + 0] = est_acc;
    d.lm_part[2 * part + 1] = nrm_acc;
  }
  BS_STAMP()
#ifdef BA_BS_DBG
  if (bs_on) for (int q = 0; q < 96; ++q) g_bs_dbg[q] = q < bs_n ? bs_s[q] : 0;
#endif
}

__device__ __forceinline__ void backsub_grp_body(const DevProblem &d, const int piece, const int part, double *lds,
                                                 double *sm) {
  const DevProblem::LinDesc *gp = d.lin_desc + piece;
  const int64_t p0 = gp->p0;
  const int l0 = gp->l0, nl = gp->nl, dd = gp->d;
  const int done = d.ctrl->done;
  const int cur = d.ctrl->cur;
  const int lbs = d.ctrl->lcur;
  const double lp1 = 1.0 + d.ctrl->lambda;
  const int tid = threadIdx.x, lane = tid & 63, wv = tid >> 6;
  const int ddv = dd > 0 ? dd : 1;
  const int nlwb = 64 / ddv < kBgLm ? 64 / ddv : kBgLm;
  const int ilw = lane / ddv, jj = lane - ilw * ddv;
  const bool lane_on = dd > 0 && ilw < nlwb;
  const int pose = dd > 0 ? d.pair_pose[p0 + jj] : 0;
  if (done) return;
  double xj[6];
  {
    const double2 *xp = (const double2 *)(d.x + (size_t)pose * 6);
    const double2 a0 = xp[0], a1 = xp[1], a2 = xp[2];
    xj[0] = a0.x; xj[1] = a0.y; xj[2] = a1.x; xj[3] = a1.y; xj[4] = a2.x; xj[5] = a2.y;
  }
  double *__restrict__ Xt = d.pts[cur ^ 1];
  const double2 *__restrict__ Wg2 = (const double2 *)d.W[lbs];
  double *Wim = lds + wv * kBgArea;
  double *Us = Wim + 64 * kWStride;
  double *Lm = Us + 64 * 3;
  double *Bx = Lm + 64 * 12;
  const int S = 64 / nlwb;
  const int per_step = 4 * nlwb;
  const int nstep = (nl + per_step - 1) / per_step;
  auto il0_of = [&](int st) { return (st * 4 + wv) * nlwb; };
  const double *lm_p[3];
  int lm_l[3], lm_e[3], lm_m[3], lm_q[3];
#pragma unroll
  for (int k = 0; k < 3; ++k) {
    const int q = min(lane + 64 * k, nlwb * 12 - 1);
    const int nc = nlwb * 6, nb = nlwb * 9;
    const int a = q < nc ? 0 : (q < nb ? 1 : 2);
    const int r = q - (a == 0 ? 0 : (a == 1 ? nc : nb));
    lm_m[k] = a == 0 ? 6 : 3;
    lm_l[k] = r / lm_m[k];
    lm_e[k] = r - lm_l[k] * lm_m[k];
    lm_p[k] = (a == 0 ? d.Cu[lbs] : (a == 1 ? d.b[lbs] : d.pts[cur])) + (size_t)l0 * lm_m[k] + lm_e[k];
    lm_q[k] = q;
  }
  double2 rwA0, rwA1, rwA2, rwA3, rwA4, rwA5, rwB0, rwB1, rwB2, rwB3, rwB4, rwB5;
  double lmA0, lmA1, lmA2, lmB0, lmB1, lmB2;
#define BSG_ISSUE(R, L, ST)                                                         \
  {                                                                                 \
    const int il0_ = il0_of(ST);                                                    \
    const int nls_ = max(0, min(nlwb, nl - il0_));                                  \
    const int last_ = max(0, nls_ * dd * 6 - 1);                                    \
    const int ilb_ = nls_ > 0 ? il0_ : 0;                                           \
    const int lml_ = max(0, nls_ - 1);                                              \
    const double2 *src_ = Wg2 + (dd > 0 ? (size_t)(p0 + (int64_t)ilb_ * dd) * 6 : (size_t)0); \
    R##0 = src_[min(lane, last_)];                                                  \
    R##1 = src_[min(lane + 64, last_)];                                             \
    R##2 = src_[min(lane + 128, last_)];                                            \
    R##3 = src_[min(lane + 192, last_)];                                            \
    R##4 = src_[min(lane + 256, last_)];                                            \
    R##5 = src_[min(lane + 320, last_)];                                            \
    L##0 = lm_p[0][(size_t)(ilb_ + min(lm_l[0], lml_)) * lm_m[0]];                  \
    L##1 = lm_p[1][(size_t)(ilb_ + min(lm_l[1], lml_)) * lm_m[1]];                  \
    L##2 = lm_p[2][(size_t)(ilb_ + min(lm_l[2], lml_)) * lm_m[2]];                  \
  }
#define BSG_WAVE_SYNC()                                                             \
  {                                                                                 \
    __builtin_amdgcn_fence(__ATOMIC_RELEASE, "wavefront");                          \
    __builtin_amdgcn_wave_barrier();                                                \
    __builtin_amdgcn_fence(__ATOMIC_ACQUIRE, "wavefront");                          \
  }
  double est_acc = 0.0, nrm_acc = 0.0;
  double *dump = d.lin_dump + (size_t)((blockIdx.x & 63) * 4 + wv) * 4;
  int sb = 0, st_b0 = 0;
  const int ls_ = lane / nlwb, lli = lane - ls_ * nlwb;
  const int sli = lane / 3, slc = lane - sli * 3;
#define BSG_STEP(R, L, TAG)                                                         \
  {                                                                                 \
                                  \
    asm volatile("; k_backsub_update group step " TAG);                             \
                                   \
    ((double2 *)Wim)[lane] = R##0;                                                  \
    ((double2 *)Wim)[lane + 64] = R##1;                                             \
    ((double2 *)Wim)[lane + 128] = R##2;                                            \
    ((double2 *)Wim)[lane + 192] = R##3;                                            \
    ((double2 *)Wim)[lane + 256] = R##4;                                            \
    ((double2 *)Wim)[lane + 320] = R##5;                                            \
    Lm[sb * nlwb * 12 + lm_q[0]] = L##0;                                            \
    Lm[sb * nlwb * 12 + lm_q[1]] = L##1;                                            \
    Lm[sb * nlwb * 12 + lm_q[2]] = L##2;                                            \
    BSG_ISSUE(R, L, st + 2)                                                         \
    BSG_WAVE_SYNC()                                                                 \
    if (lane_on) {                                                                  \
                   \
      const double2 *w2 = (const double2 *)(Wim + lane * kWStride);                 \
      const double2 k01 = w2[0], k23 = w2[1], k45 = w2[2], k67 = w2[3], k8x = w2[4], xx = w2[5]; \
      const double X0 = k8x.y, X1 = xx.x, X2 = xx.y;                                \
      const double e0 = xj[0] + (xj[4] * X2 - xj[5] * X1);                          \
      const double e1 = xj[1] + (xj[5] * X0 - xj[3] * X2);                          \
      const double e2 = xj[2] + (xj[3] * X1 - xj[4] * X0);                          \
      double *u = Us + lane * 3;                                                    \
      u[0] = fma(k67.x, e2, fma(k23.y, e1, k01.x * e0));                            \
      u[1] = fma(k67.y, e2, fma(k45.x, e1, k01.y * e0));                            \
      u[2] = fma(k8x.x, e2, fma(k45.y, e1, k23.x * e0));                            \
    }                                                                               \
    BSG_WAVE_SYNC()                                                                 \
         \
    if (lane < nlwb * 3) {                                                          \
      const double *u = Us + sli * dd * 3 + slc;                                    \
      double bx_ = 0.0;                                                             \
      for (int q_ = 0; q_ < dd; ++q_) bx_ += u[q_ * 3];                             \
      Bx[(sb * nlwb + sli) * 3 + slc] = bx_;                                        \
    }                                                                               \
    BSG_WAVE_SYNC()                                                                 \
     \
     \
     \
     \
    const bool do_lm_ = (sb + 1 == S) || (st + 1 >= nstep);                         \
    double y0 = 0.0, y1 = 0.0, y2 = 0.0, xn0 = 0.0, xn1 = 0.0, xn2 = 0.0;           \
    bool lm_on_ = false;                                                            \
    size_t i_ = 0;                                                                  \
    if (do_lm_) {                                                                   \
      const int il_ = il0_of(st_b0 + ls_) + lli;                                    \
      lm_on_ = ls_ <= sb && il_ < nl;                                               \
      i_ = (size_t)l0 + il_;                                                        \
      const double *lmp = Lm + ls_ * nlwb * 12;                                     \
      double C[6], bi[3], Xi[3];                                                    \
      _Pragma("unroll") for (int e_ = 0; e_ < 6; ++e_) C[e_] = lmp[lli * 6 + e_];   \
      _Pragma("unroll") for (int e_ = 0; e_ < 3; ++e_) bi[e_] = lmp[nlwb * 6 + lli * 3 + e_]; \
      _Pragma("unroll") for (int e_ = 0; e_ < 3; ++e_) Xi[e_] = lmp[nlwb * 9 + lli * 3 + e_]; \
      const double bx0 = Bx[lane * 3], bx1 = Bx[lane * 3 + 1], bx2 = Bx[lane * 3 + 2]; \
      double ci[6];                                                                 \
      {                                                                             \
        const double cdm[6] = {C[0] * lp1, C[1], C[2], C[3] * lp1, C[4], C[5] * lp1}; \
        spd3_inverse(cdm, ci);                                                      \
      }                                                                             \
      const double cb0 = ci[0] * bi[0] + ci[1] * bi[1] + ci[2] * bi[2];             \
      const double cb1 = ci[1] * bi[0] + ci[3] * bi[1] + ci[4] * bi[2];             \
      const double cb2 = ci[2] * bi[0] + ci[4] * bi[1] + ci[5] * bi[2];             \
      y0 = cb0 - (ci[0] * bx0 + ci[1] * bx1 + ci[2] * bx2);                         \
      y1 = cb1 - (ci[1] * bx0 + ci[3] * bx1 + ci[4] * bx2);                         \
      y2 = cb2 - (ci[2] * bx0 + ci[4] * bx1 + ci[5] * bx2);                         \
      xn0 = Xi[0] + y0;                                                             \
      xn1 = Xi[1] + y1;                                                             \
      xn2 = Xi[2] + y2;                                                             \
            \
      const double C0 = C[0] * lp1, C3 = C[3] * lp1, C5 = C[5] * lp1;               \
      double e = bi[0] * y0 + bi[1] * y1 + bi[2] * y2;                              \
      const double r0 = y0 * C0 + y1 * C[1] + y2 * C[2];                            \
      const double r1 = y0 * C[1] + y1 * C3 + y2 * C[4];                            \
      const double r2 = y0 * C[2] + y1 * C[4] + y2 * C5;                            \
      e += r0 * y0 + r1 * y1 + r2 * y2;                                             \
      e += 2.0 * (y0 * bx0 + y1 * bx1 + y2 * bx2);                                  \
      est_acc += lm_on_ ? e : 0.0;                                                  \
      nrm_acc += lm_on_ ? sqrt(y0 * y0 + y1 * y1 + y2 * y2) : 0.0;                  \
    }                                                                               \
    {                                                                               \
      double *yo = lm_on_ ? d.y + i_ * 3 : dump;                                    \
      yo[0] = y0; yo[1] = y1; yo[2] = y2;                                           \
      double *Xo = lm_on_ ? Xt + i_ * 3 : dump;                                     \
      Xo[0] = xn0; Xo[1] = xn1; Xo[2] = xn2;                                        \
    }                                                                               \
    if (do_lm_) {                                                                   \
      sb = 0;                                                                       \
      st_b0 = st + 1;                                                               \
    } else {                                                                        \
      ++sb;                                                                         \
    }                                                                               \
    BSG_WAVE_SYNC()                                                                 \
  }
  BSG_ISSUE(rwA, lmA, 0)
  BSG_ISSUE(rwB, lmB, 1)
  int st = 0;
  while (st < nstep) {
    BSG_STEP(rwA, lmA, "A")
    if (++st >= nstep) break;
    BSG_STEP(rwB, lmB, "B")
    ++st;
  }
// ... 474 lines not shown
  ctl->iter += 1;
  ctl->converged = conv ? 1 : 0;
  if (conv || ctl->iter >= ctl->max_iter) ctl->done = 1;
}

inline int cdiv(int64_t a, int64_t b) { return (int)((a + b - 1) / b); }

}

void launch_cost(const DevProblem &d, int sel, int64_t begin, hipStream_t s) {
  if (begin >= d.n_obs) return;
  const bool lds = d.n_cam <= kCamLds, slim = d.obs_cp != nullptr;
  if (lds && slim) {
    BA_LAUNCH(K_COST, (k_cost<true, true>), dim3(kCostGrid), dim3(kBlock), s, d, sel, begin);
  } else if (lds) {
    BA_LAUNCH(K_COST, (k_cost<true, false>), dim3(kCostGrid), dim3(kBlock), s, d, sel, begin);
  } else if (slim) {
    BA_LAUNCH(K_COST, (k_cost<false, true>), dim3(kCostGrid), dim3(kBlock), s, d, sel, begin);
  } else {
    BA_LAUNCH(K_COST, (k_cost<false, false>), dim3(kCostGrid), dim3(kBlock), s, d, sel, begin);
  }
}

void launch_lin_landmarks(const DevProblem &d, int sel, hipStream_t s) {
  if (d.lin_chunk0 > 0) {
    const int n_plain = d.n_lin_plain, n_mask = d.n_lin_desc - d.n_lin_plain;
    if (d.n_cam <= kCamLds) {
      if (n_plain > 0) BA_LAUNCH(K_LIN_GRP, (k_lin_grp<true, false>), dim3(n_plain), dim3(kBlock), s, d, sel, 0);
      if (n_mask > 0) BA_LAUNCH(K_LIN_GRP, (k_lin_grp<true, true>), dim3(n_mask), dim3(kBlock), s, d, sel, n_plain);
    } else {
      if (n_plain > 0) BA_LAUNCH(K_LIN_GRP, (k_lin_grp<false, false>), dim3(n_plain), dim3(kBlock), s, d, sel, 0);
      if (n_mask > 0) BA_LAUNCH(K_LIN_GRP, (k_lin_grp<false, true>), dim3(n_mask), dim3(kBlock), s, d, sel, n_plain);
    }
  }
  const int nch = d.n_bchunk - d.lin_chunk0;
  if (nch <= 0) return;
  if (d.n_cam <= kCamLds)
    BA_LAUNCH(K_LIN_LANDMARKS, k_lin_landmarks<true>, dim3(nch), dim3(kBlock), s, d, sel);
  else
    BA_LAUNCH(K_LIN_LANDMARKS, k_lin_landmarks<false>, dim3(nch), dim3(kBlock), s, d, sel);
}

void launch_lin_poses(const DevProblem &d, int sel, hipStream_t s) {
  if (d.n_achunk > 0) {
    if (d.n_cam <= kCamLds)
      BA_LAUNCH(K_LIN_POSES, k_lin_poses<true>, dim3(cdiv(d.n_achunk, kBlock / 64)), dim3(kBlock), s, d, sel);
    else
      BA_LAUNCH(K_LIN_POSES, k_lin_poses<false>, dim3(cdiv(d.n_achunk, kBlock / 64)), dim3(kBlock), s, d, sel);
  }
  if (d.N > 0)
    BA_LAUNCH(K_POSE_FINALIZE, k_pose_finalize, dim3(cdiv((int64_t)d.N * 27, kBlock)), dim3(kBlock), s, d, sel);
}

void launch_damp_invert(const DevProblem &d, hipStream_t s) {
  if (d.M > 0 && (d.n_sup > 0 || d.n_tchunk > 0))
    BA_LAUNCH(K_DAMP_INVERT, k_damp_invert, dim3(cdiv(d.M, kBlock)), dim3(kBlock), s, d, 0);
}
void launch_damp_invert_export(const DevProblem &d, hipStream_t s) {
  if (d.M > 0)
    hipLaunchKernelGGL(k_damp_invert, dim3(cdiv(d.M, kBlock)), dim3(kBlock), 0, s, d, 1);
}

#ifdef BA_LL_DBG
extern "C" int ba_debug_read_ll(long long *out) {
  return (int)hipMemcpyFromSymbol(out, HIP_SYMBOL(g_ll_dbg), sizeof(long long) * 32);
}
#endif
#ifdef BA_LG_DBG
extern "C" int ba_debug_read_lg(long long *out) {
  return (int)hipMemcpyFromSymbol(out, HIP_SYMBOL(g_lg_dbg), sizeof(long long) * 64);
}
#endif
#ifdef BA_GRP_DBG
extern "C" int ba_debug_read_grp(long long *out) {
  return (int)hipMemcpyFromSymbol(out, HIP_SYMBOL(g_grp_dbg), sizeof(long long) * 256);
}
#endif
#ifdef BA_SCHUR_DBG
extern "C" int ba_debug_read(long long *out) {
  return (int)hipMemcpyFromSymbol(out, HIP_SYMBOL(g_schur_dbg), sizeof(long long) * 4 * 160);
}
#endif
void launch_schur_accumulate(const DevProblem &d, hipStream_t s) {
  if (d.n_grp32 > 0)
    BA_LAUNCH(K_SCHUR_GRP, k_schur_grp<2>, dim3(d.n_grp32), dim3(kBlock), s, d, d.grp32);
  if (d.n_grp64 > 0)
    BA_LAUNCH(K_SCHUR_GRP, k_schur_grp<4>, dim3(d.n_grp64), dim3(kBlock), s, d, d.grp64);
  if (d.n_grp128 > 0)
    BA_LAUNCH(K_SCHUR_GRP, k_schur_grp_wide, dim3(d.n_grp128), dim3(kBlock), s, d, d.grp128);
  if (d.n_sup > 0)
    BA_LAUNCH(K_SCHUR_LDS, k_schur_lds, dim3(d.n_sup), dim3(kBlock), s, d);
  if (d.n_tchunk > 0)
    BA_LAUNCH(K_SCHUR_PARTIAL, k_schur_partial, dim3(d.n_tchunk), dim3(64), s, d);
}

void launch_schur_final(const DevProblem &d, bool direct, hipStream_t s) {
  if (d.B <= 0) return;
  if (direct)
    BA_LAUNCH(K_SCHUR_FINAL, k_schur_final_direct, dim3((unsigned)d.B), dim3(kBlock), s, d);
  else
    BA_LAUNCH(K_SCHUR_FINAL, k_schur_final, dim3((unsigned)d.B), dim3(kBlock), s, d);
}

void launch_schur(const DevProblem &d, bool direct, bool with_init, hipStream_t s) {
  if (with_init)
    launch_dense_init(d.L, d.ld, d.col_x, d.zt_I, d.zt_J, d.n_zt, d.nb, &d.ctrl->done, s);
  launch_schur_accumulate(d, s);
  launch_schur_final(d, direct, s);
}

void launch_scatter(const DevProblem &d, hipStream_t s) {
  const int64_t n = d.B * 36 + 6 * (int64_t)d.N;
  if (n > 0)
    BA_LAUNCH(K_SCATTER, k_scatter, dim3(cdiv(n, kBlock)), dim3(kBlock), s, d);
}

void launch_backsub_update(const DevProblem &d, hipStream_t s, bool zero_tiles) {
  const dim3 grid(kPoseGrid + d.n_lm_part + (zero_tiles ? d.n_zt : 0));
  if (d.n_bs_grp > 0)
    BA_LAUNCH(K_BACKSUB_UPDATE, k_backsub_update<true>, grid, dim3(kBlock), s, d);
  else
    BA_LAUNCH(K_BACKSUB_UPDATE, k_backsub_update<false>, grid, dim3(kBlock), s, d);
}

void launch_scalars(const DevProblem &d, int cost_src, hipStream_t s) {
  BA_LAUNCH(K_SCALARS, k_scalars, dim3(1), dim3(kScalBlock), s, d, 1, cost_src, -1);
}

void launch_scalars_and_control(const DevProblem &d, int cost_src, hipStream_t s, int finalize_sel) {
  const int nfin = finalize_sel >= 0 ? cdiv((int64_t)d.N * 27, kScalBlock) : 0;
  BA_LAUNCH(K_SCALARS, k_scalars, dim3(1 + nfin), dim3(kScalBlock), s, d, 2, cost_src, finalize_sel);
}

void launch_control(const DevProblem &d, hipStream_t s) {
  BA_LAUNCH(K_CONTROL, k_control, dim3(1), dim3(64), s, d);
}

void launch_init_ctrl_cost(const DevProblem &d, hipStream_t s) {
  BA_LAUNCH(K_CONTROL, k_init_ctrl_cost, dim3(1), dim3(64), s, d);
}

void launch_scalars_cost_only(const DevProblem &d, int cost_src, hipStream_t s) {
  BA_LAUNCH(K_SCALARS, k_scalars, dim3(1), dim3(kScalBlock), s, d, 0, cost_src, -1);
}

void launch_gd_pass(const DevProblem &d, const GdDev &g, hipStream_t s) {
  const bool lds = d.n_cam <= kCamLds;
  const int nb = d.n_bchunk + g.n_fix_blk;
  if (nb > 0) {
    if (lds)
      hipLaunchKernelGGL(k_gd_points<true>, dim3(nb), dim3(kBlock), 0, s, d, g);
    else
      hipLaunchKernelGGL(k_gd_points<false>, dim3(nb), dim3(kBlock), 0, s, d, g);
  }
  if (g.n_chunk > 0) {
    const dim3 grid(cdiv(g.n_chunk, kBlock / 64));
    if (lds)
      hipLaunchKernelGGL(k_gd_poses<true>, grid, dim3(kBlock), 0, s, d, g);
    else
      hipLaunchKernelGGL(k_gd_poses<false>, grid, dim3(kBlock), 0, s, d, g);
  }
}

void launch_gd_control(const DevProblem &d, const GdDev &g, int mode, hipStream_t s) {
  hipLaunchKernelGGL(k_gd_control, dim3(1 + cdiv((int64_t)d.N * 6, kGdCtrlBlock)), dim3(kGdCtrlBlock), 0, s, d, g,
                     mode);
}

void launch_gd_update(const DevProblem &d, const GdDev &g, hipStream_t s) {
  if (g.n_upd_blk > 0) hipLaunchKernelGGL(k_gd_update, dim3(g.n_upd_blk), dim3(kBlock), 0, s, d, g);
}

// ... 2 lines not shown
```

### include/ba_hip.h

```cpp
#ifndef BA_HIP_H_
#define BA_HIP_H_

#include <stdint.h>

#ifdef __cplusplus
extern "C" {
#endif

typedef struct ba_handle ba_handle;

typedef struct {
  float threshold_step_size;
  float threshold_cost_change;
  float threshold_huber_loss;
  float threshold_outlier_rejection;
  int max_num_iterations;
  float initial_lambda;
  float decrease_ratio_lambda;
  float increase_ratio_lambda;
  int gauss_newton;
} ba_options;

typedef struct {
  double cost;
// ... 25 lines not shown
                        const int32_t *pose, const int32_t *point,
                        const double *uv2);
int ba_set_shard(ba_handle *h, int rank, int world);
int ba_finalize(ba_handle *h);

int ba_update_values(ba_handle *h, const double *T_jw12, const double *X3);

int ba_partition_points(int n_pose, const uint8_t *pose_fixed, int n_pt,
                        const uint8_t *pt_fixed, int64_t n_obs,
                        const int32_t *obs_pose, const int32_t *obs_pt,
                        int world, int32_t *owner_out);

typedef int (*ba_allreduce_fn)(void *user, int which, void *dev_ptr,
                               int64_t n_doubles, void *hip_stream);
int ba_set_allreduce(ba_handle *h, ba_allreduce_fn fn, void *user);
int64_t ba_reduce_buffer_size(ba_handle *h, int which);
int ba_bind_reduce_buffer(ba_handle *h, int which, void *dev_ptr,
                          int64_t n_doubles);

int ba_gather_points(ba_handle *h);

typedef struct ba_rccl_comm ba_rccl_comm;
int ba_rccl_available(void);
int ba_rccl_get_unique_id(uint8_t id128[128]);
int ba_rccl_comm_create(ba_rccl_comm **out, int rank, int world,
                        const uint8_t id128[128], int device_id);
int ba_rccl_comm_size(ba_rccl_comm *c);
int64_t ba_rccl_comm_calls(ba_rccl_comm *c);
void ba_rccl_comm_destroy(ba_rccl_comm *c);
int ba_rccl_allreduce_hook(void *user, int which, void *dev_ptr,
                           int64_t n_doubles, void *hip_stream);

int ba_solve(ba_handle *h, const ba_options *opt, ba_iter_info *out, int cap,
             int *n_iter, int *converged);
int ba_lm_begin(ba_handle *h, const ba_options *opt);
int ba_lm_iterate(ba_handle *h, int n);
int ba_lm_sync(ba_handle *h, ba_iter_info *out, int cap, int *n_iter,
               int *converged);

int ba_gd_begin(ba_handle *h, const ba_options *opt);
int ba_gd_iterate(ba_handle *h, int n);
int ba_gd_sync(ba_handle *h, ba_iter_info *out, int cap, int *n_iter,
               int *converged);
int ba_solve_gd(ba_handle *h, const ba_options *opt, ba_iter_info *out,
                int cap, int *n_iter, int *converged);
int ba_gd_get_gradient(ba_handle *h, double *a6, double *b3);

int ba_stage_cost(ba_handle *h, double *cost);
int ba_stage_linearize(ba_handle *h, double lambda,
                       double huber);
int ba_stage_schur(ba_handle *h);
int ba_stage_solve_reduced(ba_handle *h);
int ba_stage_backsub_update(ba_handle *h);
int ba_stage_scalars(ba_handle *h, double *trial_cost, double *model_change,
                     double *pose_step_sum, double *point_step_sum);
int ba_stage_commit(ba_handle *h, int accept);

int ba_enable_stage_timing(ba_handle *h, int on);
int ba_get_stage_ms(ba_handle *h, double out8[8], int reset);

int ba_num_opt_poses(ba_handle *h);
int ba_num_opt_points(ba_handle *h);
int64_t ba_num_pairs(ba_handle *h);
int64_t ba_num_schur_blocks(ba_handle *h);
int64_t ba_num_schur_triples(ba_handle *h);
int ba_get_poses(ba_handle *h, double *T_jw12 );
int ba_get_points(ba_handle *h, double *X3 , uint8_t *owned_mask);
int ba_get_A(ba_handle *h, double *A36, double *a6);
int ba_get_C(ba_handle *h, double *C9, double *b3);
int ba_get_Cinv(ba_handle *h, double *Cinv9, double *Cinvb3);
int ba_get_pairs(ba_handle *h, int32_t *pair_i, int32_t *pair_j, double *W18);
int ba_get_S(ba_handle *h, double *S, double *rhs);
int ba_get_xy(ba_handle *h, double *x6, double *y3);

int ba_kernel_count(void);
const char *ba_kernel_name(int id);
int ba_get_kernel_ms(ba_handle *h, double *ms_out, int64_t *calls_out, int reset);

int ba_get_dense_info(ba_handle *h, double out4[4]);

int ba_get_schur_info(ba_handle *h, int64_t out8[8]);

int ba_get_lin_info(ba_handle *h, int64_t out4[4]);

int ba_get_mask_info(ba_handle *h, int64_t out4[4]);

int ba_get_dropped_pivots(ba_handle *h, int64_t *count, int reset);

typedef struct ba_stream ba_stream;
int ba_stream_create(ba_stream **out, int device_id, int n_chunks, int64_t arena_bytes);
void ba_stream_destroy(ba_stream *s);
int ba_stream_set_cameras(ba_stream *s, int n_cam, const double *intr4, const double *T_cj12);
int ba_stream_set_poses(ba_stream *s, int n_pose, const double *T_jw12, const uint8_t *fixed);
int ba_stream_set_points(ba_stream *s, int n_pt, const double *X3, const uint8_t *fixed);
int ba_stream_set_observations(ba_stream *s, int64_t n_obs, const int32_t *cam, const int32_t *pose,
                               const int32_t *point, const double *uv2);
int ba_stream_finalize(ba_stream *s);
int ba_stream_solve(ba_stream *s, const ba_options *opt, ba_iter_info *out, int cap,
                    int *n_iter, int *converged);
int ba_stream_lm_begin(ba_stream *s, const ba_options *opt);
int ba_stream_lm_iterate(ba_stream *s, int n);
int ba_stream_lm_sync(ba_stream *s, ba_iter_info *out, int cap, int *n_iter, int *converged);
int ba_stream_get_poses(ba_stream *s, double *T_jw12);
int ba_stream_get_points(ba_stream *s, double *X3);
int ba_stream_info(ba_stream *s, int64_t out6[6]);

int ba_dense_spd_solve(ba_handle *h, int n, const double *A, const double *b,
                       double *x, double *ms);

typedef struct {
  float cost, cost_change, abs_step;
} ba_po_iter;
int ba_pose_only_mono6(ba_handle *h, const float *X3, const float *uv2, int n,
                       float fx, float fy, float cx, float cy, float *T12,
                       uint8_t *mask, const ba_options *opt, ba_po_iter *iters,
                       int cap, int *n_iter, int *converged,
                       float *debug_T12);

int ba_pose_only_stereo6(ba_handle *h, const float *X3, const float *uvl2,
                         const float *uvr2, int n, const float *intr_l4,
                         const float *intr_r4, const float *T_lr12, float *T12,
                         uint8_t *mask_l, uint8_t *mask_r, const ba_options *opt,
                         ba_po_iter *iters, int cap, int *n_iter, int *converged,
                         float *debug_T12);

int ba_pose_only_mono3(ba_handle *h, const float *X3, const float *uv2, int n,
                       float fx, float fy, float cx, float cy,
                       const float *T_bc12, const float *T_wl12, float *T12,
                       uint8_t *mask, const ba_options *opt, ba_po_iter *iters,
                       int cap, int *n_iter, int *converged,
                       float *debug_T12);
int ba_pose_only_stereo3(ba_handle *h, const float *X3, const float *uvl2,
                         const float *uvr2, int n, const float *intr_l4,
                         const float *intr_r4, const float *T_bc12,
                         const float *T_lr12, const float *T_wl12, float *T12,
                         uint8_t *mask_l, uint8_t *mask_r, const ba_options *opt,
                         ba_po_iter *iters, int cap, int *n_iter, int *converged,
                         float *debug_T12);

typedef struct {
  int n_iter, converged, n_rows, status;
} ba_po_result;
int ba_pose_only_mono6_batch(ba_handle *h, int B, const int32_t *offsets,
                             const float *X3, const float *uv2,
                             const float *intr4, float *T12, uint8_t *mask,
                             const ba_options *opt, ba_po_iter *iters, int cap,
                             ba_po_result *res, float *debug_T12);
int ba_pose_only_stereo6_batch(ba_handle *h, int B, const int32_t *offsets,
                               const float *X3, const float *uvl2,
                               const float *uvr2, const float *intr_l4,
                               const float *intr_r4, const float *T_lr12,
                               float *T12, uint8_t *mask_l, uint8_t *mask_r,
                               const ba_options *opt, ba_po_iter *iters,
                               int cap, ba_po_result *res, float *debug_T12);
int ba_pose_only_mono6_batch_device(ba_handle *h, int B, const int32_t *offsets,
                                    const float *X3, const float *uv2,
                                    const float *intr4, float *T12,
                                    uint8_t *mask, const ba_options *opt,
                                    ba_po_iter *iters, int cap,
                                    ba_po_result *res, float *debug_T12,
                                    void *hip_stream);
int ba_pose_only_stereo6_batch_device(ba_handle *h, int B,
                                      const int32_t *offsets, const float *X3,
                                      const float *uvl2, const float *uvr2,
                                      const float *intr_l4, const float *camr16,
                                      float *T12, uint8_t *mask_l,
// ... 45 lines not shown
```

Baseline: 2272 it/s.

## Store grouped W blocks in slim 9-double layout and recompute Xij on the fly

For grouped pairs, the per-pair W record shrinks from 12 doubles to 9: 8 are stored interleaved and the ninth in a separate array. The camera-frame point Xij is no longer stored; consumers (schur group kernels, grouped backsub) recompute it from the current pose and point. The goal is to cut the bandwidth of W writes in linearisation and W reads in the Schur and backsub kernels. The cost is extra pose and point loads plus a small matrix-vector product per pair, and W readback now fails if parameters have moved since the last linearisation.

```diff
diff --git a/bundle_adjustment_solver_amd/_lib.py b/bundle_adjustment_solver_amd/_lib.py
--- a/bundle_adjustment_solver_amd/_lib.py
+++ b/bundle_adjustment_solver_amd/_lib.py
@@ -153,6 +153,7 @@
     "ba_get_dense_info": (C.c_int, [_P, _D]),
     "ba_get_schur_info": (C.c_int, [_P, C.POINTER(C.c_int64)]),
     "ba_get_lin_info": (C.c_int, [_P, C.POINTER(C.c_int64)]),
+    "ba_get_w_info": (C.c_int, [_P, C.POINTER(C.c_int64)]),
     "ba_get_mask_info": (C.c_int, [_P, C.POINTER(C.c_int64)]),
     "ba_get_dropped_pivots": (C.c_int, [_P, C.POINTER(C.c_int64), C.c_int]),
     "ba_dense_spd_solve": (C.c_int, [_P, C.c_int, _D, _D, _D, _D]),
diff --git a/bundle_adjustment_solver_amd/csrc/ba_api.hip b/bundle_adjustment_solver_amd/csrc/ba_api.hip
--- a/bundle_adjustment_solver_amd/csrc/ba_api.hip
+++ b/bundle_adjustment_solver_amd/csrc/ba_api.hip
@@ -527,14 +527,21 @@
   }
 
   lap("structure uploads");
+  const ba::WLayout wl = ba::w_layout(pl.P, pl.lin_groups ? pl.lm_pair_ptr[pl.M_grp] : 0);
+  d.Pg = wl.Pg;
+  const size_t w_doubles = std::max<size_t>(2, (size_t)wl.doubles);
+  h->w_stale = false;
+  h->w_alloc = (int64_t)w_doubles;
   for (int k = 0; k < 2; ++k) {
     h->kind(2);
     if (h->dalloc(&d.Cu[k], (size_t)pl.M * 6) || h->dalloc(&d.b[k], (size_t)pl.M * 3) ||
-        h->dalloc(&d.W[k], std::max<size_t>(2, (size_t)pl.P * ba::kWStride)))
+        h->dalloc(&d.W[k], w_doubles))
       return -1;
+    d.Wc[k] = d.W[k] + wl.chunk_bias;
     h->kind(0);
     if (h->dalloc(&d.A[k], (size_t)pl.N * 36) || h->dalloc(&d.a[k], (size_t)pl.N * 6)) return -1;
-    HIP_TRY(hipMemset(d.W[k], 0, std::max<size_t>(1, (size_t)pl.P * ba::kWStride) * sizeof(double)));
+    HIP_TRY(hipMemset(d.W[k], 0, w_doubles * sizeof(double)));
+    h->w_zeroed = (int64_t)w_doubles;
     HIP_TRY(hipMemset(d.A[k], 0, std::max<size_t>(1, (size_t)pl.N * 36) * sizeof(double)));
     HIP_TRY(hipMemset(d.a[k], 0, std::max<size_t>(1, (size_t)pl.N * 6) * sizeof(double)));
   }
@@ -679,6 +686,7 @@
   }
   h->gathered_valid = false;
   h->lm_begun = false;
+  h->w_stale = true;
   h->gd_begun = false;
   h->tiles_ready = false;
   return 0;
@@ -771,6 +779,7 @@
   }
   HIP_TRY(hipGetLastError());
   h->lm_begun = true;
+  h->w_stale = false;
   return 0;
 }
 
@@ -1030,6 +1039,7 @@
   if (push_ctrl(h)) return -1;
   join_side(h);
   enqueue_linearize(h, 0);
+  h->w_stale = false;
   ba::launch_damp_invert(h->d, h->stream);
   HIP_TRY(hipStreamSynchronize(h->stream));
   HIP_TRY(hipGetLastError());
@@ -1089,7 +1099,10 @@
   if (use_device(h)) return -1;
   h->gathered_valid = false;
   if (pull_ctrl(h)) return -1;
-  if (accept) h->hc.cur ^= 1;
+  if (accept) {
+    h->hc.cur ^= 1;
+    h->w_stale = true;
+  }
   if (push_ctrl(h)) return -1;
   HIP_TRY(hipStreamSynchronize(h->stream));
   return 0;
@@ -1268,14 +1281,34 @@
     }
   }
   if (W18) {
+    if (h->d.Pg > 0 && h->w_stale)
+      return fail("ba_get_pairs: the parameters have moved since the blocks were linearised "
+                  "(ba_update_values / ba_stage_commit): linearise again first");
     if (pull_ctrl(h)) return -1;
-    std::vector<double> w12((size_t)pl.P * ba::kWStride);
+    const ba::WLayout wl = ba::w_layout(pl.P, h->d.Pg);
+    std::vector<double> wall((size_t)std::max<int64_t>(wl.doubles, 1)), Tall, Xall;
     if (pl.P > 0)
-      HIP_TRY(hipMemcpy(w12.data(), h->d.W[h->hc.lcur], w12.size() * sizeof(double), hipMemcpyDeviceToHost));
+      HIP_TRY(hipMemcpy(wall.data(), h->d.W[h->hc.lcur], (size_t)wl.doubles * sizeof(double), hipMemcpyDeviceToHost));
+    if (wl.Pg > 0) {
+      Tall.resize((size_t)pl.n_pose * 12);
+      Xall.resize((size_t)pl.n_pt * 3);
+      HIP_TRY(hipMemcpy(Tall.data(), h->d.poses[h->hc.cur], Tall.size() * sizeof(double), hipMemcpyDeviceToHost));
+      HIP_TRY(hipMemcpy(Xall.data(), h->d.pts[h->hc.cur], Xall.size() * sizeof(double), hipMemcpyDeviceToHost));
+    }
+    const double *wc = wall.data() + wl.chunk_bias;
     int64_t o = 0;
     for (int64_t p = 0; p < pl.P; ++p) {
       if (padded(p)) continue;
-      const double *k = &w12[(size_t)p * ba::kWStride];
+      double k12[12];
+      if (p < wl.Pg) {
+        for (int e = 0; e < 8; ++e) k12[e] = wall[(size_t)p * 8 + e];
+        k12[8] = wall[(size_t)wl.Pg * 8 + p];
+        const double *X = &Xall[(size_t)pl.pair_lm[p] * 3];
+        ba::pose_point(&Tall[(size_t)pl.pair_pose[p] * 12], X[0], X[1], X[2], k12 + 9);
+      } else {
+        for (int e = 0; e < 12; ++e) k12[e] = wc[(size_t)p * ba::kWStride + e];
+      }
+      const double *k = k12;
       double *W = W18 + (size_t)o * 18;
       for (int e = 0; e < 9; ++e) W[e] = k[e];
       for (int c = 0; c < 3; ++c) {
@@ -1382,6 +1415,15 @@
   out8[5] = triples;
   out8[6] = mfma;
   out8[7] = (int64_t)pl.tri_p.size();
+  return 0;
+}
+
+int ba_get_w_info(ba_handle *h, int64_t out4[4]) {
+  if (!h || !h->finalized || !out4) return fail("ba_get_w_info: bad argument");
+  out4[0] = h->w_alloc;
+  out4[1] = h->d.Pg;
+  out4[2] = h->w_zeroed;
+  out4[3] = h->plan.P;
   return 0;
 }
 
diff --git a/bundle_adjustment_solver_amd/csrc/ba_device.h b/bundle_adjustment_solver_amd/csrc/ba_device.h
--- a/bundle_adjustment_solver_amd/csrc/ba_device.h
+++ b/bundle_adjustment_solver_amd/csrc/ba_device.h
@@ -3,6 +3,7 @@
 
 #include <hip/hip_runtime.h>
 #include <stdint.h>
+#include <math.h>
 #include <stdlib.h>
 
 #include <vector>
@@ -37,6 +38,25 @@
 };
 
 constexpr int kWStride = 12;
+constexpr int kWSlim = 9;
+struct WLayout {
+  int64_t Pg, pad, chunk_bias, doubles;
+};
+inline WLayout w_layout(int64_t P, int64_t Pg) {
+  WLayout l;
+  l.Pg = Pg;
+  l.pad = Pg & 1;
+  l.chunk_bias = (int64_t)kWSlim * Pg + l.pad - (int64_t)kWStride * Pg;
+  l.doubles = (int64_t)kWSlim * Pg + l.pad + (int64_t)kWStride * (P - Pg);
+  return l;
+}
+
+__host__ __device__ __forceinline__ void pose_point(const double *__restrict__ T, const double X0,
+                                                    const double X1, const double X2, double Xij[3]) {
+#pragma unroll
+  for (int r = 0; r < 3; ++r)
+    Xij[r] = fma(T[r * 3 + 2], X2, fma(T[r * 3 + 0], X0, T[r * 3 + 1] * X1)) + T[9 + r];
+}
 
 struct DevProblem {
   int n_cam, n_pose, N, n_pt, M, M_global;
@@ -109,6 +129,8 @@
   double *Cu[2];
   double *b[2];
   double *W[2];
+  double *Wc[2];
+  int64_t Pg;
   double *A[2];
   double *a[2];
   double *Cinv;
diff --git a/bundle_adjustment_solver_amd/csrc/ba_handle.h b/bundle_adjustment_solver_amd/csrc/ba_handle.h
--- a/bundle_adjustment_solver_amd/csrc/ba_handle.h
+++ b/bundle_adjustment_solver_amd/csrc/ba_handle.h
@@ -75,6 +75,8 @@
   bool ev_ok = false;
   double stage_ms[ST_N] = {0, 0, 0, 0, 0, 0, 0, 0};
   bool lm_begun = false;
+  int64_t w_alloc = 0, w_zeroed = 0;
+  bool w_stale = false;
   ba::KernelTimer kt;
   ba::DenseSchedule sched;
   ba::DenseDev ddev;
diff --git a/bundle_adjustment_solver_amd/csrc/ba_kernels.hip b/bundle_adjustment_solver_amd/csrc/ba_kernels.hip
--- a/bundle_adjustment_solver_amd/csrc/ba_kernels.hip
+++ b/bundle_adjustment_solver_amd/csrc/ba_kernels.hip
@@ -124,10 +124,7 @@
                                         const double X2, const double u,
                                         const double v, ObsGeom &g) {
 #pragma clang fp contract(fast)
-#pragma unroll
-  for (int r = 0; r < 3; ++r)
-    g.Xij[r] = (T[r * 3 + 0] * X0 + T[r * 3 + 1] * X1 + T[r * 3 + 2] * X2) +
-               T[9 + r];
+  pose_point(T, X0, X1, X2, g.Xij);
   const double *Rc = cam + 4;
   const double *tc = cam + 13;
 #pragma unroll
@@ -445,7 +442,7 @@
   LL_STAMP()
   const double *__restrict__ poses = d.poses[buf];
   const double *__restrict__ pts = d.pts[buf];
-  double *__restrict__ Wg = d.W[lb];
+  double *__restrict__ Wg = d.Wc[lb];
   double cost_acc = 0.0;
   if (tid <= lc.nl) lq[tid] = (tid < lc.nl) ? (int)(q0 - ob) : lc.no;
   constexpr int kSumIt = (kSchurLandmarks * 9 + kBlock - 1) / kBlock;
@@ -660,21 +657,28 @@
   double2 *dumpW = (double2 *)(d.lin_dump + (size_t)((bid & 63) * 4 + wv) * 4);
   double *dumpC = (double *)dumpW + 2;
   double2 *stgW = (double2 *)(cbw + 64 * 9);
-  double2 *stgW_mine = stgW + (ilw * dd + jj) * 6;
-  constexpr int kLgPass = (7 * 10 * 6 + 63) / 64;
+  double *stgW8 = cbw + 64 * 9 + 64 * 8;
+  const int rec_mine = min(ilw * dd + jj, 63);
+  double2 *stgW_mine = stgW + rec_mine * 4;
+  constexpr int kLgPass = 4;
   int il0p = nl;
   double vv[8];
   double2 wvv[kLgPass];
-  int lastp = 0;
+  double wv8;
+  int lastp = 0, lastp8 = 0;
   double2 *dstWp = dumpW;
+  double *dstWp8 = dumpC + 1;
 #define LING_FLUSH_ISSUE()                                                          \
   {                                                                                 \
     _Pragma("unroll") for (int u_ = 0; u_ < 8; ++u_) vv[u_] = sum_p[(u_ < no ? u_ : 0) * 9]; \
     const int nls_ = nl - il0p < nlw ? nl - il0p : nlw;                             \
-    const int n2_ = nls_ * dd * 6;                                                  \
-    dstWp = n2_ > 0 ? (double2 *)(Wg + (size_t)(p0 + (int64_t)il0p * dd) * kWStride) : dumpW; \
+    const int n1_ = nls_ * dd, n2_ = n1_ * 4;                                       \
+    dstWp = n2_ > 0 ? (double2 *)(Wg + (size_t)(p0 + (int64_t)il0p * dd) * 8) : dumpW; \
+    dstWp8 = n2_ > 0 ? Wg + (size_t)d.Pg * 8 + (size_t)(p0 + (int64_t)il0p * dd) : dumpC + 1; \
     lastp = n2_ > 0 ? n2_ - 1 : 0;                                                  \
+    lastp8 = n2_ > 0 ? n1_ - 1 : 0;                                                 \
     _Pragma("unroll") for (int k_ = 0; k_ < kLgPass; ++k_) wvv[k_] = stgW[min(lane + 64 * k_, lastp)]; \
+    wv8 = stgW8[min(lane, lastp8)];                                                 \
   }
 #define LING_FLUSH_FINISH()                                                         \
   {                                                                                 \
@@ -685,6 +689,7 @@
     double *dst_ = (sum_on && ils_ < nl) ? sum_g + (size_t)ils_ * sum_stride : dumpC; \
     *dst_ = sum_neg ? -sacc_ : sacc_;                                               \
     _Pragma("unroll") for (int k_ = 0; k_ < kLgPass; ++k_) dstWp[min(lane + 64 * k_, lastp)] = wvv[k_]; \
+    dstWp8[min(lane, lastp8)] = wv8;                                                \
   }
 #define LING_STEP(CUR, NXT2)                                                        \
   {                                                                                 \
@@ -715,7 +720,7 @@
       g.r1 = valid_ ? g.r1 : 0.0;                                                   \
     }                                                                               \
     cost_acc += valid_ ? sqrt(g.r0 * g.r0 + g.r1 * g.r1) : 0.0;                     \
-    double w, G[6], Rm[6], Q[12], cbv[9], kk[12];                                   \
+    double w, G[6], Rm[6], Q[12], cbv[9], kk[9];                                    \
     weight_and_G(cam, g, huber, w, G);                                              \
     w = valid_ ? w : 0.0;                                                           \
     make_R(G, T, Rm);                                                               \
@@ -737,7 +742,6 @@
       _Pragma("unroll") for (int r = 0; r < 3; ++r)                                 \
       _Pragma("unroll") for (int c = 0; c < 3; ++c)                                 \
         kk[r * 3 + c] = G[r] * wR[c] + G[3 + r] * wR[3 + c];                        \
-      _Pragma("unroll") for (int r = 0; r < 3; ++r) kk[9 + r] = g.Xij[r];           \
     }                                                                               \
     {                                                                               \
              \
@@ -764,8 +768,9 @@
       double *cb = cbw + lane * 9;                                                  \
       _Pragma("unroll") for (int e_ = 0; e_ < 9; ++e_) cb[e_] = cbv[e_];            \
       if (wr_ && lane_on) {                                                         \
-        _Pragma("unroll") for (int r = 0; r < 6; ++r)                               \
+        _Pragma("unroll") for (int r = 0; r < 4; ++r)                               \
           stgW_mine[r] = make_double2(kk[2 * r], kk[2 * r + 1]);                    \
+        stgW8[rec_mine] = kk[8];                                                    \
       }                                                                             \
     }                                                                               \
     il0p = il0_;                                                                    \
@@ -1053,7 +1058,7 @@
   BA_KEEP_S(sd.chunk_begin);
   BA_KEEP_S(done);
   if (done) return;
-  const double *__restrict__ Wg = d.W[lbs];
+  const double *__restrict__ Wg = d.Wc[lbs];
   const double *__restrict__ bg = d.b[lbs];
   const int slot = (int)(lane_word & 0xffu);
   const int h = (int)((lane_word >> 8) & 1u), sub2 = (int)((lane_word >> 9) & 0x1fu);
@@ -1229,7 +1234,7 @@
 #else
 #define GRP_STAMP()
 #endif
-template <int NT>
+template <int NT, bool SLIM>
 __global__ __launch_bounds__(kBlock, (NT == 2 && BA_GRP_KRW <= 24) ? 3 : 2) void k_schur_grp(DevProblem d, const DevProblem::GrpDesc *grps) {
   constexpr int TW = 16 * NT;
 #ifndef BA_GRP_KRW
@@ -1252,32 +1257,52 @@
   const DevProblem::GrpDesc gd = grps[blockIdx.x];
   const int done = d.ctrl->done;
   const int lb = d.ctrl->lcur;
+  const int cur = d.ctrl->cur;
   BA_KEEP_S(gd.l0);
   BA_KEEP_S(done);
   if (done) return;
-  const double *__restrict__ Wg = d.W[lb];
+  const double *__restrict__ Wg = SLIM ? d.W[lb] : d.Wc[lb];
+  const double *__restrict__ Wg8 = d.W[lb] + (size_t)d.Pg * 8;
+  const double *__restrict__ Xg = d.pts[cur];
   const double *__restrict__ bg = d.b[lb];
   const double *__restrict__ Cug = d.Cu[lb];
   const double lp1 = 1.0 + d.ctrl->lambda;
   const int dd = gd.d;
   const int nlw = min(64 / dd, KRW / 3);
   const int il = lane / dd, jj = lane - il * dd;
+  double Tp[12];
+  if (SLIM) {
+    const double2 *tp = (const double2 *)(d.poses[cur] + (size_t)grps[blockIdx.x].pose[jj] * 12);
+#pragma unroll
+    for (int k = 0; k < 6; ++k) {
+      const double2 t2 = tp[k];
+      Tp[2 * k] = t2.x;
+      Tp[2 * k + 1] = t2.y;
+    }
+  }
   const int nch = (gd.nl + nlw - 1) / nlw;
   double *va = VA[wv], *wb = WB[wv];
   for (int e = lane; e < IMG; e += 64) {
     va[e] = 0.0;
     wb[e] = 0.0;
   }
-  double2 rw[2][6], rc[2][3];
-  double rb[2][3];
+  constexpr int RD = (NT == 4 && SLIM) ? 1 : 2;
+#define GRP_RB(B) (RD == 2 ? (B) : 0)
+  double2 rw[2][SLIM ? 4 : 6], rc[2][3];
+  double rb[2][3], rk8[2], rx[2][3];
 #define GRP_PREFETCH(B, ch_)                                                        \
   {                                                                                 \
     const int c0_ = (ch_) * nlw;                                                    \
     const bool on_ = il < min(nlw, gd.nl - c0_);                                    \
-    const double2 *wp_ = (const double2 *)(Wg + (size_t)(gd.p0 + (int64_t)c0_ * dd + (on_ ? lane : 0)) * kWStride); \
+    const size_t pr_ = (size_t)(gd.p0 + (int64_t)c0_ * dd + (on_ ? lane : 0));      \
+    const double2 *wp_ = (const double2 *)(Wg + pr_ * (SLIM ? 8 : kWStride));       \
     const int lm_ = gd.l0 + c0_ + (on_ ? il : 0);                                   \
     const double2 *cp_ = (const double2 *)(Cug + (size_t)lm_ * 6);                  \
-    _Pragma("unroll") for (int k_ = 0; k_ < 6; ++k_) rw[B][k_] = wp_[k_];           \
+    _Pragma("unroll") for (int k_ = 0; k_ < (SLIM ? 4 : 6); ++k_) rw[B][k_] = wp_[k_]; \
+    if (SLIM) {                                                                     \
+      rk8[B] = Wg8[pr_];                                                            \
+      _Pragma("unroll") for (int k_ = 0; k_ < 3; ++k_) rx[B][k_] = Xg[(size_t)lm_ * 3 + k_]; \
+    }                                                                               \
     _Pragma("unroll") for (int k_ = 0; k_ < 3; ++k_) rc[B][k_] = cp_[k_];           \
     _Pragma("unroll") for (int k_ = 0; k_ < 3; ++k_) rb[B][k_] = bg[(size_t)lm_ * 3 + k_]; \
   }
@@ -1285,7 +1310,7 @@
 #pragma unroll
   for (int t = 0; t < NTILE; ++t) acc[t] = (v4f64){0.0, 0.0, 0.0, 0.0};
   if (wv < nch) GRP_PREFETCH(0, wv)
-  if (wv + 4 < nch) GRP_PREFETCH(1, wv + 4)
+  if (RD == 2 && wv + 4 < nch) GRP_PREFETCH(1, wv + 4)
 #define GRP_IDX(k_, col_) (((k_) >> 1) * RS + (col_) * 2 + ((k_) & 1))
 #define GRP_STAGE(B)                                                                \
   if (ch < nch) {                                                                   \
@@ -1295,8 +1320,10 @@
        \
       _Pragma("clang fp contract(fast)")                                            \
       const double k9[9] = {rw[B][0].x, rw[B][0].y, rw[B][1].x, rw[B][1].y, rw[B][2].x, \
-                            rw[B][2].y, rw[B][3].x, rw[B][3].y, rw[B][4].x};        \
-      const double x0 = rw[B][4].y, x1 = rw[B][5].x, x2 = rw[B][5].y;               \
+                            rw[B][2].y, rw[B][3].x, rw[B][3].y, SLIM ? rk8[B] : rw[B][SLIM ? 0 : 4].x}; \
+      double xij_[3] = {rw[B][SLIM ? 0 : 4].y, rw[B][SLIM ? 0 : 5].x, rw[B][SLIM ? 0 : 5].y}; \
+      if (SLIM) pose_point(Tp, rx[B][0], rx[B][1], rx[B][2], xij_);                 \
+      const double x0 = xij_[0], x1 = xij_[1], x2 = xij_[2];                        \
           \
       const double cd_[6] = {rc[B][0].x * lp1, rc[B][0].y, rc[B][1].x, rc[B][1].y * lp1, rc[B][2].x, rc[B][2].y * lp1}; \
       double c6[6];                                                                 \
@@ -1334,7 +1361,7 @@
       }                                                                             \
     }                                                                               \
     GRP_STAMP()                                                                     \
-    if (ch + 8 < nch) GRP_PREFETCH(B, ch + 8)                                       \
+    if (ch + 4 * RD < nch) GRP_PREFETCH(B, ch + 4 * RD)                             \
     GRP_STAMP()                                                                     \
     __builtin_amdgcn_fence(__ATOMIC_RELEASE, "wavefront");                          \
     __builtin_amdgcn_wave_barrier();                                                \
@@ -1373,10 +1400,11 @@
     ch += 4;                                                                        \
   }
   for (int ch = wv; ch < nch;) {
-    GRP_STAGE(0)
-    GRP_STAGE(1)
+    GRP_STAGE(GRP_RB(0))
+    GRP_STAGE(GRP_RB(1))
   }
 #undef GRP_STAGE
+#undef GRP_RB
 #undef GRP_IDX
 #undef GRP_PREFETCH
   GRP_STAMP()
@@ -1415,6 +1443,7 @@
 }
 
 #define GW_LDS_BARRIER() asm volatile("s_waitcnt lgkmcnt(0)\n\ts_barrier" ::: "memory")
+template <bool SLIM>
 __global__ __launch_bounds__(kBlock, 2) void k_schur_grp_wide(DevProblem d, const DevProblem::GrpDesc *grps) {
   constexpr int TW = 128;
   constexpr int LPW = 2;
@@ -1439,13 +1468,26 @@
   const int gl0 = gp->l0, gnl = gp->nl, dd = gp->d, gs0 = gp->s0;
   const int done = d.ctrl->done;
   const int lb = d.ctrl->lcur;
+  const int cur = d.ctrl->cur;
   if (done) return;
-  const double *__restrict__ Wg = d.W[lb];
+  const double *__restrict__ Wg = SLIM ? d.W[lb] : d.Wc[lb];
+  const double *__restrict__ Wg8 = d.W[lb] + (size_t)d.Pg * 8;
+  const double *__restrict__ Xg = d.pts[cur];
   const double *__restrict__ bg = d.b[lb];
   const double *__restrict__ Cug = d.Cu[lb];
   const double lp1 = 1.0 + d.ctrl->lambda;
   const int nlw = min(64 / dd, LPW);
   const int il = lane / dd, jj = lane - il * dd;
+  double Tp[12];
+  if (SLIM) {
+    const double2 *tp = (const double2 *)(d.poses[cur] + (size_t)gp->pose[jj] * 12);
+#pragma unroll
+    for (int k = 0; k < 6; ++k) {
+      const double2 t2 = tp[k];
+      Tp[2 * k] = t2.x;
+      Tp[2 * k + 1] = t2.y;
+    }
+  }
   const int li = wv * nlw + il;
   const int per_stage = 4 * nlw;
   const int nst = (gnl + per_stage - 1) / per_stage;
@@ -1453,17 +1495,21 @@
     VA[e] = 0.0;
     WB[e] = 0.0;
   }
-  double2 rw[1][6], rc[1][3];
-  double rb[1][3];
+  double2 rw[1][SLIM ? 4 : 6], rc[1][3];
+  double rb[1][3], rk8[1], rx[1][3];
 #define GW_PREFETCH(B, st_)                                                         \
   {                                                                                 \
     const int c0_ = (st_) * per_stage;                                              \
     const bool on_ = il < nlw && c0_ + li < gnl;                                     \
-    const double2 *wp_ = (const double2 *)(Wg + (size_t)(gp0 + (int64_t)(c0_ + wv * nlw) * dd + (on_ ? lane : 0)) * kWStride); \
+    const size_t pr_ = on_ ? (size_t)(gp0 + (int64_t)(c0_ + wv * nlw) * dd + lane) : (size_t)gp0; \
+    const double2 *wp_ = (const double2 *)(Wg + pr_ * (SLIM ? 8 : kWStride));       \
     const int lm_ = gl0 + (on_ ? c0_ + li : 0);                                     \
     const double2 *cp_ = (const double2 *)(Cug + (size_t)lm_ * 6);                  \
-    if (!on_) wp_ = (const double2 *)(Wg + (size_t)gp0 * kWStride);                 \
-    _Pragma("unroll") for (int k_ = 0; k_ < 6; ++k_) rw[B][k_] = wp_[k_];           \
+    _Pragma("unroll") for (int k_ = 0; k_ < (SLIM ? 4 : 6); ++k_) rw[B][k_] = wp_[k_]; \
+    if (SLIM) {                                                                     \
+      rk8[B] = Wg8[pr_];                                                            \
+      _Pragma("unroll") for (int k_ = 0; k_ < 3; ++k_) rx[B][k_] = Xg[(size_t)lm_ * 3 + k_]; \
+    }                                                                               \
     _Pragma("unroll") for (int k_ = 0; k_ < 3; ++k_) rc[B][k_] = cp_[k_];           \
     _Pragma("unroll") for (int k_ = 0; k_ < 3; ++k_) rb[B][k_] = bg[(size_t)lm_ * 3 + k_]; \
   }
@@ -1478,13 +1524,16 @@
     const int c0 = st * per_stage;                                                  \
     const int nlc = min(per_stage, gnl - c0);                                       \
                \
-    _Pragma("unroll") for (int k_ = 0; k_ < 6; ++k_) asm volatile("" : "+v"(rw[B][k_].x), "+v"(rw[B][k_].y)); \
+    _Pragma("unroll") for (int k_ = 0; k_ < (SLIM ? 4 : 6); ++k_) asm volatile("" : "+v"(rw[B][k_].x), "+v"(rw[B][k_].y)); \
+    if (SLIM) asm volatile("" : "+v"(rk8[B]), "+v"(rx[B][0]), "+v"(rx[B][1]), "+v"(rx[B][2])); \
     _Pragma("unroll") for (int k_ = 0; k_ < 3; ++k_) asm volatile("" : "+v"(rc[B][k_].x), "+v"(rc[B][k_].y), "+v"(rb[B][k_])); \
     if (il < nlw && li < nlc) {                                                     \
       _Pragma("clang fp contract(fast)")                                            \
       const double k9[9] = {rw[B][0].x, rw[B][0].y, rw[B][1].x, rw[B][1].y, rw[B][2].x, \
-                            rw[B][2].y, rw[B][3].x, rw[B][3].y, rw[B][4].x};        \
-      const double x0 = rw[B][4].y, x1 = rw[B][5].x, x2 = rw[B][5].y;               \
+                            rw[B][2].y, rw[B][3].x, rw[B][3].y, SLIM ? rk8[B] : rw[B][SLIM ? 0 : 4].x}; \
+      double xij_[3] = {rw[B][SLIM ? 0 : 4].y, rw[B][SLIM ? 0 : 5].x, rw[B][SLIM ? 0 : 5].y}; \
+      if (SLIM) pose_point(Tp, rx[B][0], rx[B][1], rx[B][2], xij_);                 \
+      const double x0 = xij_[0], x1 = xij_[1], x2 = xij_[2];                        \
       const double cd_[6] = {rc[B][0].x * lp1, rc[B][0].y, rc[B][1].x, rc[B][1].y * lp1, rc[B][2].x, rc[B][2].y * lp1}; \
       double c6[6];                                                                 \
       spd3_inverse(cd_, c6);                                                        \
@@ -1584,7 +1633,7 @@
 
 __global__ __launch_bounds__(64) void k_schur_partial(DevProblem d) {
   if (d.ctrl->done) return;
-  const double *__restrict__ Wg = d.W[d.ctrl->lcur];
+  const double *__restrict__ Wg = d.Wc[d.ctrl->lcur];
   const double *__restrict__ bg = d.b[d.ctrl->lcur];
   const int ch = blockIdx.x;
   double acc[36], racc[6];
@@ -1854,7 +1903,7 @@
 #define BS_STAMP()
 #endif
 constexpr int kBgLm = 16;
-constexpr int kBgArea = 64 * kWStride + 64 * 3 + 64 * 12 + 64 * 3;
+constexpr int kBgArea = 64 * kWSlim + 64 * 3 + 64 * 12 + 64 * 3;
 constexpr int kBsLds = (kSchurPairs * (kWStride + 6 + 3) > 4 * kBgArea) ? kSchurPairs * (kWStride + 6 + 3) : 4 * kBgArea;
 
 __device__ __forceinline__ void backsub_chunk_body(const DevProblem &d, const int bx, const int part, double *lds,
@@ -1883,7 +1932,7 @@
   if (done) return;
   const double *__restrict__ Xc = d.pts[cur];
   double *__restrict__ Xt = d.pts[cur ^ 1];
-  const double *__restrict__ Wg = d.W[lbs];
+  const double *__restrict__ Wg = d.Wc[lbs];
   const double *__restrict__ bg = d.b[lbs];
   const double *__restrict__ Cg = d.Cu[lbs];
   double2 rw[kBsRW];
@@ -2052,10 +2101,21 @@
     const double2 a0 = xp[0], a1 = xp[1], a2 = xp[2];
     xj[0] = a0.x; xj[1] = a0.y; xj[2] = a1.x; xj[3] = a1.y; xj[4] = a2.x; xj[5] = a2.y;
   }
+  double Tp[12];
+  {
+    const double2 *tp = (const double2 *)(d.poses[cur] + (size_t)pose * 12);
+#pragma unroll
+    for (int k = 0; k < 6; ++k) {
+      const double2 t2 = tp[k];
+      Tp[2 * k] = t2.x;
+      Tp[2 * k + 1] = t2.y;
+    }
+  }
   double *__restrict__ Xt = d.pts[cur ^ 1];
   const double2 *__restrict__ Wg2 = (const double2 *)d.W[lbs];
+  const double *__restrict__ Wg8 = d.W[lbs] + (size_t)d.Pg * 8;
   double *Wim = lds + wv * kBgArea;
-  double *Us = Wim + 64 * kWStride;
+  double *Us = Wim + 64 * kWSlim;
   double *Lm = Us + 64 * 3;
   double *Bx = Lm + 64 * 12;
   const int S = 64 / nlwb;
@@ -2076,22 +2136,23 @@
     lm_p[k] = (a == 0 ? d.Cu[lbs] : (a == 1 ? d.b[lbs] : d.pts[cur])) + (size_t)l0 * lm_m[k] + lm_e[k];
     lm_q[k] = q;
   }
-  double2 rwA0, rwA1, rwA2, rwA3, rwA4, rwA5, rwB0, rwB1, rwB2, rwB3, rwB4, rwB5;
+  double2 rwA0, rwA1, rwA2, rwA3, rwB0, rwB1, rwB2, rwB3;
+  double rwA4, rwB4;
   double lmA0, lmA1, lmA2, lmB0, lmB1, lmB2;
 #define BSG_ISSUE(R, L, ST)                                                         \
   {                                                                                 \
     const int il0_ = il0_of(ST);                                                    \
     const int nls_ = max(0, min(nlwb, nl - il0_));                                  \
-    const int last_ = max(0, nls_ * dd * 6 - 1);                                    \
+    const int last_ = max(0, nls_ * dd * 4 - 1);                                    \
     const int ilb_ = nls_ > 0 ? il0_ : 0;                                           \
     const int lml_ = max(0, nls_ - 1);                                              \
-    const double2 *src_ = Wg2 + (dd > 0 ? (size_t)(p0 + (int64_t)ilb_ * dd) * 6 : (size_t)0); \
+    const size_t pr_ = dd > 0 ? (size_t)(p0 + (int64_t)ilb_ * dd) : (size_t)0;      \
+    const double2 *src_ = Wg2 + pr_ * 4;                                            \
     R##0 = src_[min(lane, last_)];                                                  \
     R##1 = src_[min(lane + 64, last_)];                                             \
     R##2 = src_[min(lane + 128, last_)];                                            \
     R##3 = src_[min(lane + 192, last_)];                                            \
-    R##4 = src_[min(lane + 256, last_)];                                            \
-    R##5 = src_[min(lane + 320, last_)];                                            \
+    R##4 = Wg8[pr_ + min(lane, max(0, nls_ * dd - 1))];                             \
     L##0 = lm_p[0][(size_t)(ilb_ + min(lm_l[0], lml_)) * lm_m[0]];                  \
     L##1 = lm_p[1][(size_t)(ilb_ + min(lm_l[1], lml_)) * lm_m[1]];                  \
     L##2 = lm_p[2][(size_t)(ilb_ + min(lm_l[2], lml_)) * lm_m[2]];                  \
@@ -2116,8 +2177,7 @@
     ((double2 *)Wim)[lane + 64] = R##1;                                             \
     ((double2 *)Wim)[lane + 128] = R##2;                                            \
     ((double2 *)Wim)[lane + 192] = R##3;                                            \
-    ((double2 *)Wim)[lane + 256] = R##4;                                            \
-    ((double2 *)Wim)[lane + 320] = R##5;                                            \
+    Wim[64 * 8 + lane] = R##4;                                                      \
     Lm[sb * nlwb * 12 + lm_q[0]] = L##0;                                            \
     Lm[sb * nlwb * 12 + lm_q[1]] = L##1;                                            \
     Lm[sb * nlwb * 12 + lm_q[2]] = L##2;                                            \
@@ -2125,9 +2185,13 @@
     BSG_WAVE_SYNC()                                                                 \
     if (lane_on) {                                                                  \
                    \
-      const double2 *w2 = (const double2 *)(Wim + lane * kWStride);                 \
-      const double2 k01 = w2[0], k23 = w2[1], k45 = w2[2], k67 = w2[3], k8x = w2[4], xx = w2[5]; \
-      const double X0 = k8x.y, X1 = xx.x, X2 = xx.y;                                \
+      const double2 *w2 = (const double2 *)(Wim + lane * 8);                        \
+      const double2 k01 = w2[0], k23 = w2[1], k45 = w2[2], k67 = w2[3];             \
+      const double2 k8x = make_double2(Wim[64 * 8 + lane], 0.0);                    \
+      const double *xi_ = Lm + sb * nlwb * 12 + nlwb * 9 + ilw * 3;                 \
+      double xij_[3];                                                               \
+      pose_point(Tp, xi_[0], xi_[1], xi_[2], xij_);                                 \
+      const double X0 = xij_[0], X1 = xij_[1], X2 = xij_[2];                        \
       const double e0 = xj[0] + (xj[4] * X2 - xj[5] * X1);                          \
       const double e1 = xj[1] + (xj[5] * X0 - xj[3] * X2);                          \
       const double e2 = xj[2] + (xj[3] * X1 - xj[4] * X0);                          \
@@ -2768,12 +2832,19 @@
 }
 #endif
 void launch_schur_accumulate(const DevProblem &d, hipStream_t s) {
-  if (d.n_grp32 > 0)
-    BA_LAUNCH(K_SCHUR_GRP, k_schur_grp<2>, dim3(d.n_grp32), dim3(kBlock), s, d, d.grp32);
-  if (d.n_grp64 > 0)
-    BA_LAUNCH(K_SCHUR_GRP, k_schur_grp<4>, dim3(d.n_grp64), dim3(kBlock), s, d, d.grp64);
-  if (d.n_grp128 > 0)
-    BA_LAUNCH(K_SCHUR_GRP, k_schur_grp_wide, dim3(d.n_grp128), dim3(kBlock), s, d, d.grp128);
+  const bool slim = d.Pg > 0;
+  if (d.n_grp32 > 0) {
+    if (slim) BA_LAUNCH(K_SCHUR_GRP, (k_schur_grp<2, true>), dim3(d.n_grp32), dim3(kBlock), s, d, d.grp32);
+    else BA_LAUNCH(K_SCHUR_GRP, (k_schur_grp<2, false>), dim3(d.n_grp32), dim3(kBlock), s, d, d.grp32);
+  }
+  if (d.n_grp64 > 0) {
+    if (slim) BA_LAUNCH(K_SCHUR_GRP, (k_schur_grp<4, true>), dim3(d.n_grp64), dim3(kBlock), s, d, d.grp64);
+    else BA_LAUNCH(K_SCHUR_GRP, (k_schur_grp<4, false>), dim3(d.n_grp64), dim3(kBlock), s, d, d.grp64);
+  }
+  if (d.n_grp128 > 0) {
+    if (slim) BA_LAUNCH(K_SCHUR_GRP, k_schur_grp_wide<true>, dim3(d.n_grp128), dim3(kBlock), s, d, d.grp128);
+    else BA_LAUNCH(K_SCHUR_GRP, k_schur_grp_wide<false>, dim3(d.n_grp128), dim3(kBlock), s, d, d.grp128);
+  }
   if (d.n_sup > 0)
     BA_LAUNCH(K_SCHUR_LDS, k_schur_lds, dim3(d.n_sup), dim3(kBlock), s, d);
   if (d.n_tchunk > 0)
diff --git a/include/ba_hip.h b/include/ba_hip.h
--- a/include/ba_hip.h
+++ b/include/ba_hip.h
@@ -131,6 +131,8 @@
 int ba_get_schur_info(ba_handle *h, int64_t out8[8]);
 
 int ba_get_lin_info(ba_handle *h, int64_t out4[4]);
+
+int ba_get_w_info(ba_handle *h, int64_t out4[4]);
 
 int ba_get_mask_info(ba_handle *h, int64_t out4[4]);
 
```

New measurement: 2388 it/s (median of 6 runs). 1.05x the previous value.
